# vrenkens/tfkaldi

Measured on AMD Instinct MI355X. Metric: acoustic frames/sec (train step), higher is better.
Workload: dtype f32 emulated (3xbf16 planes, 6 products, f32 accumulate)

## Files before the change

### tfkaldi_amd/build.py

```python
import os
import shutil
import subprocess
import sys
from concurrent.futures import ThreadPoolExecutor

HERE = os.path.dirname(os.path.abspath(__file__))
CSRC = os.path.join(HERE, "csrc")
LIBDIR = os.path.join(HERE, "lib")
LIBNAME = "libtfkaldi_hip.so"
SOURCES = ["gemm_f32.hip", "gemm_bf16.hip", "kernels.hip", "ctc.hip", "engine.hip", "features.hip", "exchange.hip"]
HEADERS = ["gemm_f32.h", "gemm_bf16.h", "kernels.h", "ctc.h", "x3_layout.h", os.path.join("..", "..", "include", "tfkaldi_hip.h")]
FLAGS = ["--offload-arch=gfx950", "-O3", "-std=c++17", "-fPIC", "-Wno-unused-value"]


def lib_path():
    return os.path.join(LIBDIR, LIBNAME)


TRAFFIC_STAMP_SOURCES = ("gemm_f32.hip", "gemm_f32.h", "gemm_bf16.hip", "gemm_bf16.h", "x3_layout.h")


def csrc_hash():
    import hashlib
    h = hashlib.sha256()
    for name in sorted(TRAFFIC_STAMP_SOURCES):
        with open(os.path.join(CSRC, name), "rb") as fid:
            h.update(name.encode() + b"\0" + fid.read())
    return h.hexdigest()[:16]


def _hipcc():
    exe = shutil.which("hipcc") or "/opt/rocm/bin/hipcc"
    if not os.path.exists(exe):
        raise RuntimeError("hipcc not found: cannot build the gfx950 engine")
    return exe


def _digest(names, extra=b""):
    import hashlib
    h = hashlib.sha256(extra)
    for name in names:
        with open(os.path.join(CSRC, name), "rb") as fid:
            h.update(os.path.basename(name).encode() + b"\0" + fid.read() + b"\0")
    return h.hexdigest()


def source_id():
    return _digest(sorted(SOURCES) + sorted(HEADERS), " ".join(FLAGS).encode())[:32]


_ID_MARK = b"TFK_BUILD_ID="


def library_id(path=None):
    path = path or lib_path()
    if not os.path.exists(path):
        return None
    with open(path, "rb") as fid:
        blob = fid.read()
    at = blob.find(_ID_MARK)
    if at < 0:
        return None
    return blob[at + len(_ID_MARK):at + len(_ID_MARK) + 32].decode("ascii", "replace")


def _stale():
    return library_id() != source_id()


def build_native(force=False, verbose=False):
    if not force and not _stale():
        return lib_path()
    hipcc = _hipcc()
    os.makedirs(LIBDIR, exist_ok=True)
    objdir = os.path.join(HERE, "..", "build", "obj")
    os.makedirs(objdir, exist_ok=True)
    build_id = source_id()

    def compile_one(src):
        obj = os.path.join(objdir, src.replace(".hip", ".o"))
        flags = list(FLAGS)
        if src == "engine.hip":
            flags.append('-DTFK_BUILD_ID="%s"' % build_id)
        key = _digest([src] + sorted(HEADERS), " ".join(flags).encode())
        stamp = obj + ".sha256"
        if not force and os.path.exists(obj) and os.path.exists(stamp) and open(stamp).read() == key:
            return obj
        cmd = [hipcc] + flags + ["-c", os.path.join(CSRC, src), "-o", obj]
        r = subprocess.run(cmd, capture_output=True, text=True)
        if r.returncode != 0:
            raise RuntimeError("hipcc failed for %s:\n%s" % (src, r.stderr[-4000:]))
        if verbose and r.stderr:
            sys.stderr.write(r.stderr)
        with open(stamp, "w") as fid:
# ... 19 lines not shown
```

### tfkaldi_amd/csrc/engine.hip

```cpp
#include "../../include/tfkaldi_hip.h"
#include "ctc.h"
#include "gemm_bf16.h"
#include "gemm_f32.h"
#include "kernels.h"

#include <hip/hip_runtime.h>
#include <chrono>

#include <math.h>
#include <stdarg.h>
#include <stdlib.h>
#include <stdio.h>
#include <string.h>

#include <algorithm>
#include <string>
#include <vector>

using namespace tfk;

namespace {

thread_local std::string g_err;

// ... 11 lines not shown
  do {                                                                                            \
    hipError_t e_ = (expr);                                                                       \
    if (e_ != hipSuccess) return fail((int)e_, "%s failed: %s (%s:%d)", #expr, hipGetErrorString(e_), \
                                      __FILE__, __LINE__);                                        \
  } while (0)
#define CHK(expr)            \
  do {                       \
    int rc_ = (expr);        \
    if (rc_ != 0) return rc_; \
  } while (0)

inline size_t up(size_t x, size_t a) { return (x + a - 1) / a * a; }

struct LayerLayout {
  int d_in, d_out, ld_in, ld_out;
  size_t w_off, b_off, beta_off;
  size_t w_sz, b_sz, beta_sz;
};

enum KernelFamily {
  KF_GEMM_NN = 0, KF_GEMM_NT, KF_GEMM_TN, KF_GEMM_DUAL, KF_BN_STATS, KF_ACT_FWD, KF_HIDDEN_BWD, KF_COLSUM, KF_SOFTMAX_XENT,
  KF_LOSS_REDUCE, KF_SOFTMAX, KF_ADAM, KF_EMA, KF_MISC, KF_CTC_BEST_PATH, KF_EDIT_DISTANCE, KF_COUNT
};
const char* kFamilyName[KF_COUNT] = {"gemm_f32_nn(fwd affine)", "gemm_f32_nt(dA)",  "gemm_f32_tn(dW)",
                                     "gemm_f32_dual(dA+dW)",    "bn_stats",
                                     "act_forward",             "hidden_backward",  "colsum",          "softmax_xent",
                                     "loss_reduce",             "softmax_rows",     "adam_apply",      "bn_ema_apply",
                                     "misc",                    "ctc_best_path",    "edit_distance"};

struct ProfRec {
  int family;
  hipEvent_t a, b;
  double flops, bytes;
};

}

struct tfk_engine {
  tfk_config cfg;
  int F, L, H, O, ldF, ldH, ldO;
  float bn_decay, bn_eps, b1, b2, adam_eps;
  bool dropout;

  hipStream_t stream = nullptr, copy_stream = nullptr;
  bool own_stream = false;
  hipStream_t opt_stream = nullptr;
  hipEvent_t ev_opt_begin = nullptr, ev_opt_vec = nullptr;
  std::vector<hipEvent_t> ev_adam;
  bool opt_overlap = false;
  bool opt_pending = false;
  float* d_snap = nullptr;
  hipEvent_t ev_loss = nullptr;
  unsigned loss_seq = 0;
  bool loss_event = false;
  bool slot_lazy = true;
  hipEvent_t ev_grow = nullptr;
  std::vector<void*> host_garbage;

  float* state = nullptr;
  bool own_state = false;
  size_t P = 0, E = 0, state_floats = 0;
  size_t off_param = 0, off_grad = 0, off_scalars = 0, off_ema = 0, off_m = 0, off_v = 0, off_mov = 0, off_shadow = 0;
  size_t reduce_floats = 0;
  std::vector<LayerLayout> lay;

  int cap = 0;
  float* dX[2] = {nullptr, nullptr};
  int32_t* dY[2] = {nullptr, nullptr};
  std::vector<float*> z, a, v, rowscale, mean, rstd;
  float *logits = nullptr, *post = nullptr, *dA[2] = {nullptr, nullptr}, *row_loss = nullptr, *ws = nullptr;
  float* dRaw[2] = {nullptr, nullptr};
  int32_t* dSeg[2] = {nullptr, nullptr};
  float* hRaw[2] = {nullptr, nullptr};
  int32_t* hSeg[2] = {nullptr, nullptr};
  float* dCmvn[2] = {nullptr, nullptr};
  float* hCmvn[2] = {nullptr, nullptr};
  size_t cmvn_cap = 0;
  int seg_cap = 0;
  std::vector<float*> seg_mean, seg_rstd;
  float* ws_stats = nullptr;
  float* ws_bwd = nullptr;
  float* ws_splitk = nullptr;
  size_t ws_splitk_floats = 0;
  size_t ws_bwd_stride = 0;
  float* prior = nullptr;
  bool have_prior = false;

  float* hX[2] = {nullptr, nullptr};
  int32_t* hY[2] = {nullptr, nullptr};
  float* h_post = nullptr;
  size_t h_post_floats = 0;
  float* h_scalars = nullptr;
  float* h_scalars_dev = nullptr;
  bool apply_open = false, apply_direct = false;
  float cur_lr_t = 0.f;
  bool scalars_fresh = true;
  bool colsum_done = false;
  bool fuse_hb_enabled = true;
  bool dual_gemm = true;
  bool stack_enabled = true;
  bool fuse_eval = true;
  int post_chunk = 2048;
  std::vector<hipEvent_t> post_ev;

  int32_t *ctc_seg = nullptr, *ctc_lab_off = nullptr, *ctc_lab = nullptr;
  float *ctc_lp = nullptr, *ctc_ab = nullptr, *ctc_bb = nullptr, *ctc_utt_loss = nullptr, *ctc_lse = nullptr;
  double *ctc_off = nullptr, *ctc_offb = nullptr, *ctc_logz = nullptr;
  size_t ctc_cap_bb = 0, ctc_cap_offb = 0, ctc_cap_logz = 0;
  int32_t* h_ctc[2] = {nullptr, nullptr};
  size_t h_ctc_cap[2] = {0, 0};
  hipEvent_t ctc_staged[2] = {nullptr, nullptr};
  int ctc_stage_slot = 0;
  size_t ctc_cap_offrows = 0;
  size_t ctc_cap_seg = 0, ctc_cap_off = 0, ctc_cap_loss = 0, ctc_cap_lab = 0, ctc_cap_lp = 0, ctc_cap_ab = 0,
         ctc_cap_rows = 0;
  int32_t* ctc_dec = nullptr;
  size_t ctc_cap_dec = 0;
  int32_t* h_dec = nullptr;
  size_t h_dec_cap = 0;

  bool bf16 = false;
  bool x3 = false;
  size_t tw_elems(size_t rows, int ld) const { return x3 ? x3::elems(rows, ld) : rows * ld; }
  size_t tw_row(size_t r, int ld) const { return x3 ? x3::at(r, 0, ld) : r * ld; }
  ShadowMap wb_map;
  int ldFb = 0, ldHb = 0, ldOb = 0;
  bf16_t* Xb[2] = {nullptr, nullptr};
  std::vector<bf16_t*> ab;
  bf16_t* logb = nullptr;
  bf16_t* dAb[2] = {nullptr, nullptr};
  bf16_t* Wb = nullptr;
  std::vector<size_t> wb_off;
  std::vector<int> wb_ld;
  bool wb_aligned = false;
  bool own_wb = false;
  unsigned long long* d_checksum = nullptr;
  bool shadow_dirty = true;
  hipEvent_t copy_done[2] = {nullptr, nullptr}, compute_done[2] = {nullptr, nullptr};
  bool slot_used[2] = {false, false};
  unsigned long long slot_step[2] = {0, 0}, steps_begun = 0, steps_seen = 0;
  int slot = 0;

  int64_t global_step = 0, adam_t = 0;
  double lr_fact = 1.0;
  int initialised_layers = 0;
  uint32_t call_counter = 0;
  int later_mb = 0;
  bool grads_fresh = true;

  tfk_bucket_fn cb = nullptr;
  void* cb_user = nullptr;
  tfk_layer_fn layer_cb = nullptr;
  void* layer_user = nullptr;

  int last_T = 0, last_nfw = 0;
  uint32_t last_call = 0;
  const float* last_in = nullptr;

  bool profiling = false;
  std::vector<ProfRec> prof;
  std::vector<hipEvent_t> ev_pool;
  size_t ev_next = 0;

  int nact() const {
    if (!cfg.layerwise_init) return L;
    int n = initialised_layers + 1;
// ... 165 lines not shown
    to_bf16_rows(e->stream, e->p_param() + y.w_off, y.ld_out, e->Wb + e->wb_off[l], e->wb_ld[l], y.d_in, y.d_out, e->x3);
  }
  HIPCHK(hipGetLastError());
  e->shadow_dirty = false;
  return 0;
}

struct ActEpi {
  const float *a, *z, *mean, *rstd;
  int nonlin;
  const float* beta = nullptr;
  float eps = 0.f;
  bf16_t* twin = nullptr;
  int ld_twin = 0;
  float scale = 1.f;
};
template <class Args>
void fill_epilogue(Args& g, const ActEpi* act, float* stats, const int* row_vend) {
  g.stats = stats;
  g.stats_stride = kMaxRowSplits;
  g.act_a = act ? act->a : nullptr; g.act_z = act ? act->z : nullptr;
  g.act_mean = act ? act->mean : nullptr; g.act_rstd = act ? act->rstd : nullptr;
  g.act_nonlin = act ? act->nonlin : 0;
  g.act_beta = act ? act->beta : nullptr; g.bn_eps = act ? act->eps : 0.f;
  g.act_scale = act ? act->scale : 1.f;
  g.act_keep = act ? 1.f / act->scale : 1.f;
  g.row_vend = row_vend;
}
int grow_splitk(tfk_engine* e, size_t need, bool zero, hipStream_t st) {
  if (need <= e->ws_splitk_floats) return 0;
  dev_free(e, e->ws_splitk, true);
  e->ws_splitk = nullptr;
  e->ws_splitk_floats = 0;
  CHK(dev_alloc(e, (void**)&e->ws_splitk, need * sizeof(float), false));
  e->ws_splitk_floats = need;
  if (zero) HIPCHK(hipMemsetAsync(e->ws_splitk, 0, need * sizeof(float), st));
  return 0;
}
int run_gemm(tfk_engine* e, GemmLayout layout, const float* A, int lda, const float* B, int ldb, float* C, int ldc,
             int M, int N, int K, const float* bias, int epi, hipStream_t st = nullptr, float* stats = nullptr,
             int cfg = -1, const ActEpi* act = nullptr, const int* row_vend = nullptr) {
  if (!st) st = e->stream;
  const int fam = layout == GEMM_NN ? KF_GEMM_NN : layout == GEMM_NT ? KF_GEMM_NT : KF_GEMM_TN;
  if (e->bf16) {
    GemmArgsB b = {};
    int lda8 = 0, ldb8 = 0;
    b.A = twin_of(e, A, &lda8);
    b.B = twin_of(e, B, &ldb8);
    if (!b.A || !b.B) return fail(-1, "internal: GEMM operand without a bf16 twin");
    b.C = C; b.bias = bias;
    fill_epilogue(b, act, stats, row_vend);
    b.C_twin = act ? act->twin : nullptr; b.ldct = act ? act->ld_twin : 0;
    b.ct_x3 = e->x3;
    b.M = M; b.N = N; b.K = K; b.lda = lda8; b.ldb = ldb8; b.ldc = ldc; b.epi = epi;
    if (e->x3) {
      CHK(grow_splitk(e, gemm_bf16x3_splitk_floats(layout, M, N, K), true, st));
      b.splitk_ws = e->ws_splitk;
      b.splitk_ws_floats = e->ws_splitk_floats;
      b.err = reinterpret_cast<unsigned*>(e->h_scalars_dev + kErrWord);
    }
    ProfScope ps(e, fam, 2.0 * M * N * K,
                 (e->x3 ? 6.0 : 2.0) * ((double)M * K + (double)K * N) + 4.0 * (double)M * N * ((epi & EPI_ACCUM) ? 2 : 1), st);
    const int rc = e->x3 ? gemm_bf16x3(layout, b, st) : gemm_bf16(layout, b, st);
    if (rc != 0) return fail(rc, "gemm_bf16%s launch failed: %s", e->x3 ? "x3" : "", hipGetErrorString((hipError_t)rc));
    return 0;
  }
  GemmArgs g;
  g.A = A; g.B = B; g.C = C; g.bias = bias;
  fill_epilogue(g, act, stats, row_vend);
  g.M = M; g.N = N; g.K = K; g.lda = lda; g.ldb = ldb; g.ldc = ldc; g.epi = epi;
  if (layout == GEMM_TN && K >= gemm_f32_splitk_min_k() && (size_t)M * N < ((size_t)1 << 20)) {
    CHK(grow_splitk(e, (size_t)32 * M * ldc, false, st));
    g.splitk_ws = e->ws_splitk;
    g.splitk_ws_floats = e->ws_splitk_floats;
  }
  ProfScope ps(e, fam, 2.0 * M * N * K, 4.0 * ((double)M * K + (double)K * N + (double)M * N * ((epi & EPI_ACCUM) ? 2 : 1)), st);
  const int rc = gemm_f32(layout, g, cfg, st);
  if (rc != 0) return fail(rc, "gemm_f32 launch failed: %s", hipGetErrorString((hipError_t)rc));
  return 0;
}

int run_gemm_dual(tfk_engine* e, const float* dz, int ld_dz, const float* W, int ldw, float* da_out, int ld_da, int T,
                  int N_da, int K_da, const ActEpi* act, float* stats, const float* in, int ld_in, float* Gw, int ld_g,
                  int d_in, int d_out, int epi_w, int* chunk_rows) {
  if (!e->dual_gemm) return 1;
  const double flops = 2.0 * T * N_da * K_da + 2.0 * d_in * d_out * T;
  const double out_w = (double)d_in * d_out * ((epi_w & EPI_ACCUM) ? 2 : 1);
  if (e->bf16) {
    const int dcfg = e->x3 ? -1 : gemm_bf16_dual_config(T, N_da, d_in, d_out);
    const int bm = e->x3 ? kGemmBf16x3TileRows : gemm_bf16_dual_tile_rows(dcfg);
    if (!dcfg || (act && (T + bm - 1) / bm > kMaxRowSplits)) return 1;
    GemmArgsB a = {}, w = {};
    int ld_a = 0, ld_b = 0, ld_c = 0, ld_d = 0;
    a.A = twin_of(e, dz, &ld_a);
    a.B = twin_of(e, W, &ld_b);
    w.A = twin_of(e, in, &ld_c);
    w.B = twin_of(e, dz, &ld_d);
    if (!a.A || !a.B || !w.A || !w.B) return fail(-1, "internal: GEMM operand without a bf16 twin");
    a.C = da_out;
    fill_epilogue(a, act, stats, nullptr);
    a.M = T; a.N = N_da; a.K = K_da; a.lda = ld_a; a.ldb = ld_b; a.ldc = ld_da; a.epi = act ? EPI_DACT : 0;
    w.C = Gw;
    w.M = d_in; w.N = d_out; w.K = T; w.lda = ld_c; w.ldb = ld_d; w.ldc = ld_g; w.epi = epi_w;
    const double ob = e->x3 ? 6.0 : 2.0;
    ProfScope ps(e, KF_GEMM_DUAL, flops, ob * ((double)T * K_da + (double)K_da * N_da) + 4.0 * (double)T * N_da +
                                             ob * ((double)T * d_in + (double)T * d_out) + 4.0 * out_w);
    const int rc = e->x3 ? gemm_bf16x3_dual(a, w, e->stream) : gemm_bf16_dual(a, w, e->stream);
    if (rc != 0) ps.drop();
    if (rc == -1) return 1;
    if (rc != 0) return fail(rc, "gemm_bf16%s_dual launch failed: %s", e->x3 ? "x3" : "", hipGetErrorString((hipError_t)rc));
    if (chunk_rows) *chunk_rows = bm;
    return 0;
  }
  GemmArgs a, w = {};
  a.A = dz; a.B = W; a.C = da_out; a.bias = nullptr;
  fill_epilogue(a, act, stats, nullptr);
  a.M = T; a.N = N_da; a.K = K_da; a.lda = ld_dz; a.ldb = ldw; a.ldc = ld_da; a.epi = act ? EPI_DACT : 0;
  w.A = in; w.B = dz; w.C = Gw;
  w.M = d_in; w.N = d_out; w.K = T; w.lda = ld_in; w.ldb = ld_dz; w.ldc = ld_g; w.epi = epi_w;
  ProfScope ps(e, KF_GEMM_DUAL, flops, 4.0 * ((double)T * K_da + (double)K_da * N_da + (double)T * N_da) +
                                           4.0 * ((double)T * d_in + (double)T * d_out + out_w));
  const int rc = gemm_f32_dual(a, w, e->stream);
  if (rc != 0) ps.drop();
  if (rc == -1) return 1;
  if (rc != 0) return fail(rc, "gemm_f32_dual launch failed: %s", hipGetErrorString((hipError_t)rc));
  return 0;
}

void free_activations(tfk_engine* e, bool async = false) {
  auto fr = [&](float*& p) { dev_free(e, p, async); p = nullptr; };
  for (int s = 0; s < 2; ++s) {
    fr(e->dX[s]);
    dev_free(e, e->dY[s], async); e->dY[s] = nullptr;
    fr(e->dA[s]);
    host_retire(e, e->hX[s], async); e->hX[s] = nullptr;
    host_retire(e, e->hY[s], async); e->hY[s] = nullptr;
    fr(e->dRaw[s]);
    dev_free(e, e->dSeg[s], async); e->dSeg[s] = nullptr;
    host_retire(e, e->hRaw[s], async); e->hRaw[s] = nullptr;
    host_retire(e, e->hSeg[s], async); e->hSeg[s] = nullptr;
    fr(e->dCmvn[s]);
    host_retire(e, e->hCmvn[s], async); e->hCmvn[s] = nullptr;
  }
  e->cmvn_cap = 0;
  auto frb = [&](bf16_t*& p) { dev_free(e, p, async); p = nullptr; };
  for (int s = 0; s < 2; ++s) { frb(e->Xb[s]); frb(e->dAb[s]); }
  for (auto& p : e->ab) frb(p);
  frb(e->logb);
  for (auto& p : e->z) fr(p);
  for (auto& p : e->a) fr(p);
  for (auto& p : e->v) fr(p);
  for (auto& p : e->rowscale) fr(p);
  fr(e->logits); fr(e->post); fr(e->row_loss); fr(e->ws); fr(e->ws_bwd); fr(e->ws_stats);
  e->cap = 0;
}

int alloc_zero(float** p, size_t floats) {
  HIPCHK(hipMalloc((void**)p, floats * sizeof(float)));
  HIPCHK(hipMemset(*p, 0, floats * sizeof(float)));
  return 0;
}
int alloc_zero_b(bf16_t** p, size_t elems) {
  HIPCHK(hipMalloc((void**)p, elems * sizeof(bf16_t)));
  HIPCHK(hipMemset(*p, 0, elems * sizeof(bf16_t)));
  return 0;
}
int grow_zero(tfk_engine* e, float** p, size_t floats) { return dev_alloc(e, (void**)p, floats * sizeof(float), true); }
int grow_zero_b(tfk_engine* e, bf16_t** p, size_t elems) { return dev_alloc(e, (void**)p, elems * sizeof(bf16_t), true); }

inline size_t seg_ints(int cap) { return (size_t)2 * cap + cap / 64 + 8; }

int reserve(tfk_engine* e, int T) {
  if (T <= e->cap) return 0;
  int cap = e->cap + e->cap / 2;
  if (cap < T) cap = T;
  cap = (int)up(cap, 64);
  for (int s = 0; s < 2; ++s)
    if (e->slot_used[s]) HIPCHK(hipEventSynchronize(e->copy_done[s]));
  free_activations(e, true);
  const int L = e->L;
  for (int s = 0; s < 2; ++s) {
    CHK(grow_zero(e, &e->dX[s], (size_t)cap * e->ldF));
    CHK(dev_alloc(e, (void**)&e->dY[s], (size_t)cap * sizeof(int32_t), false));
    CHK(grow_zero(e, &e->dA[s], (size_t)cap * e->ldH));
    HIPCHK(hipHostMalloc((void**)&e->hX[s], (size_t)cap * e->F * sizeof(float), hipHostMallocDefault));
    memset(e->hX[s], 0, (size_t)cap * e->F * sizeof(float));
    HIPCHK(hipHostMalloc((void**)&e->hY[s], (size_t)cap * sizeof(int32_t), hipHostMallocDefault));
    CHK(grow_zero(e, &e->dRaw[s], (size_t)cap * e->ldF));
    CHK(dev_alloc(e, (void**)&e->dSeg[s], seg_ints(cap) * sizeof(int32_t), false));
    HIPCHK(hipHostMalloc((void**)&e->hRaw[s], (size_t)cap * e->F * sizeof(float), hipHostMallocDefault));
// ... 272 lines not shown
      if (e->bf16) { ev.twin = e->ab[l]; ev.ld_twin = e->ldHb; }
      CHK(run_gemm(e, GEMM_NN, in, ld_in, e->p_param() + y.w_off, y.ld_out, e->a[l], ldH, T, H, y.d_in,
                   e->p_param() + y.b_off, EPI_BIAS | EPI_EVAL_ACT, nullptr, nullptr, -1, &ev));
      in = e->a[l];
      ld_in = ldH;
      continue;
    }
    CHK(run_gemm(e, GEMM_NN, in, ld_in, e->p_param() + y.w_off, y.ld_out, e->z[l], ldH, T, H, y.d_in,
                 e->p_param() + y.b_off, EPI_BIAS));
    if (e->cfg.batch_norm) {
      ProfScope ps(e, KF_BN_STATS, 0, 8.0 * T * H);
      if (train)
        bn_stats_train(e->stream, e->z[l], T, H, ldH, e->bn_eps, e->bn_decay, e->mean[l], e->rstd[l], e->ema_mean(l),
                       e->ema_var(l), e->ws);
      else
        bn_stats_eval(e->stream, e->mov_mean(l), e->mov_var(l), H, e->bn_eps, e->mean[l], e->rstd[l]);
    }
    {
      ProfScope ps(e, KF_ACT_FWD, 0, 8.0 * T * H);
      const ActDesc d = act_desc(e, l, train, call);
      act_forward(e->stream, d, e->z[l], e->a[l], e->cfg.l2_norm ? e->v[l] : nullptr,
                  e->cfg.l2_norm ? e->rowscale[l] : nullptr, e->mean[l], e->rstd[l],
                  e->cfg.batch_norm ? e->p_param() + y.beta_off : nullptr, T, H, ldH, twin_a(l));
    }
    in = e->a[l];
    ld_in = ldH;
  }
  const LayerLayout& o = e->lay[e->L];
  need_params(e, e->L);
  CHK(wait_layer_update(e, e->L, nfw == 0));
  CHK(run_gemm(e, GEMM_NN, e->a[nact - 1], ldH, e->p_param() + o.w_off, o.ld_out, e->logits, e->ldO, T, e->O, H,
               e->p_param() + o.b_off, EPI_BIAS));
  HIPCHK(hipGetLastError());
  return 0;
}

int backward(tfk_engine* e, const float* Xd, int ldx, int T, int nact, uint32_t call, bool fire, const Stack* st = nullptr) {
  const int L = e->L, H = e->H, ldH = e->ldH;
  const LayerLayout& o = e->lay[L];
  float* G = e->p_grad();
  const int acc = e->grads_fresh ? 0 : 1;
  const int epi_w = acc ? EPI_ACCUM : 0;
  if (!acc)
    for (int l = nact; l < L; ++l) {
      const LayerLayout& q = e->lay[l];
      HIPCHK(hipMemsetAsync(G + q.w_off, 0, q.w_sz * sizeof(float), e->stream));
      HIPCHK(hipMemsetAsync(G + q.b_off, 0, q.b_sz * sizeof(float), e->stream));
      if (q.beta_sz) HIPCHK(hipMemsetAsync(G + q.beta_off, 0, q.beta_sz * sizeof(float), e->stream));
    }
  FinalBatch fin;
  fin.n = 0;
  fin.accumulate = acc;
  const int rs = row_splits(T);
  auto ws_of = [&](int l) { return e->ws_bwd + (size_t)l * e->ws_bwd_stride; };
  {
    if (!e->colsum_done) {
      ProfScope ps(e, KF_COLSUM, 0, 4.0 * T * e->O);
      colsum_partial(e->stream, e->logits, T, e->ldO, ws_of(L));
    }
    e->colsum_done = false;
    fin.it[fin.n++] = {ws_of(L), G + o.b_off, 0, rs, e->O, e->ldO};
  }
  int pp = 0;
  int cfg_h, cfg_o;
  const int rows_h = gemm_chunk_rows(e, GEMM_NT, T, H, H, &cfg_h), rows_o = gemm_chunk_rows(e, GEMM_NT, T, H, e->O, &cfg_o);
  const bool drop = e->cfg.keep_prob < 1.f;
  const bool fuse_hb = e->cfg.batch_norm && !e->cfg.l2_norm && (!drop || e->cfg.nonlin == TFK_NONLIN_RELU) &&
                       e->fuse_hb_enabled && (T + rows_h - 1) / rows_h <= kMaxRowSplits &&
                       (T + rows_o - 1) / rows_o <= kMaxRowSplits;
  const std::vector<float*>& mean = st ? e->seg_mean : e->mean;
  const std::vector<float*>& rstd = st ? e->seg_rstd : e->rstd;
  auto act_of = [&](int l) {
    ActEpi act = {e->a[l], e->z[l], mean[l], rstd[l], e->cfg.nonlin};
    act.scale = drop ? 1.f / e->cfg.keep_prob : 1.f;
    act.beta = e->cfg.batch_norm ? e->p_param() + e->lay[l].beta_off : nullptr;
    return act;
  };
  auto dact_gemm = [&](const float* dz, int ld_dz, const float* W, int ldw, float* out, int K, int target, int cfg) {
    if (!fuse_hb) return run_gemm(e, GEMM_NT, dz, ld_dz, W, ldw, out, ldH, T, H, K, nullptr, 0);
    const ActEpi act = act_of(target);
    return run_gemm(e, GEMM_NT, dz, ld_dz, W, ldw, out, ldH, T, H, K, nullptr, EPI_DACT, nullptr, ws_of(target), cfg, &act);
  };
  int bm_in = rows_o;
  {
    const ActEpi act = act_of(nact - 1);
    const int rc = run_gemm_dual(e, e->logits, e->ldO, e->p_param() + o.w_off, o.ld_out, e->dA[pp], ldH, T, H, e->O,
                                 fuse_hb ? &act : nullptr, fuse_hb ? ws_of(nact - 1) : nullptr, e->a[nact - 1], ldH,
                                 G + o.w_off, o.ld_out, H, e->O, epi_w, &bm_in);
    if (rc < 0) return rc;
    if (rc > 0) {
      CHK(run_gemm(e, GEMM_TN, e->a[nact - 1], ldH, e->logits, e->ldO, G + o.w_off, o.ld_out, H, e->O, T, nullptr, epi_w));
      CHK(dact_gemm(e->logits, e->ldO, e->p_param() + o.w_off, o.ld_out, e->dA[pp], e->O, nact - 1, cfg_o));
    }
  }
  if (fire && e->cb) {
    e->cb(e->cb_user, 0);
    for (int l = L - 1; l >= nact; --l) e->cb(e->cb_user, L - l);
  }
  for (int l = nact - 1; l >= 0; --l) {
    const LayerLayout& y = e->lay[l];
    float* da = e->dA[pp];
    const int chunks_in = (T + bm_in - 1) / bm_in;
    auto fin_layer = [&](int n_beta, int n_bias) {
      if (e->cfg.batch_norm) fin.it[fin.n++] = {ws_of(l), G + y.beta_off, 0, n_beta, H, ldH};
      fin.it[fin.n++] = {ws_of(l), G + y.b_off, 2, n_bias, H, ldH};
      if (fin.n + 2 > kMaxFinalItems) {
        grad_final(e->stream, fin);
        fin.n = 0;
      }
    };
    Twin tw;
    if (e->bf16) { tw.p = e->dAb[pp]; tw.ld = e->ldHb; tw.x3 = e->x3; }
    if (st) {
      if (!fuse_hb || stack_align(e) % bm_in || chunks_in > kMaxRowSplits)
        return fail(-1, "internal: EPI_DACT chunks of %d rows do not fit a stacked pass of %d rows", bm_in, T);
      int slot = 0;
      for (int i = 0; i < st->k; ++i) {
        ProfScope ps(e, KF_HIDDEN_BWD, 0, 28.0 * st->rows[i] * H);
        const ActDesc d = act_desc(e, l, 1, call + (uint32_t)i);
        Twin tws = tw;
        if (e->bf16) tws.p += e->tw_row((size_t)st->r0[i], e->ldHb);
        const size_t r = (size_t)st->r0[i] * ldH;
        hidden_backward(e->stream, d, 1, da + r, e->a[l] + r, e->z[l] + r, mean[l] + (size_t)i * ldH, rstd[l] + (size_t)i * ldH,
                        st->rows[i], H, ldH, ws_of(l) + (size_t)(st->r0[i] / bm_in) * ldH, (st->rows[i] + bm_in - 1) / bm_in, tws,
                        st->span[i], ws_of(l) + ((size_t)2 * kMaxRowSplits + slot) * ldH);
        slot += row_splits(st->span[i]);
      }
      if (slot > kMaxRowSplits) return fail(-1, "internal: %d partial-sum slots in a stacked pass", slot);
      fin_layer(chunks_in, slot);
    } else {
      const ActDesc d = act_desc(e, l, 1, call);
      int pre_du = fuse_hb ? 1 : 0;
      if (e->cfg.l2_norm) {
        ProfScope ps(e, KF_HIDDEN_BWD, 0, 12.0 * T * H);
        act_backward_rows(e->stream, d, da, e->v[l], e->rowscale[l], T, H, ldH);
        pre_du = 1;
      }
      ProfScope ps(e, KF_HIDDEN_BWD, 0, (e->cfg.batch_norm ? 28.0 : 12.0) * T * H);
      int chunks_eff = fuse_hb ? chunks_in : 0;
      if (chunks_eff > kMergeOnceChunks) {
        chunk_totals(e->stream, ws_of(l), chunks_eff, ldH);
        chunks_eff = 1;
      }
      hidden_backward(e->stream, d, pre_du, da, e->a[l], e->z[l], mean[l], rstd[l], T, H, ldH, ws_of(l), chunks_eff, tw);
      fin_layer(fuse_hb ? chunks_eff : rs, rs);
    }
    const float* in = l == 0 ? Xd : e->a[l - 1];
    const int ld_in = l == 0 ? ldx : ldH;
    bool fused = false;
    bm_in = rows_h;
    if (l > 0) {
      const ActEpi act = act_of(l - 1);
      const int rc = run_gemm_dual(e, da, ldH, e->p_param() + y.w_off, y.ld_out, e->dA[pp ^ 1], ldH, T, H, H,
                                   fuse_hb ? &act : nullptr, fuse_hb ? ws_of(l - 1) : nullptr, in, ld_in, G + y.w_off,
                                   y.ld_out, y.d_in, H, epi_w, &bm_in);
      if (rc < 0) return rc;
      fused = rc == 0;
    }
    if (!fused) {
      CHK(run_gemm(e, GEMM_TN, in, ld_in, da, ldH, G + y.w_off, y.ld_out, y.d_in, H, T, nullptr, epi_w));
      if (l > 0) CHK(dact_gemm(da, ldH, e->p_param() + y.w_off, y.ld_out, e->dA[pp ^ 1], H, l - 1, cfg_h));
    }
    if (fire && e->cb) e->cb(e->cb_user, L - l);
    pp ^= 1;
  }
  {
    ProfScope ps(e, KF_COLSUM, 0, 0);
    grad_final(e->stream, fin);
  }
  HIPCHK(hipGetLastError());
  return 0;
}

int check_kernel_errors(tfk_engine* e) {
  volatile unsigned* w = reinterpret_cast<volatile unsigned*>(e->h_scalars + kErrWord);
  if (*w == 0) return 0;
  *w = 0;
  if (e->ws_splitk)
    (void)hipMemsetAsync(e->ws_splitk, 0, e->ws_splitk_floats * sizeof(float), e->stream);
  return fail(-1, "split-K exchange timed out: a block of the fp32-emulating contraction waited ~1 s for its partner's partial "
                  "sums (workspace not zeroed, or the partner block failed); the results of this step are invalid");
}

int settle_scalars(tfk_engine* e) {
  if (e->scalars_fresh) {
    HIPCHK(hipMemsetAsync(e->p_scalars(), 0, kScalarFloats * sizeof(float), e->stream));
    e->scalars_fresh = false;
  }
  return 0;
}
int read_scalars(tfk_engine* e) {
  CHK(settle_scalars(e));
  HIPCHK(hipMemcpyAsync(e->h_scalars, e->p_scalars(), 4 * sizeof(float), hipMemcpyDeviceToHost, e->stream));
  HIPCHK(hipStreamSynchronize(e->stream));
  e->scalars_fresh = true;
  return check_kernel_errors(e);
}

struct TensorRef {
  float* ptr;
  int rows, cols, ld;
};
int tensor_ref(tfk_engine* e, int kind, int slot, int layer, TensorRef* t) {
  const int L = e->L;
  if (kind == TFK_WEIGHTS || kind == TFK_BIASES) {
    if (layer < 0 || layer > L) return fail(-1, "layer %d out of range [0, %d]", layer, L);
  } else if (kind >= TFK_BN_BETA && kind <= TFK_BN_MOVING_VAR) {
    if (layer < 0 || layer >= L) return fail(-1, "layer %d out of range [0, %d)", layer, L);
    if (!e->cfg.batch_norm) return fail(-1, "batch norm tensors requested but batch_norm is off");
  } else {
    return fail(-1, "unknown tensor kind %d", kind);
  }
  float* base;
  switch (slot) {
    case TFK_SLOT_PARAM: base = e->p_param(); break;
    case TFK_SLOT_GRAD: base = e->p_grad(); break;
    case TFK_SLOT_ADAM_M: base = e->p_m(); break;
    case TFK_SLOT_ADAM_V: base = e->p_v(); break;
    default: return fail(-1, "unknown tensor slot %d", slot);
  }
  const LayerLayout& y = e->lay[layer < 0 ? 0 : layer];
  switch (kind) {
    case TFK_WEIGHTS: *t = {base + y.w_off, y.d_in, y.d_out, y.ld_out}; break;
    case TFK_BIASES: *t = {base + y.b_off, 1, y.d_out, y.ld_out}; break;
    case TFK_BN_BETA: *t = {base + y.beta_off, 1, e->H, e->ldH}; break;
    case TFK_BN_MOVING_MEAN:
    case TFK_BN_MOVING_VAR:
      if (slot != TFK_SLOT_PARAM) return fail(-1, "moving statistics only have the PARAM slot");
      *t = {kind == TFK_BN_MOVING_MEAN ? e->mov_mean(layer) : e->mov_var(layer), 1, e->H, e->ldH};
      break;
  }
  return 0;
}

int create_impl(const tfk_config* cfg, void* state, size_t state_bytes, void* stream, tfk_engine** out) {
  if (!out) return fail(-1, "out is NULL");
  *out = nullptr;
  CHK(validate(cfg));
  HIPCHK(hipSetDevice(cfg->device));
  tfk_engine* e = new tfk_engine();
  e->cfg = *cfg;
  e->F = cfg->input_dim; e->L = cfg->num_layers; e->H = cfg->num_units; e->O = cfg->output_dim;
  e->ldF = (int)up(e->F, 4); e->ldH = (int)up(e->H, 4); e->ldO = (int)up(e->O, 4);
  e->bf16 = cfg->compute_dtype != TFK_DTYPE_F32;
  e->x3 = cfg->compute_dtype == TFK_DTYPE_F32X3;
  const size_t ldq = e->x3 ? 32 : 8;
  e->ldFb = (int)up(e->F, ldq); e->ldHb = (int)up(e->H, ldq); e->ldOb = (int)up(e->O, ldq);
  e->bn_decay = cfg->bn_decay > 0.f ? cfg->bn_decay : 0.999f;
  e->bn_eps = cfg->bn_epsilon > 0.f ? cfg->bn_epsilon : 1e-3f;
  e->b1 = cfg->adam_beta1 > 0.f ? cfg->adam_beta1 : 0.9f;
  e->b2 = cfg->adam_beta2 > 0.f ? cfg->adam_beta2 : 0.999f;
  e->adam_eps = cfg->adam_epsilon > 0.f ? cfg->adam_epsilon : 1e-8f;
  e->dropout = cfg->keep_prob < 1.f;
  compute_layout(cfg, e->lay, e->P, e->E);
  e->state_floats = total_state_floats(e->P, e->E, shadow_floats(cfg, e->lay));
  e->off_param = 0;
  e->off_grad = e->P;
  e->off_scalars = 2 * e->P;
  e->off_ema = 2 * e->P + kScalarFloats;
  e->reduce_floats = e->P + kScalarFloats + e->E;
  e->off_m = e->off_ema + e->E;
  e->off_v = e->off_m + e->P;
  e->off_mov = e->off_v + e->P;
  e->off_shadow = e->off_mov + e->E;

  auto bail = [&](int rc) { tfk_destroy(e); return rc; };
#define HIPB(expr)                                                                                          \
  do {                                                                                                      \
    hipError_t e_ = (expr);                                                                                 \
    if (e_ != hipSuccess) return bail(fail((int)e_, "%s failed: %s", #expr, hipGetErrorString(e_)));        \
  } while (0)
  if (stream) {
    e->stream = (hipStream_t)stream;
  } else {
    HIPB(hipStreamCreateWithFlags(&e->stream, hipStreamNonBlocking));
    e->own_stream = true;
  }
  HIPB(hipStreamCreateWithFlags(&e->copy_stream, hipStreamNonBlocking));
  {
    const char* v;
    if ((v = getenv("TFK_FUSE_HB"))) e->fuse_hb_enabled = atoi(v) != 0;
    if ((v = getenv("TFK_POST_CHUNK"))) e->post_chunk = atoi(v) > 0 ? (int)up((size_t)atoi(v), 64) : 0;
    if ((v = getenv("TFK_DUAL_GEMM"))) e->dual_gemm = atoi(v) != 0;
    if ((v = getenv("TFK_STACK"))) e->stack_enabled = atoi(v) != 0;
    if ((v = getenv("TFK_LOSS_EVENT"))) e->loss_event = atoi(v) != 0;
    if ((v = getenv("TFK_SLOT_EVENT"))) e->slot_lazy = atoi(v) == 0;
    if ((v = getenv("TFK_FUSE_EVAL"))) e->fuse_eval = atoi(v) != 0;
  }
  {
    const char* v = getenv("TFK_ADAM_OVERLAP");
    e->opt_overlap = v ? atoi(v) != 0 : false;
  }
  if (e->opt_overlap) {
    HIPB(hipStreamCreateWithFlags(&e->opt_stream, hipStreamNonBlocking));
    HIPB(hipEventCreateWithFlags(&e->ev_opt_begin, hipEventDisableTiming));
    HIPB(hipEventCreateWithFlags(&e->ev_opt_vec, hipEventDisableTiming));
    e->ev_adam.assign(e->L + 1, nullptr);
    for (int l = 0; l <= e->L; ++l) HIPB(hipEventCreateWithFlags(&e->ev_adam[l], hipEventDisableTiming));
  }
  HIPB(hipMalloc((void**)&e->d_snap, 16 * sizeof(float)));
  HIPB(hipEventCreateWithFlags(&e->ev_loss, hipEventDisableTiming));
  HIPB(hipEventCreateWithFlags(&e->ev_grow, hipEventDisableTiming));
  for (int s = 0; s < 2; ++s) {
    HIPB(hipEventCreateWithFlags(&e->copy_done[s], hipEventDisableTiming));
    HIPB(hipEventCreateWithFlags(&e->compute_done[s], hipEventDisableTiming));
  }
  if (state) {
    if (state_bytes < e->state_floats * sizeof(float))
      return bail(fail(-1, "state arena too small: %zu < %zu bytes", state_bytes, e->state_floats * sizeof(float)));
    if (((uintptr_t)state) % 256) return bail(fail(-1, "state arena must be 256-byte aligned"));
    e->state = (float*)state;
  } else {
    HIPB(hipMalloc((void**)&e->state, e->state_floats * sizeof(float)));
    e->own_state = true;
  }
  HIPB(hipMemsetAsync(e->state, 0, e->state_floats * sizeof(float), e->stream));
  if (cfg->batch_norm)
    for (int l = 0; l < e->L; ++l) fill(e->stream, e->mov_var(l), (size_t)e->H, 1.0f);
  HIPB(hipHostMalloc((void**)&e->h_scalars, 16 * sizeof(float), hipHostMallocMapped | hipHostMallocCoherent));
  memset(e->h_scalars, 0, 16 * sizeof(float));
  HIPB(hipHostGetDevicePointer((void**)&e->h_scalars_dev, e->h_scalars, 0));
  e->mean.assign(e->L, nullptr);
  e->rstd.assign(e->L, nullptr);
  for (int l = 0; l < e->L; ++l) {
    if (alloc_zero(&e->mean[l], (size_t)e->ldH) || alloc_zero(&e->rstd[l], (size_t)e->ldH)) return bail(-1);
  }
  if (alloc_zero(&e->prior, (size_t)e->ldO)) return bail(-1);
  if (e->bf16) {
    e->wb_aligned = e->x3 ? (e->L + 1 <= kShadowMapMax) : shadow_mirrors(cfg, e->lay);
    e->wb_off.assign(e->L + 1, 0);
    e->wb_ld.assign(e->L + 1, 0);
    e->wb_map.n = 0;
    size_t off = 0;
    for (int l = 0; l <= e->L; ++l) {
      const LayerLayout& y = e->lay[l];
      e->wb_ld[l] = (int)up(y.d_out, e->x3 ? 32 : 8);
      e->wb_off[l] = (e->wb_aligned && !e->x3) ? y.w_off : off;
      off += e->x3 ? up(x3::elems(y.d_in, e->wb_ld[l]), 64) : up((size_t)y.d_in * e->wb_ld[l], 64);
      if (e->x3 && e->wb_aligned) {
        ShadowMap& m = e->wb_map;
        m.begin[l] = (uint32_t)y.w_off; m.rows[l] = (uint32_t)y.d_in; m.ld[l] = (uint32_t)y.ld_out;
        m.ld_twin[l] = (uint32_t)e->wb_ld[l]; m.twin[l] = e->wb_off[l];
        m.n = l + 1;
      }
    }
    if (e->x3) {
      if (alloc_zero_b(&e->Wb, up(off, 128))) return bail(-1);
      e->own_wb = true;
    } else if (e->wb_aligned) {
      e->Wb = reinterpret_cast<bf16_t*>(e->state + e->off_shadow);
    } else {
      if (alloc_zero_b(&e->Wb, off)) return bail(-1);
      e->own_wb = true;
    }
    e->shadow_dirty = true;
  }
  const int cap0 = cfg->max_frames > 0 ? cfg->max_frames : 1024;
  { const int rc = reserve(e, cap0); if (rc) return bail(rc); }
  HIPB(hipStreamSynchronize(e->stream));
#undef HIPB
  *out = e;
  return 0;
}

struct CtcSpec {
  const int32_t* utt_len;
  int U;
  const int32_t* labels;
  const int32_t* label_len;
};
template <class Tp>
int grow(tfk_engine* e, Tp** p, size_t* cap, size_t need) {
  if (need <= *cap) return 0;
  dev_free(e, *p, true);
  *p = nullptr;
  *cap = 0;
  const size_t n = need + need / 2;
  CHK(dev_alloc(e, (void**)p, n * sizeof(Tp), false));
  *cap = n;
  return 0;
}
int ctc_stage(tfk_engine* e, const CtcSpec& c, int T, bool need_labels, int* max_labels_out) {
  if (c.U <= 0 || !c.utt_len || (need_labels && !c.label_len)) return fail(-1, "CTC: no utterances");
  std::vector<int32_t> seg(c.U + 1, 0), off(c.U + 1, 0);
  int max_labels = 0;
  for (int u = 0; u < c.U; ++u) {
    const int32_t n = c.label_len ? c.label_len[u] : 0;
    if (c.utt_len[u] < 0 || n < 0) return fail(-1, "CTC: negative length");
    seg[u + 1] = seg[u] + c.utt_len[u];
    off[u + 1] = off[u] + n;
    max_labels = n > max_labels ? n : max_labels;
  }
  if (seg[c.U] != T) return fail(-1, "CTC: utterance lengths sum to %d, expected T = %d", seg[c.U], T);
  if (max_labels > kCtcMaxLabels) return fail(-1, "CTC: %d labels in one utterance (limit %d)", max_labels, kCtcMaxLabels);
  const int total = off[c.U];
  if (total > 0 && !c.labels) return fail(-1, "CTC: labels is NULL");
  for (int i = 0; i < total; ++i)
    if (c.labels[i] < 0 || c.labels[i] >= e->O - 1) return fail(-1, "CTC: label %d outside [0, %d)", c.labels[i], e->O - 1);
  CHK(grow(e, &e->ctc_seg, &e->ctc_cap_seg, (size_t)c.U + 1));
  CHK(grow(e, &e->ctc_lab_off, &e->ctc_cap_off, (size_t)c.U + 1));
  CHK(grow(e, &e->ctc_lab, &e->ctc_cap_lab, (size_t)(total > 0 ? total : 1)));
  {
    const int k = e->ctc_stage_slot ^= 1;
    const size_t need = 2 * ((size_t)c.U + 1) + (size_t)total;
    if (!e->ctc_staged[k]) HIPCHK(hipEventCreateWithFlags(&e->ctc_staged[k], hipEventDisableTiming));
    else HIPCHK(hipEventSynchronize(e->ctc_staged[k]));
    if (need > e->h_ctc_cap[k]) {
      if (e->h_ctc[k]) HIPCHK(hipHostFree(e->h_ctc[k]));
      e->h_ctc[k] = nullptr;
      e->h_ctc_cap[k] = need + need / 2;
// ... 271 lines not shown
  int D;
};
int check_seg_utts(const tfk_engine* e, const char* who, const int32_t* utt_len, int U, int T, int context_width,
                   const int32_t* seg_utts, int k, int flags, SegTable* t) {
  if (flags & (TFK_DEVICE_PTRS | TFK_RAW_DEVICE)) return fail(-1, "%s takes host pointers", who);
  if (k <= 0) return fail(-1, "no micro-batch (k = %d)", k);
  const int win = 2 * context_width + 1;
  if (context_width < 0 || e->F % win) return fail(-1, "input_dim %d is not a multiple of 2*context_width+1 = %d", e->F, win);
  t->D = e->F / win;
  t->first_utt.assign(k + 1, 0);
  t->first_row.assign(k + 1, 0);
  t->seg_rows.assign(k, 0);
  for (int i = 0; i < k; ++i) {
    if (seg_utts[i] <= 0) return fail(-1, "micro-batch %d of the stack holds no utterance", i);
    t->first_utt[i + 1] = t->first_utt[i] + seg_utts[i];
    if (t->first_utt[i + 1] > U) return fail(-1, "the micro-batches hold more than U = %d utterances", U);
    for (int u = t->first_utt[i]; u < t->first_utt[i + 1]; ++u) {
      if (utt_len[u] < 0) return fail(-1, "negative utterance length");
      t->seg_rows[i] += utt_len[u];
    }
    if (t->seg_rows[i] <= 0) return fail(-1, "micro-batch %d of the stack is empty", i);
    t->first_row[i + 1] = t->first_row[i] + t->seg_rows[i];
  }
  if (t->first_utt[k] != U || t->first_row[k] != T)
    return fail(-1, "the micro-batches hold %d utterances / %d frames, expected U = %d / T = %d", t->first_utt[k], t->first_row[k], U, T);
  return 0;
}

}

namespace tfk {
int set_error(int code, const char* msg) { return fail(code, "%s", msg); }
}

extern "C" {

int tfk_abi_version(void) { return TFK_ABI_VERSION; }
#ifndef TFK_BUILD_ID
#error "compile engine.hip through tfkaldi_amd/build.py: it passes -DTFK_BUILD_ID=<hash of the sources>"
#endif
static const char kBuildId[] = "TFK_BUILD_ID=" TFK_BUILD_ID;
const char* tfk_build_id(void) { return kBuildId + 13; }
const char* tfk_last_error(void) { return g_err.c_str(); }

int tfk_state_bytes(const tfk_config* cfg, size_t* bytes) {
  CHK(validate(cfg));
  if (!bytes) return fail(-1, "bytes is NULL");
  std::vector<LayerLayout> lay;
  size_t P, E;
  compute_layout(cfg, lay, P, E);
  *bytes = total_state_floats(P, E, shadow_floats(cfg, lay)) * sizeof(float);
  return 0;
}

int tfk_create(const tfk_config* cfg, tfk_engine** out) { return create_impl(cfg, nullptr, 0, nullptr, out); }
int tfk_create_ex(const tfk_config* cfg, void* state, size_t state_bytes, void* stream, tfk_engine** out) {
  return create_impl(cfg, state, state_bytes, stream, out);
}

int tfk_destroy(tfk_engine* e) {
  if (!e) return 0;
  hipSetDevice(e->cfg.device);
  if (e->stream) hipStreamSynchronize(e->stream);
  if (e->copy_stream) hipStreamSynchronize(e->copy_stream);
  if (e->opt_stream) hipStreamSynchronize(e->opt_stream);
  free_activations(e);
  for (void* p : e->host_garbage) (void)hipHostFree(p);
  e->host_garbage.clear();
  if (e->ev_loss) hipEventDestroy(e->ev_loss);
  if (e->ev_grow) hipEventDestroy(e->ev_grow);
  if (e->ev_opt_begin) hipEventDestroy(e->ev_opt_begin);
  if (e->ev_opt_vec) hipEventDestroy(e->ev_opt_vec);
  for (hipEvent_t ev : e->ev_adam) if (ev) hipEventDestroy(ev);
  if (e->opt_stream) hipStreamDestroy(e->opt_stream);
  if (e->d_snap) hipFree(e->d_snap);
  for (auto p : e->mean) if (p) hipFree(p);
  for (auto p : e->seg_mean) if (p) hipFree(p);
  for (auto p : e->seg_rstd) if (p) hipFree(p);
  for (auto p : e->rstd) if (p) hipFree(p);
  if (e->prior) hipFree(e->prior);
  if (e->Wb && e->own_wb) hipFree(e->Wb);
  if (e->d_checksum) hipFree(e->d_checksum);
  if (e->ws_splitk) hipFree(e->ws_splitk);
  for (void* p : {(void*)e->ctc_seg, (void*)e->ctc_lab_off, (void*)e->ctc_lab, (void*)e->ctc_lp, (void*)e->ctc_ab,
                  (void*)e->ctc_utt_loss, (void*)e->ctc_lse, (void*)e->ctc_off, (void*)e->ctc_bb, (void*)e->ctc_offb,
                  (void*)e->ctc_logz, (void*)e->ctc_dec})
    if (p) hipFree(p);
  if (e->h_dec) hipHostFree(e->h_dec);
  for (hipEvent_t ev : e->post_ev) hipEventDestroy(ev);
  for (int k = 0; k < 2; ++k) {
    if (e->h_ctc[k]) hipHostFree(e->h_ctc[k]);
    if (e->ctc_staged[k]) hipEventDestroy(e->ctc_staged[k]);
  }
  if (e->h_scalars) hipHostFree(e->h_scalars);
  if (e->h_post) hipHostFree(e->h_post);
  if (e->own_state && e->state) hipFree(e->state);
  for (int s = 0; s < 2; ++s) {
    if (e->copy_done[s]) hipEventDestroy(e->copy_done[s]);
    if (e->compute_done[s]) hipEventDestroy(e->compute_done[s]);
  }
  for (auto ev : e->ev_pool) hipEventDestroy(ev);
  if (e->copy_stream) hipStreamDestroy(e->copy_stream);
  if (e->own_stream && e->stream) hipStreamDestroy(e->stream);
  delete e;
  return 0;
}

int tfk_tensor_count(tfk_engine* e, int kind, int layer, size_t* count) {
  if (!e || !count) return fail(-1, "NULL argument");
  TensorRef t;
  CHK(tensor_ref(e, kind, TFK_SLOT_PARAM, layer, &t));
  *count = (size_t)t.rows * t.cols;
  return 0;
}

int tfk_tensor_get(tfk_engine* e, int kind, int slot, int layer, float* host, size_t count) {
  if (!e || !host) return fail(-1, "NULL argument");
  TensorRef t;
  CHK(tensor_ref(e, kind, slot, layer, &t));
  if (count != (size_t)t.rows * t.cols) return fail(-1, "count %zu != %d x %d", count, t.rows, t.cols);
  HIPCHK(hipSetDevice(e->cfg.device));
  if (slot == TFK_SLOT_GRAD && e->grads_fresh) {
    memset(host, 0, count * sizeof(float));
    return 0;
  }
  if (slot == TFK_SLOT_PARAM) need_params(e, -1);
  CHK(sync_streams(e));
  HIPCHK(hipMemcpy2D(host, (size_t)t.cols * 4, t.ptr, (size_t)t.ld * 4, (size_t)t.cols * 4, t.rows, hipMemcpyDeviceToHost));
  return 0;
}

int tfk_tensor_set(tfk_engine* e, int kind, int slot, int layer, const float* host, size_t count) {
  if (!e || !host) return fail(-1, "NULL argument");
  TensorRef t;
  CHK(tensor_ref(e, kind, slot, layer, &t));
  if (count != (size_t)t.rows * t.cols) return fail(-1, "count %zu != %d x %d", count, t.rows, t.cols);
  HIPCHK(hipSetDevice(e->cfg.device));
  if (slot == TFK_SLOT_PARAM) need_params(e, -1);
  CHK(sync_streams(e));
  if (slot == TFK_SLOT_GRAD && e->grads_fresh) {
    HIPCHK(hipMemsetAsync(e->p_grad(), 0, e->P * sizeof(float), e->stream));
    e->grads_fresh = false;
  }
  HIPCHK(hipStreamSynchronize(e->stream));
  HIPCHK(hipMemcpy2D(t.ptr, (size_t)t.ld * 4, host, (size_t)t.cols * 4, (size_t)t.cols * 4, t.rows, hipMemcpyHostToDevice));
  if (slot == TFK_SLOT_PARAM) e->shadow_dirty = true;
  return 0;
}

static double current_lr(const tfk_engine* e) {
  const double frac = e->cfg.num_steps > 0 ? (double)e->global_step / (double)e->cfg.num_steps : 0.0;
  return (double)e->cfg.init_learning_rate * pow((double)e->cfg.learning_rate_decay, frac) * e->lr_fact;
}

int tfk_scalar_get(tfk_engine* e, int which, double* value) {
  if (!e || !value) return fail(-1, "NULL argument");
  switch (which) {
    case TFK_GLOBAL_STEP: *value = (double)e->global_step; return 0;
    case TFK_LEARNING_RATE_FACT: *value = e->lr_fact; return 0;
    case TFK_INITIALISED_LAYERS: *value = (double)e->initialised_layers; return 0;
    case TFK_ADAM_STEPS: *value = (double)e->adam_t; return 0;
    case TFK_LEARNING_RATE: *value = current_lr(e); return 0;
    case TFK_BATCH_LOSS:
    case TFK_NUM_FRAMES: {
      HIPCHK(hipSetDevice(e->cfg.device));
      if (e->scalars_fresh) { *value = 0.0; return 0; }
// ... 857 lines not shown
```

### tfkaldi_amd/csrc/gemm_bf16.h

```cpp
#pragma once
#include <hip/hip_runtime.h>
#include <stdint.h>

#include "gemm_f32.h"

namespace tfk {

typedef uint16_t bf16_t;

struct GemmArgsB {
  const bf16_t* A;
  const bf16_t* B;
  float* C;
  const float* bias;
  float* stats;
  const float* act_a;
  const float* act_z;
  const float* act_mean;
  const float* act_rstd;
  int act_nonlin;
  int stats_stride;
  int M, N, K;
  int lda, ldb, ldc;
  int epi;
  const float* act_beta;
  float bn_eps;
  bf16_t* C_twin;
  int ldct;
  float act_scale;
  float act_keep;
  const int* row_vend;
  int ct_x3;
  float* splitk_ws;
  size_t splitk_ws_floats;
  unsigned* err;
  int splitk_local;
  int splitk_skew;
};

constexpr int kNumGemmBf16Configs = 9;

int gemm_bf16(GemmLayout layout, const GemmArgsB& args, hipStream_t stream);

int gemm_bf16_dual(const GemmArgsB& nt, const GemmArgsB& tn, hipStream_t stream);
int gemm_bf16_dual_config(int M_nt, int N_nt, int M_tn, int N_tn);
int gemm_bf16_dual_tile_rows(int cfg);

int gemm_bf16x3(GemmLayout layout, const GemmArgsB& args, hipStream_t stream);
constexpr int kGemmBf16x3TileRows = 128;
size_t gemm_bf16x3_splitk_floats(GemmLayout layout, int M, int N, int K);
int gemm_bf16x3_dual(const GemmArgsB& nt, const GemmArgsB& tn, hipStream_t stream);

int gemm_bf16_tile_rows(int M, int N);

void gemm_bf16_force_config(int cfg);
int gemm_bf16_pick_config(int M, int N);

}
```

### tfkaldi_amd/csrc/gemm_bf16.hip

```cpp
#include "gemm_bf16.h"
#include "x3_layout.h"

#include <math.h>
#include <stdlib.h>
#include <string.h>

#include <type_traits>

namespace tfk {
namespace {

typedef __bf16 bf16x8 __attribute__((ext_vector_type(8)));
typedef __bf16 bf16x4 __attribute__((ext_vector_type(4)));
typedef float f32x16 __attribute__((ext_vector_type(16)));
typedef uint32_t u32x4 __attribute__((ext_vector_type(4)));
typedef int i32x4 __attribute__((ext_vector_type(4)));

constexpr int BK = 64;
constexpr int kOOB = (int)0x80000000;
constexpr int NUM_XCD = 8;

__device__ __forceinline__ void tile_of_seq(int tiles_m, int tiles_n, int group_rows, int seq, int& tm, int& tn) {
  const int per_group = group_rows * tiles_n;
  const int grp = seq / per_group;
  const int first_m = grp * group_rows;
  const int gsize = min(group_rows, tiles_m - first_m);
  const int within = seq - grp * per_group;
  tm = first_m + within % gsize;
  tn = within / gsize;
}
__device__ __forceinline__ void tile_of_block(int tiles_m, int tiles_n, int group_rows, int bid, int& tm, int& tn) {
  const int nwg = tiles_m * tiles_n;
  const int xcd = bid % NUM_XCD, loc = bid / NUM_XCD;
  const int q = nwg / NUM_XCD, r = nwg % NUM_XCD;
  const int seq = (xcd < r ? xcd * (q + 1) : r * (q + 1) + (xcd - r) * q) + loc;
  tile_of_seq(tiles_m, tiles_n, group_rows, seq, tm, tn);
}

__device__ __forceinline__ uint16_t f2bf(float x) { return __builtin_bit_cast(uint16_t, (__bf16)x); }

template <int EPI, int WAVES_M, int WAVES_N, int FM, int FN, bool CBUF = false>
__device__ __forceinline__ void epilogue(const GemmArgsB& p, f32x16 (&acc)[FM][FN], int tiles_m, int tm, int m0, int n0,
                                         int wm, int wn, int i, int h, float* red) {
  constexpr int BM = WAVES_M * FM * 32, BN = WAVES_N * FN * 32;
  auto row_of = [&](int a, int r) { return m0 + (wm * FM + a) * 32 + 4 * h + (r & 3) + 8 * (r >> 2); };
#pragma unroll
  for (int b = 0; b < FN; ++b) {
    const int cidx = (wn * FN + b) * 32 + i;
    const int col = n0 + cidx;
    const bool col_ok = col < p.N;
    const int colc = col_ok ? col : p.N - 1;
    if constexpr ((EPI & EPI_BIAS) != 0) {
      const float bv = p.bias[colc];
#pragma unroll
      for (int a = 0; a < FM; ++a)
#pragma unroll
        for (int r = 0; r < 16; ++r) acc[a][b][r] += bv;
    }
    if constexpr ((EPI & EPI_EVAL_ACT) != 0) {
      const bool bn = p.act_mean != nullptr;
      const float mu = bn ? p.act_mean[colc] : 0.f;
      const float rs = bn ? rsqrtf(p.act_rstd[colc] + p.bn_eps) : 1.f;
      const float be = bn ? p.act_beta[colc] : 0.f;
#pragma unroll
      for (int a = 0; a < FM; ++a)
#pragma unroll
        for (int r = 0; r < 16; ++r) {
          float u = acc[a][b][r];
          if (bn) u = (u - mu) * rs + be;
          switch (p.act_nonlin) {
            case 0: u = fmaxf(u, 0.f); break;
            case 1: u = 1.f / (1.f + expf(-u)); break;
            case 2: u = tanhf(u); break;
            default: break;
          }
          acc[a][b][r] = u;
        }
    }
    if constexpr ((EPI & EPI_COLSTATS) != 0) {
      const int vlim = p.row_vend ? min(p.M, p.row_vend[m0 >> 6]) : p.M;
      const int n_tile = max(1, min(BM, vlim - m0));
      float cmean = 0.f;
#pragma unroll
      for (int pass = 0; pass < 2; ++pass) {
        float s = 0.f;
#pragma unroll
        for (int a = 0; a < FM; ++a)
#pragma unroll
          for (int r = 0; r < 16; ++r) {
            const float v = acc[a][b][r];
            if (row_of(a, r) < vlim) s += pass == 0 ? v : (v - cmean) * (v - cmean);
          }
        s += __shfl_xor(s, 32);
        if (h == 0) red[wm * BN + cidx] = s;
        __syncthreads();
        float t = 0.f;
#pragma unroll
        for (int w = 0; w < WAVES_M; ++w) t += red[w * BN + cidx];
        if (pass == 0) {
          cmean = t / (float)n_tile;
        } else if (wm == 0 && h == 0 && col_ok) {
          p.stats[((size_t)0 * tiles_m + tm) * p.ldc + col] = cmean;
          p.stats[((size_t)1 * tiles_m + tm) * p.ldc + col] = t;
        }
        __syncthreads();
      }
    }
    if constexpr ((EPI & EPI_DACT) != 0) {
      const float mu = p.act_mean[colc], rsd = p.act_rstd[colc];
      const float dscale = p.act_scale > 0.f ? p.act_scale : 1.f;
      const bool from_a = p.act_nonlin == 0 && p.act_beta != nullptr;
      const float be = from_a ? p.act_beta[colc] : 0.f;
      const float keep = p.act_keep > 0.f ? p.act_keep : 1.f;
      float s1 = 0.f, s2 = 0.f;
#pragma unroll
      for (int a = 0; a < FM; ++a) {
        float av[16], zv[16];
#pragma unroll
        for (int r = 0; r < 16; ++r) {
          const int row = min(row_of(a, r), p.M - 1);
          av[r] = p.act_a[(size_t)row * p.ldc + colc];
        }
        if (!from_a) {
#pragma unroll
          for (int r = 0; r < 16; ++r) {
            const int row = min(row_of(a, r), p.M - 1);
            zv[r] = p.act_z[(size_t)row * p.ldc + colc];
          }
        }
#pragma unroll
        for (int r = 0; r < 16; ++r) {
          float d1;
          switch (p.act_nonlin) {
            case 0: d1 = av[r] > 0.f ? dscale : 0.f; break;
            case 1: d1 = av[r] * (1.f - av[r]); break;
            case 2: d1 = 1.f - av[r] * av[r]; break;
            default: d1 = 1.f;
          }
          const float du = acc[a][b][r] * d1;
          acc[a][b][r] = du;
          if (row_of(a, r) < p.M) {
            s1 += du;
            s2 += du * (from_a ? av[r] * keep - be : (zv[r] - mu) * rsd);
          }
        }
      }
      s1 += __shfl_xor(s1, 32);
      s2 += __shfl_xor(s2, 32);
      if (h == 0) {
        red[(0 * WAVES_M + wm) * BN + cidx] = s1;
        red[(1 * WAVES_M + wm) * BN + cidx] = s2;
      }
      __syncthreads();
      if (wm == 0 && h == 0 && col_ok) {
        float t1 = 0.f, t2 = 0.f;
#pragma unroll
        for (int w = 0; w < WAVES_M; ++w) {
          t1 += red[(0 * WAVES_M + w) * BN + cidx];
          t2 += red[(1 * WAVES_M + w) * BN + cidx];
        }
        p.stats[((size_t)0 * p.stats_stride + tm) * p.ldc + col] = t1;
        p.stats[((size_t)1 * p.stats_stride + tm) * p.ldc + col] = t2;
      }
      __syncthreads();
    }
    if constexpr (CBUF) {
      static_assert((EPI & EPI_EVAL_ACT) == 0, "no bf16 twin on this path");
      const __amdgpu_buffer_rsrc_t crs =
          __builtin_amdgcn_make_buffer_rsrc((void*)p.C, 0, (int)(((unsigned)(p.M - 1) * p.ldc + p.N) * 4u), 0x00020000);
#pragma unroll
      for (int a = 0; a < FM; ++a) {
        const unsigned base = col_ok ? ((unsigned)(m0 + (wm * FM + a) * 32 + 4 * h) * p.ldc + col) * 4u : (unsigned)kOOB;
        float old[16];
        if constexpr ((EPI & EPI_ACCUM) != 0) {
#pragma unroll
          for (int r = 0; r < 16; ++r)
            old[r] = __builtin_bit_cast(float, __builtin_amdgcn_raw_buffer_load_b32(
                                                   crs, base + (unsigned)(((r & 3) + 8 * (r >> 2)) * p.ldc) * 4u, 0, 0));
        }
#pragma unroll
        for (int r = 0; r < 16; ++r) {
          float v = acc[a][b][r];
          if (EPI & EPI_ACCUM) v += old[r];
          __builtin_amdgcn_raw_buffer_store_b32(__builtin_bit_cast(unsigned, v), crs,
                                                base + (unsigned)(((r & 3) + 8 * (r >> 2)) * p.ldc) * 4u, 0, 0);
        }
      }
      continue;
    }
#pragma unroll
    for (int a = 0; a < FM; ++a) {
      float old[16];
      if constexpr ((EPI & EPI_ACCUM) != 0) {
#pragma unroll
        for (int r = 0; r < 16; ++r) old[r] = p.C[(size_t)min(row_of(a, r), p.M - 1) * p.ldc + colc];
      }
#pragma unroll
      for (int r = 0; r < 16; ++r) {
        const int row = row_of(a, r);
        float v = acc[a][b][r];
        if (EPI & EPI_ACCUM) v += old[r];
        if (col_ok && row < p.M) {
          p.C[(size_t)row * p.ldc + col] = v;
          if constexpr ((EPI & EPI_EVAL_ACT) != 0) {
            if (p.C_twin) {
              if (p.ct_x3) {
                const size_t at = x3::at((size_t)row, col, p.ldct);
                uint16_t q0, q1, q2;
                x3::split3(v, q0, q1, q2);
                p.C_twin[at] = (bf16_t)q0;
                p.C_twin[at + 64] = (bf16_t)q1;
                p.C_twin[at + 128] = (bf16_t)q2;
              } else {
                p.C_twin[(size_t)row * p.ldct + col] = f2bf(v);
              }
            }
          }
        }
      }
    }
  }
}


template <int EXT>
__device__ __forceinline__ int ks_swz(int r) {
  return EXT == 64 ? (((r >> 1) & 1) << 2) : ((r & 3) << 2);
}

template <bool KC, int EXT, int NTH, int BKT = 64>
struct DmaOperand {
  static_assert(BKT == 64 || BKT == 32, "ring slot of 64 or 32 k");
  static constexpr int NP = EXT * BKT / 8 / NTH;
  static_assert((EXT * BKT / 8) % NTH == 0 && NP >= 1, "pieces per thread");
  i32x4 rsrc;
  int voff[NP];
  int kidx[NP];
  int kstride;
  int k_lim;

  __device__ __forceinline__ void init(const bf16_t* base, int ld, int rows, int ext0, int ext_lim, int k_lim_,
                                       int tid, long extra_bytes = 0) {
    const unsigned long long a = (unsigned long long)base;
    rsrc[0] = (int)(unsigned)a;
    rsrc[1] = (int)((unsigned)(a >> 32) & 0xffffu);
    rsrc[2] = (int)(rows * ld * 2 + extra_bytes);
    rsrc[3] = 0x00020000;
    k_lim = k_lim_;
    kstride = KC ? 2 : ld * 2;
#pragma unroll
    for (int j = 0; j < NP; ++j) {
      const int idx = tid + j * NTH;
      if (KC) {
        constexpr int CPR = BKT / 8;
        const int r = idx / CPR;
        const int sw = BKT == 64 ? ((r >> 1) & 7) : ((r >> 2) & 3);
        const int k = ((idx % CPR) ^ sw) << 3;
        const int e = ext0 + r;
        voff[j] = e < ext_lim ? (e * ld + k) * 2 : kOOB;
        kidx[j] = k;
      } else {
        constexpr int CH = EXT / 8;
        const int r = idx / CH;
        const int c = (idx % CH) ^ ks_swz<EXT>(r);
        const int e = ext0 + (c << 3);
        voff[j] = e < ext_lim ? (r * ld + e) * 2 : kOOB;
        kidx[j] = r;
      }
// ... 81 lines not shown
  __device__ __forceinline__ void issue(int j, unsigned image, int k0, int wave) const {
    const int off = (!GUARD || k0 + kidx[j] < k_lim) ? voff[j] : kOOB;
    const unsigned dst = image + (unsigned)(wave * 64 + j * NTH) * 16u;
    const int soff = k0 * kstride;
    asm volatile("s_mov_b32 m0, %0\n\ts_nop 0\n\tbuffer_load_dwordx4 %1, %2, %3 offen lds"
                 :
                 : "s"(dst), "v"(off), "s"(rsrc), "s"(soff)
                 : "memory");
  }
};

template <bool KC, int EXT, int NF>
struct Frag3 {
  int off[2];
  __device__ __forceinline__ void init(int lane, int frag0) {
#pragma unroll
    for (int v = 0; v < 2; ++v) off[v] = KC ? x3::kc_lane_off(lane, frag0, v) : x3::ks_lane_off<EXT>(lane, frag0, v);
  }
  __device__ __forceinline__ Frag3 at(int bytes) const {
    Frag3 r;
    r.off[0] = off[0] + bytes;
    r.off[1] = off[1] + bytes;
    return r;
  }
  __device__ __forceinline__ bf16x8 read(const char* img, int f, int ks, int pl) const {
    if constexpr (KC) {
      return *reinterpret_cast<const bf16x8*>(img + off[ks] + x3::kc_imm(f, pl));
    } else {
      typedef __attribute__((address_space(3))) bf16x4 lds_bf16x4;
      const int X = 3 * f + pl;
      const char* q = img + off[X & 1];
      const bf16x4 lo = __builtin_amdgcn_ds_read_tr16_b64_v4bf16((lds_bf16x4*)(q + x3::ks_imm<EXT>(X, ks, 0)));
      const bf16x4 hi = __builtin_amdgcn_ds_read_tr16_b64_v4bf16((lds_bf16x4*)(q + x3::ks_imm<EXT>(X, ks, 1)));
      return __builtin_shufflevector(lo, hi, 0, 1, 2, 3, 4, 5, 6, 7);
    }
  }
};

template <bool KC, int EXT, int NF16>
struct Frag3M {
  int off[KC ? 1 : 4];
  __device__ __forceinline__ void init(int lane, int frag0) {
    if constexpr (KC) {
      off[0] = x3::kc16_lane_off(lane, frag0);
    } else {
#pragma unroll
      for (int v = 0; v < 4; ++v) off[v] = x3::ks16_lane_off<EXT>(lane, frag0, v & 1, v >> 1);
    }
  }
  __device__ __forceinline__ Frag3M at(int bytes) const {
    Frag3M r;
#pragma unroll
    for (int v = 0; v < (KC ? 1 : 4); ++v) r.off[v] = off[v] + bytes;
    return r;
  }
  __device__ __forceinline__ bf16x8 read(const char* img, int f, int pl) const {
    if constexpr (KC) {
      return *reinterpret_cast<const bf16x8*>(img + off[0] + x3::kc16_imm(f, pl));
    } else {
      typedef __attribute__((address_space(3))) bf16x4 lds_bf16x4;
      const int X = 3 * (f >> 1) + pl;
      const char* q = img + off[(X & 1) + 2 * (f & 1)];
      const bf16x4 lo = __builtin_amdgcn_ds_read_tr16_b64_v4bf16((lds_bf16x4*)(q + x3::ks16_imm<EXT>(X, 0)));
      const bf16x4 hi = __builtin_amdgcn_ds_read_tr16_b64_v4bf16((lds_bf16x4*)(q + x3::ks16_imm<EXT>(X, 1)));
      return __builtin_shufflevector(lo, hi, 0, 1, 2, 3, 4, 5, 6, 7);
    }
  }
};

#ifndef TFKB_ABL
#define TFKB_ABL 0
#endif

#ifndef TFKB_TL
#define TFKB_TL(ev, ti)
#endif

#define TFKB_WAIT_BARRIER(n) \
  asm volatile("s_waitcnt vmcnt(%0)\n\ts_waitcnt lgkmcnt(0)\n\ts_barrier" : : "n"(n) : "memory")

constexpr int kSplitFlagWords = 4096;
constexpr int kSplitXccWord = 2048;
template <bool A_KC, bool B_KC, int EPI, int WAVES_M, int WAVES_N, int FM, int FN, int NS, int BKT = 64, int SCHED = 0,
          int NPL = 1, int KSPLIT = 1, int LOADERS = 0, bool LIST = false, bool CBUF = false>
__device__ __forceinline__ void dma_tile(const GemmArgsB& p, int tiles_m, int tiles_n, int group_rows, int bid, char* smem,
                                         int seq0 = 0, int ntiles = 1) {
  static_assert(LOADERS == 0 || (NPL == 3 && LOADERS == WAVES_M * WAVES_N), "loader waves: one per multiplying wave, x3 only");
  static_assert(!LIST || (NPL == 3 && KSPLIT == 1 && LOADERS == 0), "tile lists: the unsplit fp32-emulating contraction, no loader waves");
  constexpr int NTH = WAVES_M * WAVES_N * 64;
  constexpr int BM = WAVES_M * FM * 32, BN = WAVES_N * FN * 32;
  typedef typename std::conditional<NPL == 3, DmaOperand3<A_KC, BM, NTH>, DmaOperand<A_KC, BM, NTH, BKT>>::type OA;
  typedef typename std::conditional<NPL == 3, DmaOperand3<B_KC, BN, NTH>, DmaOperand<B_KC, BN, NTH, BKT>>::type OB;
  constexpr int A_BYTES = BM * BKT * 2, B_BYTES = BN * BKT * 2, STAGE = NPL * (A_BYTES + B_BYTES);
  constexpr int NPA = OA::NP, NPB = OB::NP, NP = OA::NP + OB::NP;
  constexpr int KSPT = BKT / 16;
  static_assert(KSPT == 4 || KSPT == 2, "ring slot of 64 or 32 k");
  static_assert(NS >= 3 && (NS - 2) * NP + (NPL == 3 ? NP / 2 : 0) <= 63, "ring depth / vmcnt range");
  static_assert(FM * FN >= 2 || NPL == 3, "two independent accumulator chains per wave");
  static_assert(NPL == 1 || (NPL == 3 && SCHED == 0), "planes");
  static_assert(KSPLIT == 1 || (KSPLIT == 2 && NPL == 3), "split-K: the fp32-emulating contraction only");

  const int tid = threadIdx.x;
  const int lane = tid & 63;
  const int i = lane & 31, h = lane >> 5;
  const int wave = __builtin_amdgcn_readfirstlane(tid >> 6);
  const int wm = wave / WAVES_N, wn = wave % WAVES_N;
  int tm, tn;
  const int khalf = KSPLIT == 2 ? (bid / NUM_XCD) & 1 : 0;
  const int tile_bid = KSPLIT == 2 ? (bid / NUM_XCD >> 1) * NUM_XCD + bid % NUM_XCD : bid;
  if constexpr (LIST) tile_of_seq(tiles_m, tiles_n, group_rows, seq0, tm, tn);
  else tile_of_block(tiles_m, tiles_n, group_rows, tile_bid, tm, tn);
  int m0 = tm * BM, n0 = tn * BN;
  unsigned my_xcc = 0;
  if constexpr (KSPLIT == 2) {
    if (p.splitk_local) {
      asm volatile("s_getreg_b32 %0, hwreg(HW_REG_XCC_ID, 0, 4)" : "=s"(my_xcc));
      if (tid == 0)
        __hip_atomic_store(reinterpret_cast<unsigned*>(p.splitk_ws) + kSplitXccWord + 2 * (tm * tiles_n + tn) + khalf, my_xcc + 1,
                           __ATOMIC_RELAXED, __HIP_MEMORY_SCOPE_AGENT);
    }
  }

  const int K8 = (p.K + 7) & ~7;
  const int nk_all = (p.K + BKT - 1) / BKT;
  const int h0 = KSPLIT == 2 ? max(1, (nk_all + 1) / 2 - p.splitk_skew) : nk_all;
  const int kbase = khalf ? h0 : 0;
  const int nk = KSPLIT == 2 ? (khalf ? nk_all - h0 : h0) : nk_all;
  const int k_end = (kbase + nk) * BKT;
  const unsigned lds0 = __builtin_amdgcn_readfirstlane((unsigned)(unsigned long long)smem);
  OA la;
  OB lb;
  const int a_klim = min(A_KC ? K8 : p.K, k_end), b_klim = min(B_KC ? K8 : p.K, k_end);
  const int nk_full = min(a_klim, b_klim) / BKT - kbase;
  if constexpr (LOADERS > 0) {
    if (wave >= WAVES_M * WAVES_N) {
      const int lwave = wave - WAVES_M * WAVES_N;
      la.init(p.A, p.lda, A_KC ? p.M : p.K, m0, A_KC ? p.M : ((p.M + 7) & ~7), a_klim, tid - NTH);
      lb.init(p.B, p.ldb, B_KC ? p.N : p.K, n0, B_KC ? p.N : ((p.N + 7) & ~7), b_klim, tid - NTH);
      auto tile = [&](auto guard, int slot, int kt) {
        if (TFKB_ABL & 2) return;
#pragma unroll
        for (int j = 0; j < NPA; ++j)
          la.template issue<decltype(guard)::value>(j, lds0 + (unsigned)(slot * STAGE), (kt + kbase) * BKT, lwave);
#pragma unroll
        for (int j = 0; j < NPB; ++j)
          lb.template issue<decltype(guard)::value>(j, lds0 + (unsigned)(slot * STAGE + NPL * A_BYTES), (kt + kbase) * BKT, lwave);
      };
#pragma unroll
      for (int t = 0; t < NS - 1; ++t) tile(std::true_type(), t, t);
      TFKB_WAIT_BARRIER((NS - 2) * NP);
      int ws = NS - 1;
      const int n_fast = max(0, min(nk, nk_full - (NS - 1)));
#pragma unroll 1
      for (int kt = 0; kt < nk; ++kt) {
        if (kt < n_fast) tile(std::false_type(), ws, kt + NS - 1);
        else tile(std::true_type(), ws, kt + NS - 1);
        TFKB_WAIT_BARRIER((NS - 2) * NP);
        ws = ws + 1 == NS ? 0 : ws + 1;
      }
      TFKB_WAIT_BARRIER(0);
      return;
    }
  }
  auto init_loaders = [&]() {
    if constexpr (LOADERS == 0) {
      la.init(p.A, p.lda, A_KC ? p.M : p.K, m0, A_KC ? p.M : ((p.M + 7) & ~7), a_klim, tid);
      lb.init(p.B, p.ldb, B_KC ? p.N : p.K, n0, B_KC ? p.N : ((p.N + 7) & ~7), b_klim, tid);
    }
  };
  init_loaders();
  typename std::conditional<NPL == 3, Frag3<A_KC, BM, FM>, Frag<A_KC, BM, FM, BKT>>::type qa;
// ... 302 lines not shown
#pragma unroll
            for (int a = 0; a < FM; ++a)
#pragma unroll
              for (int b = 0; b < FN; ++b) {
                if (c < 5)
                  acc2[a][b] = __builtin_amdgcn_mfma_f32_32x32x16_bf16(fa[cur][PA[c]][a], fb[cur][PB[c]][b], acc2[a][b], 0, 0, 0);
                else
                  acc[a][b] = __builtin_amdgcn_mfma_f32_32x32x16_bf16(fa[cur][PA[c]][a], fb[cur][PB[c]][b], acc[a][b], 0, 0, 0);
              }
          }
          __builtin_amdgcn_sched_barrier(0);
        }
      };
      if (!primed) read_frags(0, smem, 0);
      const int n_fast = max(0, min(nk, nk_full - NS));
      auto iteration = [&](auto guard, int t1, int t2, bool fetch, bool switch_tile) {
        const auto ra = qa.at(rs * STAGE);
        const auto rb = qb.at(rs * STAGE + NPL * A_BYTES);
        step3(guard, 0, true, ra, rb, 1, NPH, NP, ws, t1);
        TFKB_WAIT_BARRIER((NS - 2) * NP);
        rs = rs + 1 == NS ? 0 : rs + 1;
        ws = ws + 1 == NS ? 0 : ws + 1;
        if constexpr (CHAIN) {
          if (switch_tile) {
            tile_of_seq(tiles_m, tiles_n, group_rows, seq0 + ti + 1, tm, tn);
            m0 = tm * BM;
            n0 = tn * BN;
            init_loaders();
          }
        }
        const auto na = qa.at(rs * STAGE);
        const auto nb = qb.at(rs * STAGE + NPL * A_BYTES);
        step3(guard, 1, fetch, na, nb, 0, 0, NPH, ws, t2);
      };
      const int n_own = chain_next ? nk - NS : nk;
      TFKB_TL(1, ti);
#pragma unroll 1
      for (int kt = 0; kt < n_fast; ++kt) iteration(std::false_type(), kt + NS - 1, kt + NS, kt + 1 < nk, false);
#pragma unroll 1
      for (int kt = n_fast; kt < n_own; ++kt) iteration(std::true_type(), kt + NS - 1, kt + NS, kt + 1 < nk, false);
      if constexpr (CHAIN) {
        if (chain_next) {
          iteration(std::true_type(), nk - 1, 0, true, true);
#pragma unroll 1
          for (int t = 0; t < NS - 1; ++t) iteration(std::true_type(), t, t + 1, true, false);
        }
      }
      TFKB_TL(2, ti);
    } else {
    read_frags(0, smem, 0);
#pragma unroll 1
    for (int kt = 0; kt < nk; ++kt) {
      const char* st = smem + rs * STAGE;
#pragma unroll
      for (int ks = 0; ks < KSPT - 1; ++ks) {
        const int cur = ks & 1;
        read_frags(cur ^ 1, st, ks + 1);
#pragma unroll
        for (int j = ks * NP / (KSPT - 1); j < (ks + 1) * NP / (KSPT - 1); ++j) piece(j, ws, kt + NS - 1);
        mfma_step(cur);
        __builtin_amdgcn_sched_barrier(0);
      }
      TFKB_WAIT_BARRIER((NS - 2) * NP);
      rs = rs + 1 == NS ? 0 : rs + 1;
      ws = ws + 1 == NS ? 0 : ws + 1;
      if (kt + 1 < nk) read_frags(0, smem + rs * STAGE, 0);
      mfma_step((KSPT - 1) & 1);
      __builtin_amdgcn_sched_barrier(0);
    }
    }
    if (!chain_next) TFKB_WAIT_BARRIER(0);
    if constexpr (NPL == 3) {
#pragma unroll
      for (int a = 0; a < FM; ++a)
#pragma unroll
        for (int b = 0; b < FN; ++b)
#pragma unroll
          for (int r = 0; r < 16; ++r) acc[a][b][r] += acc2[a][b][r];
    }
    if constexpr (KSPLIT == 2) {
      typedef float f32x4 __attribute__((ext_vector_type(4)));
      unsigned* flags = reinterpret_cast<unsigned*>(p.splitk_ws);
      const int tile = tm * tiles_n + tn;
      constexpr int kSys = 1 | (1 << 4);
      __amdgpu_buffer_rsrc_t part = __builtin_amdgcn_make_buffer_rsrc(
          (void*)(p.splitk_ws + kSplitFlagWords + (size_t)tile * (BM * BN)), 0, BM * BN * 4, 0x00020000);
      unsigned* sh = reinterpret_cast<unsigned*>(smem);
      if (tid == 0) {
        sh[0] = __hip_atomic_fetch_add(&flags[2 * tile], 1u, __ATOMIC_RELAXED, __HIP_MEMORY_SCOPE_AGENT);
        sh[1] = p.splitk_local ? __hip_atomic_load(&flags[kSplitXccWord + 2 * tile + (khalf ^ 1)], __ATOMIC_RELAXED, __HIP_MEMORY_SCOPE_AGENT)
                               : 0u;
      }
      __syncthreads();
      const bool first = sh[0] == 0;
      if (first) {
        const bool same_xcd = p.splitk_local && sh[1] == my_xcc + 1;
        if (same_xcd) {
#pragma unroll
          for (int a = 0; a < FM; ++a)
#pragma unroll
            for (int b = 0; b < FN; ++b)
#pragma unroll
              for (int q = 0; q < 4; ++q)
                __builtin_amdgcn_raw_buffer_store_b128(
                    __builtin_bit_cast(u32x4, f32x4{acc[a][b][4 * q], acc[a][b][4 * q + 1], acc[a][b][4 * q + 2], acc[a][b][4 * q + 3]}),
                    part, ((((wave * FM + a) * FN + b) * 4 + q) * 64 + lane) * 16, 0, 0);
        } else {
#pragma unroll
          for (int a = 0; a < FM; ++a)
#pragma unroll
            for (int b = 0; b < FN; ++b)
#pragma unroll
              for (int q = 0; q < 4; ++q)
                __builtin_amdgcn_raw_buffer_store_b128(
                    __builtin_bit_cast(u32x4, f32x4{acc[a][b][4 * q], acc[a][b][4 * q + 1], acc[a][b][4 * q + 2], acc[a][b][4 * q + 3]}),
                    part, ((((wave * FM + a) * FN + b) * 4 + q) * 64 + lane) * 16, 0, kSys);
        }
        asm volatile("s_waitcnt vmcnt(0)" : : : "memory");
        __syncthreads();
        if (tid == 0) __hip_atomic_store(&flags[2 * tile + 1], 1u, __ATOMIC_RELAXED, __HIP_MEMORY_SCOPE_AGENT);
        return;
      }
      if (tid == 0) {
        int spin = 0;
        for (; spin < (1 << 23) && __hip_atomic_load(&flags[2 * tile + 1], __ATOMIC_RELAXED, __HIP_MEMORY_SCOPE_AGENT) == 0; ++spin)
          __builtin_amdgcn_s_sleep(2);
        if (spin == (1 << 23) && p.err) __hip_atomic_store(p.err, 1u, __ATOMIC_RELAXED, __HIP_MEMORY_SCOPE_SYSTEM);
        __hip_atomic_store(&flags[2 * tile], 0u, __ATOMIC_RELAXED, __HIP_MEMORY_SCOPE_AGENT);
        __hip_atomic_store(&flags[2 * tile + 1], 0u, __ATOMIC_RELAXED, __HIP_MEMORY_SCOPE_AGENT);
        __hip_atomic_store(&flags[kSplitXccWord + 2 * tile], 0u, __ATOMIC_RELAXED, __HIP_MEMORY_SCOPE_AGENT);
        __hip_atomic_store(&flags[kSplitXccWord + 2 * tile + 1], 0u, __ATOMIC_RELAXED, __HIP_MEMORY_SCOPE_AGENT);
      }
      __syncthreads();
#pragma unroll
      for (int a = 0; a < FM; ++a)
#pragma unroll
        for (int b = 0; b < FN; ++b)
#pragma unroll
          for (int q = 0; q < 4; ++q) {
            const f32x4 o = __builtin_bit_cast(
                f32x4, __builtin_amdgcn_raw_buffer_load_b128(part, ((((wave * FM + a) * FN + b) * 4 + q) * 64 + lane) * 16, 0, kSys));
            acc[a][b][4 * q] += o.x;
            acc[a][b][4 * q + 1] += o.y;
            acc[a][b][4 * q + 2] += o.z;
            acc[a][b][4 * q + 3] += o.w;
          }
      __syncthreads();
    }
    epilogue<EPI, WAVES_M, WAVES_N, FM, FN, CBUF>(p, acc, tiles_m, tm_out, m0_out, n0_out, wm, wn, i, h, red);
    TFKB_TL(3, ti);
    if constexpr (LIST) {
      primed = chain_next;
      if (!chain_next && ti + 1 < nlist) __syncthreads();
    }
  }
}

template <bool A_KC, bool B_KC, int EPI, int WAVES_M, int WAVES_N, int FM, int FN, int NS, int BKT = 64, int SCHED = 0,
          int NPL = 1, int KSPLIT = 1, int LOADERS = 0>
__global__ void __launch_bounds__((WAVES_M * WAVES_N + LOADERS) * 64)
gemm_bf16_dma_kernel(GemmArgsB p, int tiles_m, int tiles_n, int group_rows) {
  extern __shared__ __attribute__((aligned(16))) char smem[];
  dma_tile<A_KC, B_KC, EPI, WAVES_M, WAVES_N, FM, FN, NS, BKT, SCHED, NPL, KSPLIT, LOADERS>(p, tiles_m, tiles_n, group_rows,
                                                                                            blockIdx.x, smem);
}

template <int EPI_NT, int EPI_TN, int GWM, int GWN, int GFM, int GFN, int GNS, int HWM, int HWN, int HFM, int HFN, int HNS,
          int HBK>
__global__ void __launch_bounds__(GWM * GWN * 64)
gemm_bf16_dual_kernel(GemmArgsB p1, GemmArgsB p2, int tiles_m1, int tiles_n1, int group1, int tiles_m2, int tiles_n2,
                      int group2) {
  static_assert(GWM * GWN == HWM * HWN, "both halves run on the same block size");
  extern __shared__ __attribute__((aligned(16))) char smem[];
  const int n1 = tiles_m1 * tiles_n1;
  if ((int)blockIdx.x < n1)
    dma_tile<true, true, EPI_NT, GWM, GWN, GFM, GFN, GNS>(p1, tiles_m1, tiles_n1, group1, blockIdx.x, smem);
  else
    dma_tile<false, false, EPI_TN, HWM, HWN, HFM, HFN, HNS, HBK, (HBK == 32 ? 2 : 0)>(p2, tiles_m2, tiles_n2, group2, blockIdx.x - n1,
                                                                                      smem);
}

constexpr int NT = 256, PF = 4;
constexpr int KC_LD = BK + 8;

template <bool KC, int EXT>
struct Operand {
  static constexpr int LD = KC ? KC_LD : EXT + 32;
  static constexpr int SZ = (KC ? EXT : BK) * LD;
  static constexpr int NCH = EXT * BK / 8 / NT;
};

template <bool KC, int EXT>
struct Loader {
  static constexpr int NCH = Operand<KC, EXT>::NCH;
  __amdgpu_buffer_rsrc_t rsrc;
  int voff[NCH];
  int kidx[NCH];
  int kstride;
  int k_lim;

  static __device__ __forceinline__ void coords(int c, int& r, int& q) {
    if (KC) { r = c >> 3; q = (c & 7) << 3; }
    else { r = c / (EXT / 8); q = (c % (EXT / 8)) << 3; }
  }
  __device__ __forceinline__ void init(const bf16_t* base, int ld, int rows, int ext0, int ext_lim, int k_lim_,
                                       int tid) {
    rsrc = __builtin_amdgcn_make_buffer_rsrc((void*)base, 0, rows * ld * 2, 0x00020000);
    k_lim = k_lim_;
    kstride = KC ? 2 : ld * 2;
#pragma unroll
    for (int j = 0; j < NCH; ++j) {
      int r, q;
      coords(tid + j * NT, r, q);
      if (KC) {
        voff[j] = (ext0 + r < ext_lim) ? ((ext0 + r) * ld + q) * 2 : kOOB;
        kidx[j] = q;
      } else {
        voff[j] = (ext0 + q < ext_lim) ? (r * ld + ext0 + q) * 2 : kOOB;
        kidx[j] = r;
      }
    }
  }
  __device__ __forceinline__ void load(u32x4 (&v)[NCH], int k0) const {
#pragma unroll
    for (int j = 0; j < NCH; ++j) {
      const int off = (k0 + kidx[j] < k_lim) ? voff[j] : kOOB;
      v[j] = __builtin_amdgcn_raw_buffer_load_b128(rsrc, off, k0 * kstride, 0);
    }
  }
  __device__ __forceinline__ void store(const u32x4 (&v)[NCH], bf16_t* s, int tid) const {
#pragma unroll
    for (int j = 0; j < NCH; ++j) {
// ... 39 lines not shown
  tile_of_block(tiles_m, tiles_n, group_rows, blockIdx.x, tm, tn);
  const int m0 = tm * BM, n0 = tn * BN;

  const int K8 = (p.K + 7) & ~7;
  Loader<A_KC, BM> la;
  Loader<B_KC, BN> lb;
  la.init(p.A, p.lda, A_KC ? p.M : p.K, m0, A_KC ? p.M : ((p.M + 7) & ~7), A_KC ? K8 : p.K, tid);
  lb.init(p.B, p.ldb, B_KC ? p.N : p.K, n0, B_KC ? p.N : ((p.N + 7) & ~7), B_KC ? K8 : p.K, tid);

  constexpr bool ALT = FM * FN == 1;
  f32x16 acc[FM][FN], acc_alt;
#pragma unroll
  for (int r = 0; r < 16; ++r) acc_alt[r] = 0.f;
#pragma unroll
  for (int a = 0; a < FM; ++a)
#pragma unroll
    for (int b = 0; b < FN; ++b)
#pragma unroll
      for (int r = 0; r < 16; ++r) acc[a][b][r] = 0.f;

  const int nk = (p.K + BK - 1) / BK;
  u32x4 ra[PF][OA::NCH], rb[PF][OB::NCH];
#pragma unroll
  for (int j = 0; j < PF; ++j) {
    la.load(ra[j], j * BK);
    lb.load(rb[j], j * BK);
  }
  bf16_t* st0 = smem;
  bf16_t* st1 = smem + STAGE;
  bf16_t* st2 = smem + 2 * STAGE;
  la.store(ra[0], st0, tid);
  lb.store(rb[0], st0 + A_SZ, tid);
  la.store(ra[1], st1, tid);
  lb.store(rb[1], st1 + A_SZ, tid);
  la.load(ra[0], PF * BK);
  lb.load(rb[0], PF * BK);
  la.load(ra[1], (PF + 1) * BK);
  lb.load(rb[1], (PF + 1) * BK);
  __syncthreads();
  bf16x8 fa[2][FM], fb[2][FN];
  auto read_frags = [&](int buf, const bf16_t* st, int ks) {
#pragma unroll
    for (int a = 0; a < FM; ++a) fa[buf][a] = fragment<A_KC, OA::LD>(st, wm * 32 * FM + a * 32, ks, lane);
#pragma unroll
    for (int b = 0; b < FN; ++b) fb[buf][b] = fragment<B_KC, OB::LD>(st + A_SZ, wn * 32 * FN + b * 32, ks, lane);
  };
  read_frags(0, st0, 0);
#pragma unroll 1
  for (int kt0 = 0; kt0 < nk; kt0 += PF) {
#pragma unroll
    for (int j = 0; j < PF; ++j) {
      const int kt = kt0 + j;
      const int s2 = (j + 2) % PF;
      la.store(ra[s2], st2, tid);
      lb.store(rb[s2], st2 + A_SZ, tid);
      la.load(ra[s2], (kt + 2 + PF) * BK);
      lb.load(rb[s2], (kt + 2 + PF) * BK);
#pragma unroll
      for (int ks = 0; ks < KSTEPS; ++ks) {
        const int cur = ks & 1;
        if (ks + 1 < KSTEPS) read_frags(cur ^ 1, st0, ks + 1);
        else read_frags(cur ^ 1, st1, 0);
        if (ALT && (ks & 1)) {
          acc_alt = __builtin_amdgcn_mfma_f32_32x32x16_bf16(fa[cur][0], fb[cur][0], acc_alt, 0, 0, 0);
        } else {
#pragma unroll
          for (int a = 0; a < FM; ++a)
#pragma unroll
            for (int b = 0; b < FN; ++b)
              acc[a][b] = __builtin_amdgcn_mfma_f32_32x32x16_bf16(fa[cur][a], fb[cur][b], acc[a][b], 0, 0, 0);
        }
      }
      __syncthreads();
      bf16_t* t = st0; st0 = st1; st1 = st2; st2 = t;
    }
  }
  if constexpr (ALT) {
#pragma unroll
    for (int r = 0; r < 16; ++r) acc[0][0][r] += acc_alt[r];
  }
  epilogue<EPI, 2, 2, FM, FN>(p, acc, tiles_m, tm, m0, n0, wm, wn, i, h, reinterpret_cast<float*>(smem));
}

template <int EPI_NT, int EPI_TN, int WN>
__global__ void __launch_bounds__(WN == 2 ? 256 : 512)
gemm_bf16x3_dual_kernel(GemmArgsB p1, GemmArgsB p2, int tiles_m1, int tiles_n1, int group1, int tiles_m2, int tiles_n2, int group2,
                        int tn_first, int per) {
  extern __shared__ __attribute__((aligned(16))) char smem[];
  const int n1 = tiles_m1 * tiles_n1, n2 = tiles_m2 * tiles_n2;
  const int b = blockIdx.x;
  constexpr bool LIST = WN != 0;
  constexpr int WNN = WN ? WN : 2, FNN = WN ? 4 / WN : 2, LD = WN ? 0 : 4;
  const int n_long = tn_first ? n2 : n1;
  if (b < n_long) {
    if (tn_first) dma_tile<false, false, EPI_TN, 2, WNN, 2, FNN, 3, 32, 0, 3, 1, LD, false, true>(p2, tiles_m2, tiles_n2, group2, b, smem);
    else dma_tile<true, true, EPI_NT, 2, WNN, 2, FNN, 3, 32, 0, 3, 1, LD, false, true>(p1, tiles_m1, tiles_n1, group1, b, smem);
    return;
  }
  int seq0 = 0, count = 1;
  if constexpr (LIST) {
    x3::dual_block_tiles(tn_first ? n1 : n2, per, b - n_long, seq0, count);
    if (count == 0) return;
  }
  if (tn_first)
    dma_tile<true, true, EPI_NT, 2, WNN, 2, FNN, 3, 32, 0, 3, 1, LD, LIST, true>(p1, tiles_m1, tiles_n1, group1, b - n_long, smem, seq0,
                                                                                 count);
  else
    dma_tile<false, false, EPI_TN, 2, WNN, 2, FNN, 3, 32, 0, 3, 1, LD, LIST, true>(p2, tiles_m2, tiles_n2, group2, b - n_long, smem, seq0,
                                                                                  count);
}

struct CfgB {
  int bm, bn;
};
const CfgB kCfgB[kNumGemmBf16Configs] = {{64, 64}, {128, 64}, {128, 128}, {128, 64}, {128, 128}, {256, 128}, {128, 64}, {256, 128},
                                         {256, 256}};
int g_forced_b = -2;
int g_group_rows = 0;

template <class Kern>
int launch_grid(Kern kern, const GemmArgsB& p, int bm, int bn, int threads, size_t lds, hipStream_t stream, bool* attr_done,
                int blocks_per_tile = 1) {
  const int tiles_m = (p.M + bm - 1) / bm, tiles_n = (p.N + bn - 1) / bn;
  if (!*attr_done) {
    hipError_t e = hipFuncSetAttribute(reinterpret_cast<const void*>(kern), hipFuncAttributeMaxDynamicSharedMemorySize,
                                       160 * 1024);
    if (e != hipSuccess) return (int)e;
    *attr_done = true;
  }
  int group_rows = g_group_rows;
  if (group_rows <= 0) {
    const double per_xcd = (double)tiles_m * tiles_n / NUM_XCD;
    group_rows = (int)(sqrt(per_xcd * bn / bm) + 0.5);
  }
  if (group_rows < 1) group_rows = 1;
  if (group_rows > tiles_m) group_rows = tiles_m;
  hipLaunchKernelGGL(kern, dim3(tiles_m * tiles_n * blocks_per_tile), dim3(threads), lds, stream, p, tiles_m, tiles_n, group_rows);
  return (int)hipGetLastError();
}

template <bool A_KC, bool B_KC, int EPI, int FM, int FN>
int launch_reg(const GemmArgsB& p, hipStream_t stream) {
  constexpr int BM = 64 * FM, BN = 64 * FN;
  const size_t lds = (size_t)3 * (Operand<A_KC, BM>::SZ + Operand<B_KC, BN>::SZ) * sizeof(bf16_t);
  static bool attr_done = false;
  return launch_grid(&gemm_bf16_kernel<A_KC, B_KC, EPI, FM, FN>, p, BM, BN, NT, lds, stream, &attr_done);
}
template <bool A_KC, bool B_KC, int EPI, int WAVES_M, int WAVES_N, int FM, int FN, int NS, int BKT = 64, int SCHED = 0,
          int NPL = 1, int KSPLIT = 1, int LOADERS = 0>
int launch_dma(const GemmArgsB& p, hipStream_t stream) {
  constexpr int BM = WAVES_M * FM * 32, BN = WAVES_N * FN * 32;
  const size_t lds = (size_t)NS * NPL * (BM + BN) * BKT * 2;
  static_assert((size_t)NS * NPL * (BM + BN) * BKT * 2 <= 160 * 1024, "LDS");
  static bool attr_done = false;
  return launch_grid(&gemm_bf16_dma_kernel<A_KC, B_KC, EPI, WAVES_M, WAVES_N, FM, FN, NS, BKT, SCHED, NPL, KSPLIT, LOADERS>, p,
                     BM, BN, (WAVES_M * WAVES_N + LOADERS) * 64, lds, stream, &attr_done, KSPLIT);
}

int g_x3_cfg = -2;
int x3_cfg() {
  if (g_x3_cfg == -2) {
    const char* q = getenv("TFK_BF16X3_CFG");
    g_x3_cfg = q ? atoi(q) : -1;
  }
  return g_x3_cfg;
}
bool x3_split_shape(bool tn, int M, int N, int K) {
  const long tiles = (long)((M + 127) / 128) * ((N + 127) / 128);
  return !tn && tiles >= 64 && tiles < 200 && tiles % NUM_XCD == 0 && 2 * tiles <= kSplitXccWord && K >= 512;
}
bool x3_split_shape_tn(int M, int N, int K) {
  const long m128 = (M + 127) / 128, tiles128 = m128 * ((N + 127) / 128), tiles64 = m128 * ((N + 63) / 64);
  return tiles128 < 100 && tiles64 >= 64 && tiles64 < 200 && tiles64 % NUM_XCD == 0 && 2 * tiles64 <= kSplitXccWord && K >= 512;
}
int x3_waves() {
  static const int w = [] {
    const char* q = getenv("TFK_BF16X3_WAVES");
    const int v = q ? atoi(q) : 8;
    return v == 4 || v == 44 ? v : 8;
  }();
  return w;
}
int x3_handover_local() {
  static const int v = [] {
    const char* q = getenv("TFK_X3_HANDOVER");
    return (q && !strcmp(q, "l2")) ? 1 : 0;
  }();
  return v;
}
int x3_kskew() {
  static const int v = [] {
    const char* q = getenv("TFK_X3_KSKEW");
// ... 77 lines not shown
    if (e != hipSuccess) return (int)e;
    attr_done = true;
  }
  const int tma = (a.M + BMA - 1) / BMA, tna = (a.N + BNA - 1) / BNA, tmw = (w.M + BMW - 1) / BMW, tnw = (w.N + BNW - 1) / BNW;
  hipLaunchKernelGGL(kern, dim3(tma * tna + tmw * tnw), dim3(GWM * GWN * 64), lds, stream, a, w, tma, tna,
                     pick_group_rows(tma, tna, BMA, BNA), tmw, tnw, pick_group_rows(tmw, tnw, BMW, BNW));
  return (int)hipGetLastError();
}

template <int GWM, int GWN, int GFM, int GFN, int GNS, int HWM, int HWN, int HFM, int HFN, int HNS, int HBK>
int launch_dual_epi(const GemmArgsB& a, const GemmArgsB& w, hipStream_t stream) {
  const int key = (a.epi == EPI_DACT ? 2 : 0) + (w.epi == EPI_ACCUM ? 1 : 0);
  switch (key) {
    case 0: return launch_dual<0, 0, GWM, GWN, GFM, GFN, GNS, HWM, HWN, HFM, HFN, HNS, HBK>(a, w, stream);
    case 1: return launch_dual<0, EPI_ACCUM, GWM, GWN, GFM, GFN, GNS, HWM, HWN, HFM, HFN, HNS, HBK>(a, w, stream);
    case 2: return launch_dual<EPI_DACT, 0, GWM, GWN, GFM, GFN, GNS, HWM, HWN, HFM, HFN, HNS, HBK>(a, w, stream);
    default: return launch_dual<EPI_DACT, EPI_ACCUM, GWM, GWN, GFM, GFN, GNS, HWM, HWN, HFM, HFN, HNS, HBK>(a, w, stream);
  }
}

int g_dual_cfg = -2;

}

int gemm_bf16_dual_config(int M_nt, int N_nt, int M_tn, int N_tn) {
  if (g_dual_cfg == -2) {
    const char* q = getenv("TFK_BF16_DUAL_CFG");
    g_dual_cfg = q ? atoi(q) : -1;
  }
  if (g_dual_cfg == 0) return 0;
  if (g_dual_cfg == 3 || g_dual_cfg == 4 || g_dual_cfg == 5 || g_dual_cfg == 8) return g_dual_cfg;
  auto tiles = [](int M, int N, int bm, int bn) { return (long)((M + bm - 1) / bm) * ((N + bn - 1) / bn); };
  if (tiles(M_nt, N_nt, 256, 128) >= 200 && tiles(M_tn, N_tn, 256, 256) >= 200) return 8;
  if (tiles(M_nt, N_nt, 256, 128) + tiles(M_tn, N_tn, 256, 128) >= 512) return 5;
  if (tiles(M_nt, N_nt, 128, 128) + tiles(M_tn, N_tn, 128, 128) >= 256) return 4;
  if (tiles(M_nt, N_nt, 128, 64) + tiles(M_tn, N_tn, 128, 64) >= 256) return 3;
  return 0;
}
int gemm_bf16_dual_tile_rows(int cfg) { return (cfg == 5 || cfg == 8) ? 256 : (cfg == 3 || cfg == 4) ? 128 : 0; }

int gemm_bf16_dual(const GemmArgsB& nt, const GemmArgsB& tn, hipStream_t stream) {
  if (nt.M <= 0 || nt.N <= 0 || nt.K <= 0 || tn.M <= 0 || tn.N <= 0 || tn.K <= 0) return (int)hipErrorInvalidValue;
  if ((nt.lda & 7) || (nt.ldb & 7) || (nt.ldc & 3) || (tn.lda & 7) || (tn.ldb & 7) || (tn.ldc & 3)) return (int)hipErrorInvalidValue;
  if ((long)nt.M * nt.lda * 2 >= (1L << 31) || (long)nt.N * nt.ldb * 2 >= (1L << 31) ||
      (long)tn.K * tn.lda * 2 >= (1L << 31) || (long)tn.K * tn.ldb * 2 >= (1L << 31)) return (int)hipErrorInvalidValue;
  if ((nt.epi != 0 && nt.epi != EPI_DACT) || (tn.epi != 0 && tn.epi != EPI_ACCUM)) return -1;
  switch (gemm_bf16_dual_config(nt.M, nt.N, tn.M, tn.N)) {
    case 3: return launch_dual_epi<2, 2, 2, 1, 5, 2, 2, 2, 1, 5, 64>(nt, tn, stream);
    case 4: return launch_dual_epi<2, 2, 2, 2, 4, 2, 2, 2, 2, 4, 64>(nt, tn, stream);
    case 5: return launch_dual_epi<4, 2, 2, 2, 3, 4, 2, 2, 2, 3, 64>(nt, tn, stream);
    case 8: return launch_dual_epi<4, 2, 2, 2, 3, 4, 2, 2, 4, 4, 32>(nt, tn, stream);
  }
  return -1;
}

void gemm_bf16_force_config(int cfg) { g_forced_b = (cfg >= 0 && cfg < kNumGemmBf16Configs) ? cfg : -1; }

int gemm_bf16_pick_config(int M, int N) {
  if (g_forced_b == -2) {
    const char* q = getenv("TFK_BF16_CFG");
    const int v = q ? atoi(q) : -1;
    g_forced_b = (v >= 0 && v < kNumGemmBf16Configs) ? v : -1;
    if ((q = getenv("TFK_BF16_GROUP_ROWS"))) g_group_rows = atoi(q);
  }
  if (g_forced_b >= 0) return g_forced_b;
  const long m256 = (M + 255) / 256, m128 = (M + 127) / 128, n128 = (N + 127) / 128, n64 = (N + 63) / 64;
  if (m256 * n128 >= 200) return 5;
  if (m128 * n128 >= 200) return 4;
  return m128 * n64 > 256 ? 6 : 3;
}

int gemm_bf16_tile_rows(int M, int N) { return kCfgB[gemm_bf16_pick_config(M, N)].bm; }

size_t gemm_bf16x3_splitk_floats(GemmLayout layout, int M, int N, int K) {
  const int forced = x3_cfg();
  if (!(forced == 2 || forced < 0)) return 0;
  if (layout == GEMM_TN)
    return x3_split_shape_tn(M, N, K) ? (size_t)kSplitFlagWords + (size_t)((M + 127) / 128) * ((N + 63) / 64) * 128 * 64 : 0;
  if (!x3_split_shape(false, M, N, K)) return 0;
  return (size_t)kSplitFlagWords + (size_t)((M + 127) / 128) * ((N + 127) / 128) * 128 * 128;
}

namespace {
template <int EPI_NT, int EPI_TN, int WN>
int launch_x3_dual(const GemmArgsB& a, const GemmArgsB& w, hipStream_t stream) {
  constexpr size_t lds = (size_t)3 * 3 * (128 + 128) * 32 * 2 + 2 * 2 * 128 * sizeof(float);
  auto kern = &gemm_bf16x3_dual_kernel<EPI_NT, EPI_TN, WN>;
  static bool attr_done = false;
  if (!attr_done) {
    hipError_t e = hipFuncSetAttribute(reinterpret_cast<const void*>(kern), hipFuncAttributeMaxDynamicSharedMemorySize, 160 * 1024);
    if (e != hipSuccess) return (int)e;
    attr_done = true;
  }
  const int tma = (a.M + 127) / 128, tna = (a.N + 127) / 128, tmw = (w.M + 127) / 128, tnw = (w.N + 127) / 128;
  const int tn_first = w.K > a.K ? 1 : 0;
  const int n_long = tn_first ? tmw * tnw : tma * tna, n_short = tn_first ? tma * tna : tmw * tnw;
  const int nk_long = ((tn_first ? w.K : a.K) + 31) / 32, nk_short = ((tn_first ? a.K : w.K) + 31) / 32;
  const int per = WN == 0 ? 1 : x3::dual_tiles_per_block(n_long, nk_long, n_short, nk_short);
  const int blocks = n_long + (WN == 0 ? n_short : x3::dual_short_blocks(n_short, per));
  hipLaunchKernelGGL(kern, dim3(blocks), dim3(WN == 2 ? 256 : 512), lds, stream, a, w, tma, tna, pick_group_rows(tma, tna, 128, 128), tmw, tnw,
                     pick_group_rows(tmw, tnw, 128, 128), tn_first, per);
  return (int)hipGetLastError();
}
bool x3_operands_ok(const GemmArgsB& p, long a_rows, long b_rows) {
  if (p.M <= 0 || p.N <= 0 || p.K <= 0 || (p.lda & 31) || (p.ldb & 31) || (p.ldc & 3)) return false;
  return (long)x3::elems(a_rows, p.lda) * 2 < (1L << 31) && (long)x3::elems(b_rows, p.ldb) * 2 < (1L << 31);
}
}

int gemm_bf16x3_dual(const GemmArgsB& nt, const GemmArgsB& tn, hipStream_t stream) {
  if (!x3_operands_ok(nt, nt.M, nt.N) || !x3_operands_ok(tn, tn.K, tn.K)) return (int)hipErrorInvalidValue;
  if ((nt.epi != 0 && nt.epi != EPI_DACT) || (tn.epi != 0 && tn.epi != EPI_ACCUM)) return -1;
  static const bool on = !getenv("TFK_BF16X3_DUAL") || atoi(getenv("TFK_BF16X3_DUAL")) != 0;
  const long tiles = (long)((nt.M + 127) / 128) * ((nt.N + 127) / 128) + (long)((tn.M + 127) / 128) * ((tn.N + 127) / 128);
  if (!on || tiles < 256) return -1;
  if ((long)nt.M * nt.ldc * 4 >= (1L << 31) || (long)tn.M * tn.ldc * 4 >= (1L << 31)) return -1;
  const int key = (nt.epi == EPI_DACT ? 2 : 0) + (tn.epi == EPI_ACCUM ? 1 : 0);
  switch (key) {
#define TFK_X3_DUAL(E1, E2)                                                                \
  (x3_waves() == 8    ? launch_x3_dual<E1, E2, 4>(nt, tn, stream)                            \
   : x3_waves() == 44 ? launch_x3_dual<E1, E2, 0>(nt, tn, stream)                            \
                      : launch_x3_dual<E1, E2, 2>(nt, tn, stream))
    case 0: return TFK_X3_DUAL(0, 0);
    case 1: return TFK_X3_DUAL(0, EPI_ACCUM);
    case 2: return TFK_X3_DUAL(EPI_DACT, 0);
    default: return TFK_X3_DUAL(EPI_DACT, EPI_ACCUM);
#undef TFK_X3_DUAL
  }
}

int gemm_bf16x3(GemmLayout layout, const GemmArgsB& p, hipStream_t stream) {
  if (p.M <= 0 || p.N <= 0 || p.K <= 0) return (int)hipErrorInvalidValue;
  if (!x3_operands_ok(p, layout == GEMM_TN ? p.K : p.M, layout == GEMM_NT ? p.N : p.K)) return (int)hipErrorInvalidValue;
  switch (layout) {
    case GEMM_NN:
      switch (p.epi) {
        case 0: return launch_x3<true, false, 0>(p, stream);
        case EPI_BIAS: return launch_x3<true, false, EPI_BIAS>(p, stream);
        case EPI_BIAS | EPI_COLSTATS: return launch_x3<true, false, EPI_BIAS | EPI_COLSTATS>(p, stream);
        case EPI_BIAS | EPI_EVAL_ACT: return launch_x3<true, false, EPI_BIAS | EPI_EVAL_ACT>(p, stream);
      }
      break;
    case GEMM_NT:
      if (p.epi == 0) return launch_x3<true, true, 0>(p, stream);
      if (p.epi == EPI_DACT) return launch_x3<true, true, EPI_DACT>(p, stream);
      break;
    case GEMM_TN:
      if (p.epi == 0) return launch_x3<false, false, 0>(p, stream);
      if (p.epi == EPI_ACCUM) return launch_x3<false, false, EPI_ACCUM>(p, stream);
      break;
  }
  return (int)hipErrorInvalidValue;
}

int gemm_bf16(GemmLayout layout, const GemmArgsB& p, hipStream_t stream) {
  if (p.M <= 0 || p.N <= 0 || p.K <= 0) return (int)hipErrorInvalidValue;
  if ((p.lda & 7) || (p.ldb & 7) || (p.ldc & 3)) return (int)hipErrorInvalidValue;
  {
    const long a_rows = layout == GEMM_TN ? p.K : p.M;
    const long b_rows = layout == GEMM_NT ? p.N : p.K;
    if (a_rows * p.lda * 2 >= (1L << 31) || b_rows * p.ldb * 2 >= (1L << 31)) return (int)hipErrorInvalidValue;
  }
  switch (layout) {
    case GEMM_NN:
      switch (p.epi) {
        case 0: return launch<true, false, 0>(p, stream);
        case EPI_BIAS: return launch<true, false, EPI_BIAS>(p, stream);
        case EPI_BIAS | EPI_COLSTATS: return launch<true, false, EPI_BIAS | EPI_COLSTATS>(p, stream);
        case EPI_BIAS | EPI_EVAL_ACT: return launch<true, false, EPI_BIAS | EPI_EVAL_ACT>(p, stream);
      }
      break;
    case GEMM_NT:
      if (p.epi == 0) return launch<true, true, 0>(p, stream);
      if (p.epi == EPI_DACT) return launch<true, true, EPI_DACT>(p, stream);
      break;
    case GEMM_TN:
      if (p.epi == 0) return launch<false, false, 0>(p, stream);
      if (p.epi == EPI_ACCUM) return launch<false, false, EPI_ACCUM>(p, stream);
      break;
  }
  return (int)hipErrorInvalidValue;
}

}
```

### tfkaldi_amd/csrc/kernels.hip

```cpp
#include "kernels.h"

#include <math.h>
#include <stdlib.h>

namespace tfk {
namespace {

constexpr int NONLIN_RELU = 0, NONLIN_SIGMOID = 1, NONLIN_TANH = 2, NONLIN_LINEAR = 3;

__device__ __forceinline__ float wave_sum(float v) {
#pragma unroll
  for (int o = 32; o > 0; o >>= 1) v += __shfl_xor(v, o);
  return v;
}
__device__ __forceinline__ float wave_max(float v) {
#pragma unroll
  for (int o = 32; o > 0; o >>= 1) v = fmaxf(v, __shfl_xor(v, o));
  return v;
}
__device__ __forceinline__ float block_sum(float v, float* sm) {
  v = wave_sum(v);
  const int w = threadIdx.x >> 6, nw = blockDim.x >> 6;
  if ((threadIdx.x & 63) == 0) sm[w] = v;
  __syncthreads();
  float t = 0.f;
  for (int k = 0; k < nw; ++k) t += sm[k];
  __syncthreads();
  return t;
}
__device__ __forceinline__ float block_max(float v, float* sm) {
  v = wave_max(v);
  const int w = threadIdx.x >> 6, nw = blockDim.x >> 6;
  if ((threadIdx.x & 63) == 0) sm[w] = v;
  __syncthreads();
  float t = sm[0];
  for (int k = 1; k < nw; ++k) t = fmaxf(t, sm[k]);
  __syncthreads();
  return t;
}

__device__ __forceinline__ uint4 philox4x32(uint4 c, uint2 k) {
#pragma unroll
  for (int r = 0; r < 7; ++r) {
    const uint32_t hi0 = __umulhi(0xD2511F53u, c.x), lo0 = 0xD2511F53u * c.x;
    const uint32_t hi1 = __umulhi(0xCD9E8D57u, c.z), lo1 = 0xCD9E8D57u * c.z;
    c = make_uint4(hi1 ^ c.y ^ k.x, lo1, hi0 ^ c.w ^ k.y, lo0);
    k.x += 0x9E3779B9u;
    k.y += 0xBB67AE85u;
  }
  return c;
}
struct Keep4 { bool k[4]; };
__device__ __forceinline__ Keep4 keep_mask(const ActDesc& d, int row, int c4) {
  const uint4 r = philox4x32(make_uint4((uint32_t)c4, (uint32_t)row, d.layer, d.call),
                             make_uint2((uint32_t)d.seed, (uint32_t)(d.seed >> 32)));
  const uint32_t thr = (uint32_t)fminf((1.0f - d.keep) * 4294967296.0f, 4294967295.0f);
  Keep4 m;
  m.k[0] = r.x >= thr; m.k[1] = r.y >= thr; m.k[2] = r.z >= thr; m.k[3] = r.w >= thr;
  return m;
}

__device__ __forceinline__ float nonlin_fwd(float u, int nonlin) {
  switch (nonlin) {
    case NONLIN_RELU: return fmaxf(u, 0.f);
    case NONLIN_SIGMOID: return 1.f / (1.f + expf(-u));
    case NONLIN_TANH: return tanhf(u);
    default: return u;
  }
}
__device__ __forceinline__ float nonlin_bwd(float v, int nonlin) {
  switch (nonlin) {
    case NONLIN_RELU: return v > 0.f ? 1.f : 0.f;
    case NONLIN_SIGMOID: return v * (1.f - v);
    case NONLIN_TANH: return 1.f - v * v;
    default: return 1.f;
  }
}

__device__ __forceinline__ float4 ld4(const float* p) { return *reinterpret_cast<const float4*>(p); }
typedef uint16_t u16x4 __attribute__((ext_vector_type(4)));
__device__ __forceinline__ uint16_t to_bf16(float x) { return __builtin_bit_cast(uint16_t, (__bf16)x); }
__device__ __forceinline__ void st4_twin(const Twin& t, size_t row, int col, float4 v) {
  if (!t.p) return;
  if (t.x3) {
    uint16_t a[4], b[4], c[4];
    twin_split3(v.x, a[0], b[0], c[0]); twin_split3(v.y, a[1], b[1], c[1]);
    twin_split3(v.z, a[2], b[2], c[2]); twin_split3(v.w, a[3], b[3], c[3]);
    u16x4 q1, q2, q3;
    q1.x = a[0]; q1.y = a[1]; q1.z = a[2]; q1.w = a[3];
    q2.x = b[0]; q2.y = b[1]; q2.z = b[2]; q2.w = b[3];
    q3.x = c[0]; q3.y = c[1]; q3.z = c[2]; q3.w = c[3];
    uint16_t* d = t.p + x3::at(row, col, t.ld);
    *reinterpret_cast<u16x4*>(d) = q1;
    *reinterpret_cast<u16x4*>(d + 64) = q2;
    *reinterpret_cast<u16x4*>(d + 128) = q3;
    return;
  }
  u16x4 q;
  q.x = to_bf16(v.x); q.y = to_bf16(v.y); q.z = to_bf16(v.z); q.w = to_bf16(v.w);
  *reinterpret_cast<u16x4*>(t.p + row * t.ld + col) = q;
}
__device__ __forceinline__ void st4(float* p, float4 v) { *reinterpret_cast<float4*>(p) = v; }
typedef float v4f_nt __attribute__((ext_vector_type(4)));
__device__ __forceinline__ void st4_nt(float* p, float4 v) {
  v4f_nt q;
  q.x = v.x; q.y = v.y; q.z = v.z; q.w = v.w;
  __builtin_nontemporal_store(q, reinterpret_cast<v4f_nt*>(p));
}
__device__ __forceinline__ void st4_twin_nt(const Twin& t, size_t row, int col, float4 v) {
  if (!t.p) return;
  if (t.x3) {
    uint16_t a[4], b[4], c[4];
    twin_split3(v.x, a[0], b[0], c[0]); twin_split3(v.y, a[1], b[1], c[1]);
    twin_split3(v.z, a[2], b[2], c[2]); twin_split3(v.w, a[3], b[3], c[3]);
    u16x4 q1, q2, q3;
    q1.x = a[0]; q1.y = a[1]; q1.z = a[2]; q1.w = a[3];
    q2.x = b[0]; q2.y = b[1]; q2.z = b[2]; q2.w = b[3];
    q3.x = c[0]; q3.y = c[1]; q3.z = c[2]; q3.w = c[3];
    uint16_t* d = t.p + x3::at(row, col, t.ld);
    __builtin_nontemporal_store(q1, reinterpret_cast<u16x4*>(d));
    __builtin_nontemporal_store(q2, reinterpret_cast<u16x4*>(d + 64));
    __builtin_nontemporal_store(q3, reinterpret_cast<u16x4*>(d + 128));
    return;
  }
  u16x4 q;
  q.x = to_bf16(v.x); q.y = to_bf16(v.y); q.z = to_bf16(v.z); q.w = to_bf16(v.w);
  __builtin_nontemporal_store(q, reinterpret_cast<u16x4*>(t.p + row * t.ld + col));
}
__device__ __forceinline__ float4 ld4s(const float* p, int nt) {
  if (nt & 4) {
    const v4f_nt q = __builtin_nontemporal_load(reinterpret_cast<const v4f_nt*>(p));
    return make_float4(q.x, q.y, q.z, q.w);
  }
  return *reinterpret_cast<const float4*>(p);
}
int bn_nt_mode(const Twin& tw, int rows, int ld) {
  static const int forced = [] { const char* q = getenv("TFK_BN_NT"); return q ? atoi(q) : -1; }();
  if (forced >= 0) return forced;
  const size_t twin_bytes = tw.p ? (size_t)rows * ld * (tw.x3 ? 6 : 2) : 0;
  return 1 | (twin_bytes >= ((size_t)8 << 20) ? 2 : 0);
}
__device__ __forceinline__ float& el(float4& v, int i) { return reinterpret_cast<float*>(&v)[i]; }
__device__ __forceinline__ float el(const float4& v, int i) { return reinterpret_cast<const float*>(&v)[i]; }

constexpr int CT_X = 32, CT_Y = 8;
constexpr int RB = 4;

struct ColTile {
  int c4;
  int col;
  bool valid;
  int r0, r1;
};
__device__ __forceinline__ ColTile col_tile(int T, int ld, int rows_per) {
  ColTile t;
  t.c4 = blockIdx.x * CT_X + threadIdx.x;
  t.col = t.c4 * 4;
  t.valid = t.col < ld;
  t.r0 = blockIdx.y * rows_per;
  t.r1 = min(T, t.r0 + rows_per);
  return t;
}
__device__ __forceinline__ float4 reduce_rows(float4 v, float4 (*sm)[CT_X]) {
  sm[threadIdx.y][threadIdx.x] = v;
  __syncthreads();
  float4 t = make_float4(0.f, 0.f, 0.f, 0.f);
  if (threadIdx.y == 0) {
#pragma unroll
    for (int k = 0; k < CT_Y; ++k) {
      const float4 q = sm[k][threadIdx.x];
      t.x += q.x; t.y += q.y; t.z += q.z; t.w += q.w;
    }
  }
  __syncthreads();
  return t;
}

__global__ void __launch_bounds__(CT_X * CT_Y)
bn_stats_partial_kernel(const float* __restrict__ z, int T, int ld, int rows_per, int rs, float* __restrict__ ws) {
  __shared__ float4 sm[CT_Y][CT_X];
  __shared__ float4 sm_mean[CT_X];
  const ColTile t = col_tile(T, ld, rows_per);
  const float4 zero4 = make_float4(0.f, 0.f, 0.f, 0.f);
  float4 s = zero4;
  float4 keep[RB];
#pragma unroll
  for (int j = 0; j < RB; ++j) keep[j] = zero4;
  if (t.valid) {
    const int rfirst = t.r0 + threadIdx.y;
#pragma unroll
    for (int j = 0; j < RB; ++j) {
      const int r = rfirst + j * CT_Y;
      if (r < t.r1) keep[j] = ld4(z + (size_t)r * ld + t.col);
    }
#pragma unroll
    for (int j = 0; j < RB; ++j) { s.x += keep[j].x; s.y += keep[j].y; s.z += keep[j].z; s.w += keep[j].w; }
    for (int r = rfirst + RB * CT_Y; r < t.r1; r += CT_Y) {
      const float4 v = ld4(z + (size_t)r * ld + t.col);
      s.x += v.x; s.y += v.y; s.z += v.z; s.w += v.w;
    }
  }
  s = reduce_rows(s, sm);
  const int n = max(t.r1 - t.r0, 0);
  if (threadIdx.y == 0) {
    const float inv = n > 0 ? 1.f / (float)n : 0.f;
    sm_mean[threadIdx.x] = make_float4(s.x * inv, s.y * inv, s.z * inv, s.w * inv);
  }
  __syncthreads();
  const float4 mu = sm_mean[threadIdx.x];
  float4 q = zero4;
  if (t.valid) {
    const int rfirst = t.r0 + threadIdx.y;
#pragma unroll
    for (int j = 0; j < RB; ++j) {
      if (rfirst + j * CT_Y < t.r1) {
        const float dx = keep[j].x - mu.x, dy = keep[j].y - mu.y, dz = keep[j].z - mu.z, dw = keep[j].w - mu.w;
        q.x += dx * dx; q.y += dy * dy; q.z += dz * dz; q.w += dw * dw;
      }
    }
    for (int r = rfirst + RB * CT_Y; r < t.r1; r += CT_Y) {
      const float4 v = ld4(z + (size_t)r * ld + t.col);
      const float dx = v.x - mu.x, dy = v.y - mu.y, dz = v.z - mu.z, dw = v.w - mu.w;
      q.x += dx * dx; q.y += dy * dy; q.z += dz * dz; q.w += dw * dw;
    }
  }
  q = reduce_rows(q, sm);
  if (threadIdx.y == 0 && t.valid) {
    st4(ws + ((size_t)0 * rs + blockIdx.y) * ld + t.col, mu);
    st4(ws + ((size_t)1 * rs + blockIdx.y) * ld + t.col, q);
  }
// ... 211 lines not shown
  const float4 rsd = smm[threadIdx.x];
  const bool drop = d.train && d.keep < 1.f;
  const float inv_keep = drop ? 1.f / d.keep : 1.f;
  for (int rb = rb0; rb < t.r1; rb += CT_Y * RB) {
    float4 zn[RB];
    const int rbn = rb + CT_Y * RB;
#pragma unroll
    for (int j = 0; j < RB; ++j) {
      const int r = rbn + j * CT_Y;
      zn[j] = rbn < t.r1 ? ld4s(z + (size_t)(r < t.r1 ? r : rbn) * ld + t.col, nt) : zero4;
    }
#pragma unroll
    for (int j = 0; j < RB; ++j) {
      const int r = rb + j * CT_Y;
      if (r >= t.r1) continue;
      float4 v;
      v.x = (zv[j].x - mu.x) * rsd.x + be.x; v.y = (zv[j].y - mu.y) * rsd.y + be.y;
      v.z = (zv[j].z - mu.z) * rsd.z + be.z; v.w = (zv[j].w - mu.w) * rsd.w + be.w;
#pragma unroll
      for (int k = 0; k < 4; ++k) el(v, k) = (t.col + k < H) ? nonlin_fwd(el(v, k), d.nonlin) : 0.f;
      if (drop) {
        const Keep4 m = keep_mask(d, r, t.c4);
#pragma unroll
        for (int k = 0; k < 4; ++k) el(v, k) = m.k[k] ? el(v, k) * inv_keep : 0.f;
      }
      if (nt & 1) st4_nt(a + (size_t)r * ld + t.col, v);
      else st4(a + (size_t)r * ld + t.col, v);
      if (nt & 2) st4_twin_nt(tw, r, t.col, v);
      else st4_twin(tw, r, t.col, v);
    }
#pragma unroll
    for (int j = 0; j < RB; ++j) zv[j] = zn[j];
  }
}

__global__ void __launch_bounds__(256)
act_backward_rows_kernel(ActDesc d, float* __restrict__ da, const float* __restrict__ vbuf,
                         const float* __restrict__ rowscale, int T, int H, int ld) {
  __shared__ float sm[4];
  const int nc4 = ld >> 2;
  const bool drop = d.keep < 1.f;
  const float inv_keep = drop ? 1.f / d.keep : 1.f;
  for (int row = blockIdx.x; row < T; row += gridDim.x) {
    float* gr = da + (size_t)row * ld;
    const float* vr = vbuf + (size_t)row * ld;
    const float s = rowscale[row];
    float dot = 0.f;
    if (s > 1.f) {
      for (int c4 = threadIdx.x; c4 < nc4; c4 += blockDim.x) {
        const int col = c4 << 2;
        float4 g = ld4(gr + col);
        const float4 v = ld4(vr + col);
        if (drop) {
          const Keep4 m = keep_mask(d, row, c4);
#pragma unroll
          for (int k = 0; k < 4; ++k) el(g, k) = m.k[k] ? el(g, k) * inv_keep : 0.f;
        }
        dot += g.x * v.x + g.y * v.y + g.z * v.z + g.w * v.w;
      }
      dot = block_sum(dot, sm);
    }
    const float k1 = s > 1.f ? 1.f / s : 1.f;
    const float k2 = s > 1.f ? 2.f * dot / ((float)H * s * s) : 0.f;
    for (int c4 = threadIdx.x; c4 < nc4; c4 += blockDim.x) {
      const int col = c4 << 2;
      float4 g = ld4(gr + col);
      const float4 v = ld4(vr + col);
      if (drop) {
        const Keep4 m = keep_mask(d, row, c4);
#pragma unroll
        for (int k = 0; k < 4; ++k) el(g, k) = m.k[k] ? el(g, k) * inv_keep : 0.f;
      }
      float4 o;
#pragma unroll
      for (int k = 0; k < 4; ++k) {
        const float dv = el(g, k) * k1 - el(v, k) * k2;
        el(o, k) = (col + k < H) ? dv * nonlin_bwd(el(v, k), d.nonlin) : 0.f;
      }
      st4(gr + col, o);
    }
  }
}

__device__ __forceinline__ float4 compute_du(const ActDesc& d, int pre_du, float4 g, float4 a, int row, int c4) {
  if (pre_du) return g;
  float4 o;
  if (d.keep < 1.f) {
    const Keep4 m = keep_mask(d, row, c4);
    const float inv_keep = 1.f / d.keep;
#pragma unroll
    for (int k = 0; k < 4; ++k)
      el(o, k) = m.k[k] ? el(g, k) * inv_keep * nonlin_bwd(el(a, k) * d.keep, d.nonlin) : 0.f;
  } else {
#pragma unroll
    for (int k = 0; k < 4; ++k) el(o, k) = el(g, k) * nonlin_bwd(el(a, k), d.nonlin);
  }
  return o;
}

__global__ void __launch_bounds__(CT_X * CT_Y)
hb_stats_kernel(ActDesc d, int pre_du, const float* __restrict__ da, const float* __restrict__ a,
                const float* __restrict__ z, const float* __restrict__ mean, const float* __restrict__ rstd, int T,
                int ld, int rows_per, int rs, float* __restrict__ ws) {
  __shared__ float4 sm[CT_Y][CT_X];
  const ColTile t = col_tile(T, ld, rows_per);
  float4 s1 = make_float4(0.f, 0.f, 0.f, 0.f), s2 = s1;
  if (t.valid) {
    const float4 mu = ld4(mean + t.col), rsd = ld4(rstd + t.col);
    for (int rb = t.r0 + threadIdx.y; rb < t.r1; rb += CT_Y * RB) {
      float4 g[RB], av[RB], zv[RB];
#pragma unroll
      for (int j = 0; j < RB; ++j) {
        const int r = rb + j * CT_Y;
        const size_t off = (size_t)(r < t.r1 ? r : rb) * ld + t.col;
        g[j] = ld4(da + off);
        av[j] = pre_du ? g[j] : ld4(a + off);
        zv[j] = ld4(z + off);
      }
#pragma unroll
      for (int j = 0; j < RB; ++j) {
        const int r = rb + j * CT_Y;
        if (r >= t.r1) continue;
        const float4 du = compute_du(d, pre_du, g[j], av[j], r, t.c4);
        s1.x += du.x; s1.y += du.y; s1.z += du.z; s1.w += du.w;
        s2.x += du.x * (zv[j].x - mu.x) * rsd.x; s2.y += du.y * (zv[j].y - mu.y) * rsd.y;
        s2.z += du.z * (zv[j].z - mu.z) * rsd.z; s2.w += du.w * (zv[j].w - mu.w) * rsd.w;
      }
    }
  }
  s1 = reduce_rows(s1, sm);
  s2 = reduce_rows(s2, sm);
  if (threadIdx.y == 0 && t.valid) {
    st4(ws + ((size_t)0 * kMaxRowSplits + blockIdx.y) * ld + t.col, s1);
    st4(ws + ((size_t)1 * kMaxRowSplits + blockIdx.y) * ld + t.col, s2);
  }
}

__global__ void __launch_bounds__(CT_X * CT_Y)
hb_apply_kernel(ActDesc d, int pre_du, float* __restrict__ da, const float* __restrict__ a,
                const float* __restrict__ z, const float* __restrict__ mean, const float* __restrict__ rstd, int T,
                int H, int ld, int rows_per, int rs_in, float* __restrict__ ws, Twin tw, int T_apply,
                float* __restrict__ ws_dz, int nt) {
  __shared__ float4 sm[CT_Y][CT_X];
  const ColTile t = col_tile(T_apply, ld, rows_per);
  float4 sz = make_float4(0.f, 0.f, 0.f, 0.f);
  const float4 zero4 = sz;
  float4 m1 = sz, m2 = sz;
  const int rb0 = t.r0 + threadIdx.y;
  float4 g[RB], av[RB], zv[RB];
#pragma unroll
  for (int j = 0; j < RB; ++j) {
    const int r = rb0 + j * CT_Y;
    const bool ok = t.valid && rb0 < t.r1;
    const size_t off = (size_t)(r < t.r1 ? r : rb0) * ld + t.col;
    g[j] = ok ? ld4s(da + off, nt) : zero4;
    av[j] = (ok && !pre_du) ? ld4s(a + off, nt) : g[j];
    zv[j] = (ok && d.bn) ? ld4s(z + off, nt) : g[j];
  }
  float4 mu = sz, rsd = sz;
  if (d.bn && t.valid) {
    mu = ld4(mean + t.col); rsd = ld4(rstd + t.col);
  }
  if (d.bn) {
    float4 p1 = sz, p2 = sz;
    if (t.valid)
      for (int k = threadIdx.y; k < rs_in; k += CT_Y) {
        const float4 q1 = ld4(ws + ((size_t)0 * kMaxRowSplits + k) * ld + t.col);
        const float4 q2 = ld4(ws + ((size_t)1 * kMaxRowSplits + k) * ld + t.col);
        p1.x += q1.x; p1.y += q1.y; p1.z += q1.z; p1.w += q1.w;
        p2.x += q2.x; p2.y += q2.y; p2.z += q2.z; p2.w += q2.w;
      }
    __shared__ float4 smm[2][CT_X];
    p1 = reduce_rows(p1, sm);
    p2 = reduce_rows(p2, sm);
    if (threadIdx.y == 0) {
      const float invT = 1.f / (float)T;
      smm[0][threadIdx.x] = make_float4(p1.x * invT, p1.y * invT, p1.z * invT, p1.w * invT);
      smm[1][threadIdx.x] = make_float4(p2.x * invT, p2.y * invT, p2.z * invT, p2.w * invT);
    }
    __syncthreads();
    m1 = smm[0][threadIdx.x];
    m2 = smm[1][threadIdx.x];
  }
  if (t.valid) {
    for (int rb = rb0; rb < t.r1; rb += CT_Y * RB) {
      float4 gn[RB], an[RB], zn[RB];
      const int rbn = rb + CT_Y * RB;
#pragma unroll
      for (int j = 0; j < RB; ++j) {
        const int r = rbn + j * CT_Y;
        const bool ok = rbn < t.r1;
        const size_t off = (size_t)(r < t.r1 ? r : rbn) * ld + t.col;
        gn[j] = ok ? ld4s(da + off, nt) : zero4;
        an[j] = (ok && !pre_du) ? ld4s(a + off, nt) : gn[j];
        zn[j] = (ok && d.bn) ? ld4s(z + off, nt) : gn[j];
      }
#pragma unroll
      for (int j = 0; j < RB; ++j) {
        const int r = rb + j * CT_Y;
        if (r >= t.r1) continue;
        float4 dz = compute_du(d, pre_du, g[j], av[j], r, t.c4);
        if (d.bn) {
          dz.x = rsd.x * (dz.x - m1.x - (zv[j].x - mu.x) * rsd.x * m2.x);
          dz.y = rsd.y * (dz.y - m1.y - (zv[j].y - mu.y) * rsd.y * m2.y);
          dz.z = rsd.z * (dz.z - m1.z - (zv[j].z - mu.z) * rsd.z * m2.z);
          dz.w = rsd.w * (dz.w - m1.w - (zv[j].w - mu.w) * rsd.w * m2.w);
        }
        if (r >= T) dz = zero4;
#pragma unroll
        for (int k = 0; k < 4; ++k)
          if (t.col + k >= H) el(dz, k) = 0.f;
        if (tw.p) {
          if (nt & 2) st4_twin_nt(tw, r, t.col, dz);
          else st4_twin(tw, r, t.col, dz);
        } else {
          st4(da + (size_t)r * ld + t.col, dz);
        }
        sz.x += dz.x; sz.y += dz.y; sz.z += dz.z; sz.w += dz.w;
      }
#pragma unroll
      for (int j = 0; j < RB; ++j) {
        g[j] = gn[j]; av[j] = an[j]; zv[j] = zn[j];
      }
    }
  }
  sz = reduce_rows(sz, sm);
  if (threadIdx.y == 0 && t.valid) st4(ws_dz + (size_t)blockIdx.y * ld + t.col, sz);
}

__global__ void __launch_bounds__(FIN_COLS * FIN_KL) grad_final_kernel(FinalBatch b) {
  __shared__ float sm[FIN_KL][FIN_COLS];
  const FinalItem it = b.it[blockIdx.y];
  const int c = blockIdx.x * FIN_COLS + threadIdx.x;
  const int ky = threadIdx.y;
  float v[FIN_PER];
#pragma unroll
  for (int j = 0; j < FIN_PER; ++j) {
    const int k = ky + j * FIN_KL;
    v[j] = (c < it.N && k < it.rs) ? it.ws[((size_t)it.which * kMaxRowSplits + k) * it.ld + c] : 0.f;
  }
  float s = 0.f;
#pragma unroll
  for (int j = 0; j < FIN_PER; ++j) s += v[j];
  sm[ky][threadIdx.x] = s;
  __syncthreads();
  if (ky != 0 || c >= it.N) return;
  s = 0.f;
#pragma unroll
  for (int k = 0; k < FIN_KL; ++k) s += sm[k][threadIdx.x];
  it.g[c] = b.accumulate ? it.g[c] + s : s;
}

__global__ void __launch_bounds__(FIN_COLS * FIN_KL) chunk_totals_kernel(float* __restrict__ ws, int chunks, int ld) {
  __shared__ float sm[FIN_KL][FIN_COLS];
  const int c = blockIdx.x * FIN_COLS + threadIdx.x;
  const int ky = threadIdx.y;
  float* slab = ws + (size_t)blockIdx.y * kMaxRowSplits * ld;
  float v[FIN_PER];
#pragma unroll
  for (int j = 0; j < FIN_PER; ++j) {
    const int k = ky + j * FIN_KL;
    v[j] = (c < ld && k < chunks) ? slab[(size_t)k * ld + c] : 0.f;
  }
  float s = 0.f;
#pragma unroll
  for (int j = 0; j < FIN_PER; ++j) s += v[j];
  sm[ky][threadIdx.x] = s;
  __syncthreads();
  if (ky != 0 || c >= ld) return;
  s = 0.f;
#pragma unroll
  for (int k = 0; k < FIN_KL; ++k) s += sm[k][threadIdx.x];
  slab[c] = s;
}

__global__ void __launch_bounds__(CT_X * CT_Y)
colsum_partial_kernel(const float* __restrict__ x, int T, int ld, int rows_per, int rs, float* __restrict__ ws) {
  __shared__ float4 sm[CT_Y][CT_X];
  const ColTile t = col_tile(T, ld, rows_per);
  float4 s = make_float4(0.f, 0.f, 0.f, 0.f);
  if (t.valid)
    for (int r = t.r0 + threadIdx.y; r < t.r1; r += CT_Y) {
      const float4 v = ld4(x + (size_t)r * ld + t.col);
      s.x += v.x; s.y += v.y; s.z += v.z; s.w += v.w;
    }
  s = reduce_rows(s, sm);
  if (threadIdx.y == 0 && t.valid) st4(ws + (size_t)blockIdx.y * ld + t.col, s);
}

__device__ __forceinline__ float loss_sum_256(const float* __restrict__ row_loss, int T, int tid, float* sm4) {
  float s = 0.f;
  for (int i = tid; i < T; i += 256) s += row_loss[i];
#pragma unroll
  for (int off = 32; off > 0; off >>= 1) s += __shfl_down(s, off, 64);
  if ((tid & 63) == 0) sm4[tid >> 6] = s;
  __syncthreads();
  return ((sm4[0] + sm4[1]) + sm4[2]) + sm4[3];
}
__device__ __forceinline__ void loss_commit(float s, float* __restrict__ scalars, int overwrite, float frames, float microbatches) {
  scalars[0] = overwrite ? s : scalars[0] + s;
  scalars[1] = overwrite ? frames : scalars[1] + frames;
  scalars[2] = overwrite ? microbatches : scalars[2] + microbatches;
}
__global__ void __launch_bounds__(CT_X * CT_Y)
colsum_loss_kernel(const float* __restrict__ x, int T, int ld, int rows_per, int rs, float* __restrict__ ws,
                   const float* __restrict__ row_loss, int T_loss, float* __restrict__ scalars, int overwrite, float frames,
                   float microbatches) {
  __shared__ float4 sm[CT_Y][CT_X];
  if ((int)blockIdx.y == rs) {
    if (blockIdx.x != 0) return;
// ... 348 lines not shown
      }
    }
    el(o, k) = v;
  }
  const int trow = out_seg ? out_seg[lo] + (t - first) : t;
  st4(out + (size_t)trow * ldo + (c4 << 2), o);
}

__global__ void __launch_bounds__(256)
checksum_kernel(const uint32_t* __restrict__ p, size_t n, unsigned long long* __restrict__ out) {
  unsigned long long acc = 0;
  const size_t stride = (size_t)gridDim.x * blockDim.x;
  for (size_t i = (size_t)blockIdx.x * blockDim.x + threadIdx.x; i < n; i += stride)
    acc += (unsigned long long)p[i] * (unsigned long long)((i & 0xffffu) + 1u);
#pragma unroll
  for (int o = 32; o > 0; o >>= 1) acc += __shfl_xor(acc, o);
  if ((threadIdx.x & 63) == 0) atomicAdd(out, acc);
}

inline dim3 ct_grid(int ld, int rs) { return dim3((ld / 4 + CT_X - 1) / CT_X, rs); }
inline dim3 ct_block() { return dim3(CT_X, CT_Y); }

}

int row_splits(int T) {
  static const int rows = [] { const char* q = getenv("TFK_CT_ROWS"); const int v = q ? atoi(q) : 32; return v >= 8 ? v : 32; }();
  int rs = (T + rows - 1) / rows;
  if (rs < 1) rs = 1;
  if (rs > kMaxRowSplits) rs = kMaxRowSplits;
  return rs;
}

int row_splits_fwd(int T) {
  static const int rows = [] { const char* q = getenv("TFK_CT_ROWS_FWD"); const int v = q ? atoi(q) : 16; return v >= 8 ? v : 16; }();
  if (getenv("TFK_CT_ROWS") && !getenv("TFK_CT_ROWS_FWD")) return row_splits(T);
  int rs = (T + rows - 1) / rows;
  if (rs < 1) rs = 1;
  if (rs > kMaxRowSplits) rs = kMaxRowSplits;
  return rs;
}

void bn_stats_train(hipStream_t s, const float* z, int T, int H, int ld, float eps, float decay, float* mean,
                    float* rstd, float* e_mean, float* e_var, float* ws) {
  const int rs = row_splits(T), rows_per = (T + rs - 1) / rs;
  hipLaunchKernelGGL(bn_stats_partial_kernel, ct_grid(ld, rs), ct_block(), 0, s, z, T, ld, rows_per, rs, ws);
  hipLaunchKernelGGL(bn_stats_final_kernel, dim3((ld + FIN_COLS - 1) / FIN_COLS), dim3(FIN_COLS, FIN_KL), 0, s, ws, T, H, ld, rows_per, rs, eps,
                     decay, mean, rstd, e_mean, e_var);
}

void bn_stats_eval(hipStream_t s, const float* mov_mean, const float* mov_var, int H, float eps, float* mean,
                   float* rstd) {
  hipLaunchKernelGGL(bn_stats_eval_kernel, dim3((H + 255) / 256), dim3(256), 0, s, mov_mean, mov_var, H, eps, mean,
                     rstd);
}

void bn_act_forward(hipStream_t s, const ActDesc& d, const float* z, float* a, const float* stats, int chunk_rows,
                    int T, int H, int ld, float eps, float decay, float* mean, float* rstd, float* e_mean,
                    float* e_var, const float* beta, Twin tw, int T_apply, int slab_chunks) {
  if (T_apply < T) T_apply = T;
  const int rs = row_splits_fwd(T_apply), rows_per = (T_apply + rs - 1) / rs;
  const int nchunk = (T + chunk_rows - 1) / chunk_rows;
  hipLaunchKernelGGL(bn_act_forward_kernel, ct_grid(ld, rs), ct_block(), 0, s, d, z, a, stats, nchunk, chunk_rows, T, H,
                     ld, rows_per, eps, decay, mean, rstd, e_mean, e_var, beta, tw, T_apply,
                     slab_chunks > 0 ? slab_chunks : nchunk, bn_nt_mode(tw, T_apply, ld));
}

void act_forward(hipStream_t s, const ActDesc& d, const float* z, float* a, float* v, float* rowscale,
                 const float* mean, const float* rstd, const float* beta, int T, int H, int ld, Twin tw) {
  const int grid = T < 4096 ? T : 4096;
  if (d.l2)
    hipLaunchKernelGGL(act_forward_kernel<true>, dim3(grid), dim3(256), 0, s, d, z, a, v, rowscale, mean, rstd, beta,
                       T, H, ld, tw);
  else
    hipLaunchKernelGGL(act_forward_kernel<false>, dim3(grid), dim3(256), 0, s, d, z, a, v, rowscale, mean, rstd, beta,
                       T, H, ld, tw);
}

void act_backward_rows(hipStream_t s, const ActDesc& d, float* da, const float* v, const float* rowscale, int T,
                       int H, int ld) {
  const int grid = T < 4096 ? T : 4096;
  hipLaunchKernelGGL(act_backward_rows_kernel, dim3(grid), dim3(256), 0, s, d, da, v, rowscale, T, H, ld);
}

void hidden_backward(hipStream_t s, const ActDesc& d, int pre_du, float* da, const float* a, const float* z,
                     const float* mean, const float* rstd, int T, int H, int ld, float* ws, int stats_chunks,
                     Twin tw, int T_apply, float* ws_dz) {
  if (T_apply < T) T_apply = T;
  const int rs = row_splits(T_apply), rows_per = (T_apply + rs - 1) / rs;
  if (d.bn && stats_chunks <= 0)
    hipLaunchKernelGGL(hb_stats_kernel, ct_grid(ld, rs), ct_block(), 0, s, d, pre_du, da, a, z, mean, rstd, T, ld,
                       rows_per, rs, ws);
  hipLaunchKernelGGL(hb_apply_kernel, ct_grid(ld, rs), ct_block(), 0, s, d, pre_du, da, a, z, mean, rstd, T, H, ld,
                     rows_per, stats_chunks > 0 ? stats_chunks : rs, ws, tw, T_apply,
                     ws_dz ? ws_dz : ws + (size_t)2 * kMaxRowSplits * ld, bn_nt_mode(tw, T_apply, ld));
}

void bn_stats_from_chunks(hipStream_t s, const float* stats, int chunk_rows, int T, int H, int ld, float eps, float decay,
                          float* mean, float* rstd, float* e_mean, float* e_var) {
  const int nchunk = (T + chunk_rows - 1) / chunk_rows;
  hipLaunchKernelGGL(bn_stats_final_kernel, dim3((ld + FIN_COLS - 1) / FIN_COLS), dim3(FIN_COLS, FIN_KL), 0, s, stats, T, H,
                     ld, chunk_rows, nchunk, eps, decay, mean, rstd, e_mean, e_var);
}

void chunk_totals(hipStream_t s, float* ws, int chunks, int ld) {
  hipLaunchKernelGGL(chunk_totals_kernel, dim3((ld + FIN_COLS - 1) / FIN_COLS, 2), dim3(FIN_COLS, FIN_KL), 0, s, ws, chunks,
                     ld);
}

void colsum_partial(hipStream_t s, const float* x, int T, int ld, float* ws) {
  const int rs = row_splits(T), rows_per = (T + rs - 1) / rs;
  hipLaunchKernelGGL(colsum_partial_kernel, ct_grid(ld, rs), ct_block(), 0, s, x, T, ld, rows_per, rs, ws);
}

void grad_final(hipStream_t s, const FinalBatch& b) {
  if (b.n <= 0) return;
  int maxn = 0;
  for (int i = 0; i < b.n; ++i) maxn = b.it[i].N > maxn ? b.it[i].N : maxn;
  hipLaunchKernelGGL(grad_final_kernel, dim3((maxn + FIN_COLS - 1) / FIN_COLS, b.n), dim3(FIN_COLS, FIN_KL), 0, s, b);
}

void softmax_xent(hipStream_t s, float* logits, const int32_t* y, int T, int O, int ld, float* row_loss,
                  int with_grad, Twin tw) {
  const int nc4 = ld / 4;
  const dim3 g(T), b(256);
#define TFK_SMX(NV) hipLaunchKernelGGL(softmax_xent_kernel<NV>, g, b, 0, s, logits, y, O, ld, row_loss, with_grad, tw)
  if (nc4 <= 256) TFK_SMX(1);
  else if (nc4 <= 512) TFK_SMX(2);
  else if (nc4 <= 1024) TFK_SMX(4);
  else if (nc4 <= 2048) TFK_SMX(8);
  else TFK_SMX(0);
#undef TFK_SMX
}

void loss_reduce(hipStream_t s, const float* row_loss, int T, float* scalars, bool overwrite, int frames, int microbatches) {
  hipLaunchKernelGGL(loss_reduce_kernel, dim3(1), dim3(256), 0, s, row_loss, T, scalars, overwrite ? 1 : 0,
                     (float)(frames >= 0 ? frames : T), (float)microbatches);
}

void colsum_loss(hipStream_t s, const float* x, int T, int ld, float* ws, const float* row_loss, int T_loss, float* scalars,
                 bool overwrite, int frames, int microbatches) {
  const int rs = row_splits(T), rows_per = (T + rs - 1) / rs;
  const dim3 g = ct_grid(ld, rs);
  hipLaunchKernelGGL(colsum_loss_kernel, dim3(g.x, rs + 1), ct_block(), 0, s, x, T, ld, rows_per, rs, ws, row_loss, T_loss,
                     scalars, overwrite ? 1 : 0, (float)(frames >= 0 ? frames : T_loss), (float)microbatches);
}

void softmax_rows(hipStream_t s, const float* logits, int T, int O, int ld, float* out, int64_t ldo,
                  const float* prior) {
  const int nc4 = ld / 4;
  const int vec = ((ldo & 3) == 0 && (((uintptr_t)out) & 15) == 0) ? 1 : 0;
  const dim3 g(T), b(256);
  if (nc4 <= 256) hipLaunchKernelGGL(softmax_rows_kernel<1>, g, b, 0, s, logits, O, ld, out, ldo, prior, vec);
  else if (nc4 <= 512) hipLaunchKernelGGL(softmax_rows_kernel<2>, g, b, 0, s, logits, O, ld, out, ldo, prior, vec);
  else if (nc4 <= 1024) hipLaunchKernelGGL(softmax_rows_kernel<4>, g, b, 0, s, logits, O, ld, out, ldo, prior, vec);
  else if (nc4 <= 2048) hipLaunchKernelGGL(softmax_rows_kernel<8>, g, b, 0, s, logits, O, ld, out, ldo, prior, vec);
  else hipLaunchKernelGGL(softmax_rows_kernel<0>, g, b, 0, s, logits, O, ld, out, ldo, prior, vec);
}

void adam_apply(hipStream_t s, float* w, float* g, float* m, float* v, size_t n, const float* scalars, float lr_t,
                float beta1, float beta2, float eps, int grid_cap, uint16_t* wb, size_t n_wb, const ShadowMap* map,
                size_t first) {
  ShadowMap sm;
  if (map) sm = *map;
  else sm.n = 0;
  const size_t n4 = n / 4;
  static const int un_div = [] { const char* q = getenv("TFK_ADAM_UNROLL"); const int u = q ? atoi(q) : 2; return u == 4 ? 4 : u == 2 ? 2 : 1; }();
  size_t blocks = ((n4 + un_div - 1) / un_div + 255) / 256;
  static const size_t max_blocks = [] { const char* q = getenv("TFK_ADAM_GRID"); return (size_t)(q ? atoi(q) : (1 << 22)); }();
  if (blocks > max_blocks) blocks = max_blocks;
  if (grid_cap > 0 && blocks > (size_t)grid_cap) blocks = grid_cap;
  if (blocks == 0) return;
  static const int forced = [] { const char* q = getenv("TFK_ADAM_NT"); return q ? atoi(q) : -1; }();
  const int nt = forced >= 0 ? forced : ((wb && sm.n == 0) ? 2 : 1);
  static const int un = [] { const char* q = getenv("TFK_ADAM_UNROLL"); return q ? atoi(q) : 2; }();
#define TFK_ADAM_LAUNCH(NTV, UNV)                                                                                  \
  hipLaunchKernelGGL((adam_kernel<NTV, UNV>), dim3((unsigned)blocks), dim3(256), 0, s, w, g, m, v, n4, scalars, lr_t, \
                     beta1, beta2, eps, wb, n_wb / 4, sm, first)
// ... 52 lines not shown
```

### tfkaldi_amd/csrc/x3_layout.h

```cpp
#pragma once
#include <stddef.h>
#include <stdint.h>

#if defined(__HIPCC__)
#define X3_HD __host__ __device__ __forceinline__
#else
#define X3_HD inline
#endif

namespace tfk {
namespace x3 {

constexpr int kSlotK = 32;

#ifndef TFK_X3_M16
#define TFK_X3_M16 0
#endif

X3_HD size_t elems(size_t rows, int ld) { return ((rows + 1) >> 1) * (size_t)(ld >> 5) * 192; }
X3_HD size_t at(size_t row, int col, int ld) {
  return ((row >> 1) * (size_t)(ld >> 5) + (size_t)(col >> 5)) * 192 + (row & 1) * 32 + (col & 31);
}

#if TFK_X3_M16
// ... 10 lines not shown
X3_HD int kc_addr(int r, int q, int c) { return (r >> 1) * 384 + q * 128 + (r & 1) * 64 + ((c ^ kc_swz(r)) << 4); }

template <int EXT>
X3_HD void ks_decode(int n, int& r, int& b, int& q, int& e8) {
  constexpr int CPP = EXT / 32 * 24;
  const int P = n / CPP, pos = n - P * CPP;
  const int nq = (pos >> 2) ^ ((P & 1) << 1);
  b = nq / 6;
  const int rem = nq - 6 * b;
  q = rem >> 1;
  r = 2 * P + (rem & 1);
#if TFK_X3_M16
  e8 = (pos & 3) ^ (((P >> 2) & 1) << 1);
#else
  e8 = pos & 3;
#endif
}
template <int EXT>
X3_HD int ks_addr(int r, int b, int q, int e8) {
  const int P = r >> 1;
#if TFK_X3_M16
  e8 ^= ((P >> 2) & 1) << 1;
#endif
  return P * (EXT / 32 * 384) + ((((6 * b + 2 * q + (r & 1)) ^ ((P & 1) << 1)) << 2) + e8) * 16;
}

X3_HD int kc_lane_off(int lane, int frag0, int ks) { return kc_addr(frag0 * 32 + (lane & 31), 0, 2 * ks + (lane >> 5)); }
X3_HD int kc_imm(int f, int q) { return f * (16 * 384) + q * 128; }
template <int EXT>
X3_HD int ks_lane_off(int lane, int frag0, int x_odd) {
  const int kb = lane >> 5, half = (lane >> 4) & 1, j = (lane >> 2) & 3, qq = lane & 3;
  const int t = (j >> 1) & 1;
  const int base = (4 * kb + (j >> 1)) * (EXT / 32 * 384) + (j & 1) * 64 + (2 * half + (qq >> 1)) * 16 + ((qq & 1) << 3) +
                   128 * 3 * frag0;
  const int xt_odd = (frag0 + x_odd) & 1;
  return base + (xt_odd ? -128 * t : 128 * t) + (x_odd ? 128 : 0);
}
template <int EXT>
X3_HD int ks_imm(int X, int ks, int hi) {
  return 128 * (X & ~1) + (ks * 8 + hi * 2) * (EXT / 32 * 384);
}

X3_HD int kc16_lane_off(int lane, int frag0) { return kc_addr(frag0 * 16 + (lane & 15), 0, lane >> 4); }
X3_HD int kc16_imm(int f, int q) { return f * (8 * 384) + q * 128; }
template <int EXT>
X3_HD int ks16_lane_off(int lane, int frag0, int x_odd, int f_odd) {
  const int g = lane >> 4, j = (lane >> 2) & 3, qq = lane & 3;
  const int t = (j >> 1) & 1;
  const int unit0 = frag0 >> 1;
  const int base = (4 * g + (j >> 1)) * (EXT / 32 * 384) + (j & 1) * 64 + ((f_odd ^ (g & 1)) << 5) + (qq >> 1) * 16 + ((qq & 1) << 3) +
                   128 * 3 * unit0;
  const int xt_odd = (unit0 + x_odd) & 1;
  return base + (xt_odd ? -128 * t : 128 * t) + (x_odd ? 128 : 0);
}
template <int EXT>
X3_HD int ks16_imm(int X, int hi) {
  return 128 * (X & ~1) + hi * 2 * (EXT / 32 * 384);
}

constexpr int kXcds = 8;
constexpr int kCus = 256;
X3_HD int dual_tiles_per_block(int n_long, int nk_long, int n_short, int nk_short) {
  int per = (nk_long + (nk_short - 1) / 2) / nk_short;
  if (per < 1) per = 1;
  while (per > 1 && n_long + (n_short + per - 1) / per < kCus) --per;
  return per;
}
X3_HD void dual_block_tiles(int n_short, int per, int g, int& seq0, int& count) {
  const int xcd = g % kXcds, j = g / kXcds;
  const int q = n_short / kXcds, r = n_short % kXcds;
  const int start = xcd < r ? xcd * (q + 1) : r * (q + 1) + (xcd - r) * q;
  const int cnt = q + (xcd < r ? 1 : 0);
  const int left = cnt - j * per;
  seq0 = start + j * per;
  count = left <= 0 ? 0 : left < per ? left : per;
}
X3_HD int dual_short_blocks(int n_short, int per) {
  const int q = n_short / kXcds, r = n_short % kXcds;
  if (q == 0) return r;
  const int j_q = (q + per - 1) / per, j_q1 = (q + 1 + per - 1) / per;
  return (r > 0 && j_q1 > j_q) ? kXcds * j_q + r : kXcds * j_q;
}

#if defined(__HIPCC__)
__device__ __forceinline__ void split3(float x, uint16_t& p1, uint16_t& p2, uint16_t& p3) {
  const uint32_t ux = __builtin_bit_cast(uint32_t, x);
  uint32_t b1 = (uint32_t)__builtin_bit_cast(uint16_t, (__bf16)x) << 16;
  const bool edge = (b1 & 0x7fffffffu) == 0x7f800000u && (ux & 0x7fffffffu) < 0x7f800000u;
  if (edge) b1 = ux & 0xffff0000u;
  const float r1 = x - __builtin_bit_cast(float, b1);
  uint32_t b2 = (uint32_t)__builtin_bit_cast(uint16_t, (__bf16)r1) << 16;
  if (edge) b2 = __builtin_bit_cast(uint32_t, r1) & 0xffff0000u;
  const float r2 = r1 - __builtin_bit_cast(float, b2);
  p1 = (uint16_t)(b1 >> 16);
  p2 = (uint16_t)(b2 >> 16);
  p3 = (uint16_t)(__builtin_bit_cast(uint32_t, r2) >> 16);
}
#endif

}
}
```

Baseline: 960,500.

## Fuse hidden-layer backward apply as a tail of the dual x3 GEMM kernel

Moves the hidden-backward apply step into the end of the fp32-emulating dual GEMM launch. Blocks of the dz half count completions with an atomic counter, and once all are done every block pulls work items from a ticket counter and runs the shared hb_apply body. The dz results and stats are written with system-coherent buffer stores so other blocks can see them. The aim is to drop a separate kernel launch and fill idle CUs at the tail of the GEMM. The cost is spin polling, counter reset logic and a deadlock risk if the blocks are not all resident at once.

```diff
diff --git a/tfkaldi_amd/build.py b/tfkaldi_amd/build.py
--- a/tfkaldi_amd/build.py
+++ b/tfkaldi_amd/build.py
@@ -9,7 +9,7 @@
 LIBDIR = os.path.join(HERE, "lib")
 LIBNAME = "libtfkaldi_hip.so"
 SOURCES = ["gemm_f32.hip", "gemm_bf16.hip", "kernels.hip", "ctc.hip", "engine.hip", "features.hip", "exchange.hip"]
-HEADERS = ["gemm_f32.h", "gemm_bf16.h", "kernels.h", "ctc.h", "x3_layout.h", os.path.join("..", "..", "include", "tfkaldi_hip.h")]
+HEADERS = ["gemm_f32.h", "gemm_bf16.h", "kernels.h", "hb_apply.h", "ctc.h", "x3_layout.h", os.path.join("..", "..", "include", "tfkaldi_hip.h")]
 FLAGS = ["--offload-arch=gfx950", "-O3", "-std=c++17", "-fPIC", "-Wno-unused-value"]
 
 
diff --git a/tfkaldi_amd/csrc/engine.hip b/tfkaldi_amd/csrc/engine.hip
--- a/tfkaldi_amd/csrc/engine.hip
+++ b/tfkaldi_amd/csrc/engine.hip
@@ -117,6 +117,7 @@
   float* ws_bwd = nullptr;
   float* ws_splitk = nullptr;
   size_t ws_splitk_floats = 0;
+  float* hb_tail_ctr = nullptr;
   size_t ws_bwd_stride = 0;
   float* prior = nullptr;
   bool have_prior = false;
@@ -448,7 +449,8 @@
 
 int run_gemm_dual(tfk_engine* e, const float* dz, int ld_dz, const float* W, int ldw, float* da_out, int ld_da, int T,
                   int N_da, int K_da, const ActEpi* act, float* stats, const float* in, int ld_in, float* Gw, int ld_g,
-                  int d_in, int d_out, int epi_w, int* chunk_rows) {
+                  int d_in, int d_out, int epi_w, int* chunk_rows, const HbTailArgs* tail = nullptr, int* tail_ran = nullptr) {
+  if (tail_ran) *tail_ran = 0;
   if (!e->dual_gemm) return 1;
   const double flops = 2.0 * T * N_da * K_da + 2.0 * d_in * d_out * T;
   const double out_w = (double)d_in * d_out * ((epi_w & EPI_ACCUM) ? 2 : 1);
@@ -471,7 +473,7 @@
     const double ob = e->x3 ? 6.0 : 2.0;
     ProfScope ps(e, KF_GEMM_DUAL, flops, ob * ((double)T * K_da + (double)K_da * N_da) + 4.0 * (double)T * N_da +
                                              ob * ((double)T * d_in + (double)T * d_out) + 4.0 * out_w);
-    const int rc = e->x3 ? gemm_bf16x3_dual(a, w, e->stream) : gemm_bf16_dual(a, w, e->stream);
+    const int rc = e->x3 ? gemm_bf16x3_dual(a, w, e->stream, tail, tail_ran) : gemm_bf16_dual(a, w, e->stream);
     if (rc != 0) ps.drop();
     if (rc == -1) return 1;
     if (rc != 0) return fail(rc, "gemm_bf16%s_dual launch failed: %s", e->x3 ? "x3" : "", hipGetErrorString((hipError_t)rc));
@@ -910,11 +912,24 @@
     return run_gemm(e, GEMM_NT, dz, ld_dz, W, ldw, out, ldH, T, H, K, nullptr, EPI_DACT, nullptr, ws_of(target), cfg, &act);
   };
   int bm_in = rows_o;
+  HbTailArgs tail_args;
+  auto tail_of = [&](int target, int slot) -> const HbTailArgs* {
+    if (st || !fuse_hb || !e->x3 || !e->hb_tail_ctr || (T + kGemmBf16x3TileRows - 1) / kGemmBf16x3TileRows > kMergeOnceChunks)
+      return nullptr;
+    Twin tw;
+    tw.p = e->dAb[slot]; tw.ld = e->ldHb; tw.x3 = e->x3;
+    tail_args = HbTailArgs();
+    tail_args.hb = hidden_backward_args(act_desc(e, target, 1, call), 1, e->dA[slot], e->a[target], e->z[target], mean[target],
+                                        rstd[target], T, H, ldH, ws_of(target), (T + kGemmBf16x3TileRows - 1) / kGemmBf16x3TileRows, tw);
+    tail_args.ctr = reinterpret_cast<unsigned*>(e->hb_tail_ctr);
+    return &tail_args;
+  };
+  int hb_done = 0;
   {
     const ActEpi act = act_of(nact - 1);
     const int rc = run_gemm_dual(e, e->logits, e->ldO, e->p_param() + o.w_off, o.ld_out, e->dA[pp], ldH, T, H, e->O,
                                  fuse_hb ? &act : nullptr, fuse_hb ? ws_of(nact - 1) : nullptr, e->a[nact - 1], ldH,
-                                 G + o.w_off, o.ld_out, H, e->O, epi_w, &bm_in);
+                                 G + o.w_off, o.ld_out, H, e->O, epi_w, &bm_in, tail_of(nact - 1, pp), &hb_done);
     if (rc < 0) return rc;
     if (rc > 0) {
       CHK(run_gemm(e, GEMM_TN, e->a[nact - 1], ldH, e->logits, e->ldO, G + o.w_off, o.ld_out, H, e->O, T, nullptr, epi_w));
@@ -964,24 +979,27 @@
         act_backward_rows(e->stream, d, da, e->v[l], e->rowscale[l], T, H, ldH);
         pre_du = 1;
       }
-      ProfScope ps(e, KF_HIDDEN_BWD, 0, (e->cfg.batch_norm ? 28.0 : 12.0) * T * H);
       int chunks_eff = fuse_hb ? chunks_in : 0;
-      if (chunks_eff > kMergeOnceChunks) {
-        chunk_totals(e->stream, ws_of(l), chunks_eff, ldH);
-        chunks_eff = 1;
+      if (!hb_done) {
+        ProfScope ps(e, KF_HIDDEN_BWD, 0, (e->cfg.batch_norm ? 28.0 : 12.0) * T * H);
+        if (chunks_eff > kMergeOnceChunks) {
+          chunk_totals(e->stream, ws_of(l), chunks_eff, ldH);
+          chunks_eff = 1;
+        }
+        hidden_backward(e->stream, d, pre_du, da, e->a[l], e->z[l], mean[l], rstd[l], T, H, ldH, ws_of(l), chunks_eff, tw);
       }
-      hidden_backward(e->stream, d, pre_du, da, e->a[l], e->z[l], mean[l], rstd[l], T, H, ldH, ws_of(l), chunks_eff, tw);
       fin_layer(fuse_hb ? chunks_eff : rs, rs);
     }
     const float* in = l == 0 ? Xd : e->a[l - 1];
     const int ld_in = l == 0 ? ldx : ldH;
     bool fused = false;
     bm_in = rows_h;
+    hb_done = 0;
     if (l > 0) {
       const ActEpi act = act_of(l - 1);
       const int rc = run_gemm_dual(e, da, ldH, e->p_param() + y.w_off, y.ld_out, e->dA[pp ^ 1], ldH, T, H, H,
                                    fuse_hb ? &act : nullptr, fuse_hb ? ws_of(l - 1) : nullptr, in, ld_in, G + y.w_off,
-                                   y.ld_out, y.d_in, H, epi_w, &bm_in);
+                                   y.ld_out, y.d_in, H, epi_w, &bm_in, tail_of(l - 1, pp ^ 1), &hb_done);
       if (rc < 0) return rc;
       fused = rc == 0;
     }
@@ -1006,6 +1024,8 @@
   *w = 0;
   if (e->ws_splitk)
     (void)hipMemsetAsync(e->ws_splitk, 0, e->ws_splitk_floats * sizeof(float), e->stream);
+  if (e->hb_tail_ctr)
+    (void)hipMemsetAsync(e->hb_tail_ctr, 0, kHbTailCtrWords * sizeof(unsigned), e->stream);
   return fail(-1, "split-K exchange timed out: a block of the fp32-emulating contraction waited ~1 s for its partner's partial "
                   "sums (workspace not zeroed, or the partner block failed); the results of this step are invalid");
 }
@@ -1154,6 +1174,7 @@
     if (alloc_zero(&e->mean[l], (size_t)e->ldH) || alloc_zero(&e->rstd[l], (size_t)e->ldH)) return bail(-1);
   }
   if (alloc_zero(&e->prior, (size_t)e->ldO)) return bail(-1);
+  if (e->x3 && alloc_zero(&e->hb_tail_ctr, (size_t)kHbTailCtrWords)) return bail(-1);
   if (e->bf16) {
     e->wb_aligned = e->x3 ? (e->L + 1 <= kShadowMapMax) : shadow_mirrors(cfg, e->lay);
     e->wb_off.assign(e->L + 1, 0);
@@ -1591,6 +1612,7 @@
   if (e->Wb && e->own_wb) hipFree(e->Wb);
   if (e->d_checksum) hipFree(e->d_checksum);
   if (e->ws_splitk) hipFree(e->ws_splitk);
+  if (e->hb_tail_ctr) hipFree(e->hb_tail_ctr);
   for (void* p : {(void*)e->ctc_seg, (void*)e->ctc_lab_off, (void*)e->ctc_lab, (void*)e->ctc_lp, (void*)e->ctc_ab,
                   (void*)e->ctc_utt_loss, (void*)e->ctc_lse, (void*)e->ctc_off, (void*)e->ctc_bb, (void*)e->ctc_offb,
                   (void*)e->ctc_logz, (void*)e->ctc_dec})
diff --git a/tfkaldi_amd/csrc/gemm_bf16.h b/tfkaldi_amd/csrc/gemm_bf16.h
--- a/tfkaldi_amd/csrc/gemm_bf16.h
+++ b/tfkaldi_amd/csrc/gemm_bf16.h
@@ -3,6 +3,7 @@
 #include <stdint.h>
 
 #include "gemm_f32.h"
+#include "hb_apply.h"
 
 namespace tfk {
 
@@ -49,7 +50,17 @@
 int gemm_bf16x3(GemmLayout layout, const GemmArgsB& args, hipStream_t stream);
 constexpr int kGemmBf16x3TileRows = 128;
 size_t gemm_bf16x3_splitk_floats(GemmLayout layout, int M, int N, int K);
-int gemm_bf16x3_dual(const GemmArgsB& nt, const GemmArgsB& tn, hipStream_t stream);
+struct HbTailArgs {
+  HbApplyArgs hb;
+  unsigned* ctr;
+  int n_da;
+  int n_items;
+  int polls;
+  int polls_dw;
+};
+constexpr int kHbTailCtrWords = 96;
+int gemm_bf16x3_dual(const GemmArgsB& nt, const GemmArgsB& tn, hipStream_t stream, const HbTailArgs* tail = nullptr,
+                     int* tail_ran = nullptr);
 
 int gemm_bf16_tile_rows(int M, int N);
 
diff --git a/tfkaldi_amd/csrc/gemm_bf16.hip b/tfkaldi_amd/csrc/gemm_bf16.hip
--- a/tfkaldi_amd/csrc/gemm_bf16.hip
+++ b/tfkaldi_amd/csrc/gemm_bf16.hip
@@ -1,4 +1,5 @@
 #include "gemm_bf16.h"
+#include "hb_apply.h"
 #include "x3_layout.h"
 
 #include <math.h>
@@ -39,7 +40,8 @@
 
 __device__ __forceinline__ uint16_t f2bf(float x) { return __builtin_bit_cast(uint16_t, (__bf16)x); }
 
-template <int EPI, int WAVES_M, int WAVES_N, int FM, int FN, bool CBUF = false>
+constexpr int kAuxSys = 1 | (1 << 4);
+template <int EPI, int WAVES_M, int WAVES_N, int FM, int FN, bool CBUF = false, bool WT = false>
 __device__ __forceinline__ void epilogue(const GemmArgsB& p, f32x16 (&acc)[FM][FN], int tiles_m, int tm, int m0, int n0,
                                          int wm, int wn, int i, int h, float* red) {
   constexpr int BM = WAVES_M * FM * 32, BN = WAVES_N * FN * 32;
@@ -159,12 +161,23 @@
           t1 += red[(0 * WAVES_M + w) * BN + cidx];
           t2 += red[(1 * WAVES_M + w) * BN + cidx];
         }
-        p.stats[((size_t)0 * p.stats_stride + tm) * p.ldc + col] = t1;
-        p.stats[((size_t)1 * p.stats_stride + tm) * p.ldc + col] = t2;
+        if constexpr (WT) {
+          const __amdgpu_buffer_rsrc_t srs = __builtin_amdgcn_make_buffer_rsrc(
+              (void*)p.stats, 0, (int)(2u * (unsigned)p.stats_stride * (unsigned)p.ldc * 4u), 0x00020000);
+          __builtin_amdgcn_raw_buffer_store_b32(__builtin_bit_cast(unsigned, t1), srs,
+                                                ((unsigned)(0 * p.stats_stride + tm) * p.ldc + col) * 4u, 0, kAuxSys);
+          __builtin_amdgcn_raw_buffer_store_b32(__builtin_bit_cast(unsigned, t2), srs,
+                                                ((unsigned)(1 * p.stats_stride + tm) * p.ldc + col) * 4u, 0, kAuxSys);
+        } else {
+          p.stats[((size_t)0 * p.stats_stride + tm) * p.ldc + col] = t1;
+          p.stats[((size_t)1 * p.stats_stride + tm) * p.ldc + col] = t2;
+        }
       }
       __syncthreads();
     }
     if constexpr (CBUF) {
+      static_assert(!WT || (EPI & EPI_DACT) != 0, "write-through results: the EPI_DACT half of a dual launch");
+      constexpr int c_aux = WT ? kAuxSys : 0;
       static_assert((EPI & EPI_EVAL_ACT) == 0, "no bf16 twin on this path");
       const __amdgpu_buffer_rsrc_t crs =
           __builtin_amdgcn_make_buffer_rsrc((void*)p.C, 0, (int)(((unsigned)(p.M - 1) * p.ldc + p.N) * 4u), 0x00020000);
@@ -183,7 +196,7 @@
           float v = acc[a][b][r];
           if (EPI & EPI_ACCUM) v += old[r];
           __builtin_amdgcn_raw_buffer_store_b32(__builtin_bit_cast(unsigned, v), crs,
-                                                base + (unsigned)(((r & 3) + 8 * (r >> 2)) * p.ldc) * 4u, 0, 0);
+                                                base + (unsigned)(((r & 3) + 8 * (r >> 2)) * p.ldc) * 4u, 0, c_aux);
         }
       }
       continue;
@@ -431,11 +444,12 @@
 constexpr int kSplitFlagWords = 4096;
 constexpr int kSplitXccWord = 2048;
 template <bool A_KC, bool B_KC, int EPI, int WAVES_M, int WAVES_N, int FM, int FN, int NS, int BKT = 64, int SCHED = 0,
-          int NPL = 1, int KSPLIT = 1, int LOADERS = 0, bool LIST = false, bool CBUF = false>
+          int NPL = 1, int KSPLIT = 1, int LOADERS = 0, bool LIST = false, bool CBUF = false, bool WT = false>
 __device__ __forceinline__ void dma_tile(const GemmArgsB& p, int tiles_m, int tiles_n, int group_rows, int bid, char* smem,
                                          int seq0 = 0, int ntiles = 1) {
   static_assert(LOADERS == 0 || (NPL == 3 && LOADERS == WAVES_M * WAVES_N), "loader waves: one per multiplying wave, x3 only");
   static_assert(!LIST || (NPL == 3 && KSPLIT == 1 && LOADERS == 0), "tile lists: the unsplit fp32-emulating contraction, no loader waves");
+  static_assert(!WT || (!LIST && CBUF && NPL == 3 && KSPLIT == 1), "write-through results: the one-tile blocks of a dual launch");
   constexpr int NTH = WAVES_M * WAVES_N * 64;
   constexpr int BM = WAVES_M * FM * 32, BN = WAVES_N * FN * 32;
   typedef typename std::conditional<NPL == 3, DmaOperand3<A_KC, BM, NTH>, DmaOperand<A_KC, BM, NTH, BKT>>::type OA;
@@ -904,7 +918,7 @@
       typedef float f32x4 __attribute__((ext_vector_type(4)));
       unsigned* flags = reinterpret_cast<unsigned*>(p.splitk_ws);
       const int tile = tm * tiles_n + tn;
-      constexpr int kSys = 1 | (1 << 4);
+      constexpr int kSys = kAuxSys;
       __amdgpu_buffer_rsrc_t part = __builtin_amdgcn_make_buffer_rsrc(
           (void*)(p.splitk_ws + kSplitFlagWords + (size_t)tile * (BM * BN)), 0, BM * BN * 4, 0x00020000);
       unsigned* sh = reinterpret_cast<unsigned*>(smem);
@@ -969,7 +983,7 @@
           }
       __syncthreads();
     }
-    epilogue<EPI, WAVES_M, WAVES_N, FM, FN, CBUF>(p, acc, tiles_m, tm_out, m0_out, n0_out, wm, wn, i, h, red);
+    epilogue<EPI, WAVES_M, WAVES_N, FM, FN, CBUF, WT>(p, acc, tiles_m, tm_out, m0_out, n0_out, wm, wn, i, h, red);
     TFKB_TL(3, ti);
     if constexpr (LIST) {
       primed = chain_next;
@@ -1175,15 +1189,86 @@
   epilogue<EPI, 2, 2, FM, FN>(p, acc, tiles_m, tm, m0, n0, wm, wn, i, h, reinterpret_cast<float*>(smem));
 }
 
-template <int EPI_NT, int EPI_TN, int WN>
+template <int NTH>
+__device__ __forceinline__ void hb_tail(const HbTailArgs& t, bool is_da, char* smem) {
+  using namespace hbk;
+  constexpr int NV = NTH / (CT_X * CT_Y);
+  static_assert(NV == 1 || NV == 2, "one or two virtual blocks per block");
+  constexpr int kVbBytes = (CT_Y + 2) * CT_X * (int)sizeof(float4);
+  const int tid = threadIdx.x;
+  unsigned* sh = reinterpret_cast<unsigned*>(smem);
+  const int half = tid / (CT_X * CT_Y), within = tid % (CT_X * CT_Y);
+  float4(*sm)[CT_X] = reinterpret_cast<float4(*)[CT_X]>(smem + 64 + half * kVbBytes);
+  float4(*smm)[CT_X] = sm + CT_Y;
+  unsigned* done = t.ctr;
+  unsigned* ticket = t.ctr + 32;
+  unsigned* exited = t.ctr + 64;
+  if (is_da) asm volatile("s_waitcnt vmcnt(0)" : : : "memory");
+  __syncthreads();
+  if (tid == 0) {
+    unsigned go = 0;
+    if (is_da) {
+      go = __hip_atomic_fetch_add(done, 1u, __ATOMIC_RELAXED, __HIP_MEMORY_SCOPE_AGENT) + 1u == (unsigned)t.n_da;
+      TFKB_TL(5, 0);
+    }
+    const int polls = is_da ? t.polls : t.polls_dw;
+    for (int spin = 0; !go && spin < polls; ++spin) {
+      if (spin) __builtin_amdgcn_s_sleep(8);
+      go = __hip_atomic_load(done, __ATOMIC_RELAXED, __HIP_MEMORY_SCOPE_AGENT) >= (unsigned)t.n_da;
+    }
+    sh[0] = go;
+  }
+  __syncthreads();
+  if (sh[0]) {
+    bool first = true;
+    for (;;) {
+      if (tid == 0) sh[1] = __hip_atomic_fetch_add(ticket, 1u, __ATOMIC_RELAXED, __HIP_MEMORY_SCOPE_AGENT);
+      __syncthreads();
+      const int item = (int)sh[1];
+      if (item >= t.n_items) break;
+      if (first) TFKB_TL(6, 0);
+      first = false;
+      VBlock vb;
+      vb.tx = within % CT_X;
+      vb.ty = within / CT_X;
+      vb.live = x3::hb_tail_vblock(t.hb.gx, t.hb.gy, NV, item, half, vb.bx, vb.by);
+      hb_apply_body<true>(t.hb, vb, sm, smm);
+      TFKB_TL(7, 0);
+    }
+  }
+  if (tid == 0) {
+    if (__hip_atomic_fetch_add(exited, 1u, __ATOMIC_RELAXED, __HIP_MEMORY_SCOPE_AGENT) + 1u == gridDim.x) {
+      __hip_atomic_store(done, 0u, __ATOMIC_RELAXED, __HIP_MEMORY_SCOPE_AGENT);
+      __hip_atomic_store(ticket, 0u, __ATOMIC_RELAXED, __HIP_MEMORY_SCOPE_AGENT);
+      __hip_atomic_store(exited, 0u, __ATOMIC_RELAXED, __HIP_MEMORY_SCOPE_AGENT);
+    }
+  }
+}
+
+template <int EPI_NT, int EPI_TN, int WN, bool TAIL = false>
 __global__ void __launch_bounds__(WN == 2 ? 256 : 512)
 gemm_bf16x3_dual_kernel(GemmArgsB p1, GemmArgsB p2, int tiles_m1, int tiles_n1, int group1, int tiles_m2, int tiles_n2, int group2,
-                        int tn_first, int per) {
+                        int tn_first, int per, HbTailArgs tail) {
   extern __shared__ __attribute__((aligned(16))) char smem[];
   const int n1 = tiles_m1 * tiles_n1, n2 = tiles_m2 * tiles_n2;
   const int b = blockIdx.x;
   constexpr bool LIST = WN != 0;
   constexpr int WNN = WN ? WN : 2, FNN = WN ? 4 / WN : 2, LD = WN ? 0 : 4;
+  if constexpr (TAIL) {
+    static_assert(LIST && (EPI_NT & EPI_DACT) != 0, "a tail: tile lists, behind an EPI_DACT half");
+    const bool is_da = b < n1;
+    if (is_da) {
+      dma_tile<true, true, EPI_NT, 2, WNN, 2, FNN, 3, 32, 0, 3, 1, LD, false, true, true>(p1, tiles_m1, tiles_n1, group1, b, smem);
+    } else {
+      int seq0 = 0, count = 1;
+      x3::dual_block_tiles(n2, per, b - n1, seq0, count);
+      if (count > 0)
+        dma_tile<false, false, EPI_TN, 2, WNN, 2, FNN, 3, 32, 0, 3, 1, LD, LIST, true>(p2, tiles_m2, tiles_n2, group2, b - n1, smem, seq0,
+                                                                                      count);
+    }
+    hb_tail<(WN == 2 ? 256 : 512)>(tail, is_da, smem);
+    return;
+  } else {
   const int n_long = tn_first ? n2 : n1;
   if (b < n_long) {
     if (tn_first) dma_tile<false, false, EPI_TN, 2, WNN, 2, FNN, 3, 32, 0, 3, 1, LD, false, true>(p2, tiles_m2, tiles_n2, group2, b, smem);
@@ -1201,6 +1286,7 @@
   else
     dma_tile<false, false, EPI_TN, 2, WNN, 2, FNN, 3, 32, 0, 3, 1, LD, LIST, true>(p2, tiles_m2, tiles_n2, group2, b - n_long, smem, seq0,
                                                                                   count);
+  }
 }
 
 struct CfgB {
@@ -1444,10 +1530,10 @@
 }
 
 namespace {
-template <int EPI_NT, int EPI_TN, int WN>
-int launch_x3_dual(const GemmArgsB& a, const GemmArgsB& w, hipStream_t stream) {
+template <int EPI_NT, int EPI_TN, int WN, bool TAIL = false>
+int launch_x3_dual(const GemmArgsB& a, const GemmArgsB& w, hipStream_t stream, const HbTailArgs* tail = nullptr) {
   constexpr size_t lds = (size_t)3 * 3 * (128 + 128) * 32 * 2 + 2 * 2 * 128 * sizeof(float);
-  auto kern = &gemm_bf16x3_dual_kernel<EPI_NT, EPI_TN, WN>;
+  auto kern = &gemm_bf16x3_dual_kernel<EPI_NT, EPI_TN, WN, TAIL>;
   static bool attr_done = false;
   if (!attr_done) {
     hipError_t e = hipFuncSetAttribute(reinterpret_cast<const void*>(kern), hipFuncAttributeMaxDynamicSharedMemorySize, 160 * 1024);
@@ -1460,9 +1546,22 @@
   const int nk_long = ((tn_first ? w.K : a.K) + 31) / 32, nk_short = ((tn_first ? a.K : w.K) + 31) / 32;
   const int per = WN == 0 ? 1 : x3::dual_tiles_per_block(n_long, nk_long, n_short, nk_short);
   const int blocks = n_long + (WN == 0 ? n_short : x3::dual_short_blocks(n_short, per));
+  HbTailArgs t = {};
+  if (TAIL) {
+    if (!tail || tn_first) return (int)hipErrorInvalidValue;
+    t = *tail;
+    t.n_da = n_long;
+    t.n_items = x3::hb_tail_items(t.hb.gx, t.hb.gy, WN == 2 ? 1 : 2);
+    t.polls = 64;
+    t.polls_dw = 8;
+  }
   hipLaunchKernelGGL(kern, dim3(blocks), dim3(WN == 2 ? 256 : 512), lds, stream, a, w, tma, tna, pick_group_rows(tma, tna, 128, 128), tmw, tnw,
-                     pick_group_rows(tmw, tnw, 128, 128), tn_first, per);
+                     pick_group_rows(tmw, tnw, 128, 128), tn_first, per, t);
   return (int)hipGetLastError();
+}
+bool hb_tail_on() {
+  static const bool on = [] { const char* q = getenv("TFK_HB_TAIL"); return q && atoi(q) != 0; }();
+  return on;
 }
 bool x3_operands_ok(const GemmArgsB& p, long a_rows, long b_rows) {
   if (p.M <= 0 || p.N <= 0 || p.K <= 0 || (p.lda & 31) || (p.ldb & 31) || (p.ldc & 3)) return false;
@@ -1470,13 +1569,27 @@
 }
 }
 
-int gemm_bf16x3_dual(const GemmArgsB& nt, const GemmArgsB& tn, hipStream_t stream) {
+int gemm_bf16x3_dual(const GemmArgsB& nt, const GemmArgsB& tn, hipStream_t stream, const HbTailArgs* tail, int* tail_ran) {
+  if (tail_ran) *tail_ran = 0;
   if (!x3_operands_ok(nt, nt.M, nt.N) || !x3_operands_ok(tn, tn.K, tn.K)) return (int)hipErrorInvalidValue;
   if ((nt.epi != 0 && nt.epi != EPI_DACT) || (tn.epi != 0 && tn.epi != EPI_ACCUM)) return -1;
   static const bool on = !getenv("TFK_BF16X3_DUAL") || atoi(getenv("TFK_BF16X3_DUAL")) != 0;
   const long tiles = (long)((nt.M + 127) / 128) * ((nt.N + 127) / 128) + (long)((tn.M + 127) / 128) * ((tn.N + 127) / 128);
   if (!on || tiles < 256) return -1;
   if ((long)nt.M * nt.ldc * 4 >= (1L << 31) || (long)tn.M * tn.ldc * 4 >= (1L << 31)) return -1;
+  if (tail && tail->ctr && hb_tail_on() && nt.epi == EPI_DACT && tn.K <= nt.K && x3_waves() != 44 && tail->hb.pre_du == 1 &&
+      tail->hb.da == nt.C && tail->hb.ws == nt.stats && tail->hb.ld == nt.ldc && tail->hb.T == nt.M && tail->hb.T_apply == nt.M &&
+      tail->hb.gx > 0 && tail->hb.gy > 0) {
+    int rc;
+    if (tn.epi == EPI_ACCUM)
+      rc = x3_waves() == 8 ? launch_x3_dual<EPI_DACT, EPI_ACCUM, 4, true>(nt, tn, stream, tail)
+                           : launch_x3_dual<EPI_DACT, EPI_ACCUM, 2, true>(nt, tn, stream, tail);
+    else
+      rc = x3_waves() == 8 ? launch_x3_dual<EPI_DACT, 0, 4, true>(nt, tn, stream, tail)
+                           : launch_x3_dual<EPI_DACT, 0, 2, true>(nt, tn, stream, tail);
+    if (rc == 0 && tail_ran) *tail_ran = 1;
+    return rc;
+  }
   const int key = (nt.epi == EPI_DACT ? 2 : 0) + (tn.epi == EPI_ACCUM ? 1 : 0);
   switch (key) {
 #define TFK_X3_DUAL(E1, E2)                                                                \
diff --git a/tfkaldi_amd/csrc/hb_apply.h b/tfkaldi_amd/csrc/hb_apply.h
--- /dev/null
+++ b/tfkaldi_amd/csrc/hb_apply.h
@@ -0,0 +1,281 @@
+#pragma once
+#include "kernels.h"
+
+namespace tfk {
+
+struct HbApplyArgs {
+  ActDesc d;
+  int pre_du;
+  float* da;
+  const float *a, *z, *mean, *rstd;
+  int T, H, ld, rows_per, rs_in;
+  float* ws;
+  Twin tw;
+  int T_apply;
+  float* ws_dz;
+  int nt;
+  int gx, gy;
+};
+HbApplyArgs hidden_backward_args(const ActDesc& d, int pre_du, float* da, const float* a, const float* z, const float* mean,
+                                 const float* rstd, int T, int H, int ld, float* ws, int stats_chunks, Twin tw, int T_apply = 0,
+                                 float* ws_dz = nullptr);
+
+#if defined(__HIPCC__)
+namespace hbk {
+
+constexpr int NONLIN_RELU = 0, NONLIN_SIGMOID = 1, NONLIN_TANH = 2, NONLIN_LINEAR = 3;
+
+__device__ __forceinline__ uint4 philox4x32(uint4 c, uint2 k) {
+#pragma unroll
+  for (int r = 0; r < 7; ++r) {
+    const uint32_t hi0 = __umulhi(0xD2511F53u, c.x), lo0 = 0xD2511F53u * c.x;
+    const uint32_t hi1 = __umulhi(0xCD9E8D57u, c.z), lo1 = 0xCD9E8D57u * c.z;
+    c = make_uint4(hi1 ^ c.y ^ k.x, lo1, hi0 ^ c.w ^ k.y, lo0);
+    k.x += 0x9E3779B9u;
+    k.y += 0xBB67AE85u;
+  }
+  return c;
+}
+struct Keep4 { bool k[4]; };
+__device__ __forceinline__ Keep4 keep_mask(const ActDesc& d, int row, int c4) {
+  const uint4 r = philox4x32(make_uint4((uint32_t)c4, (uint32_t)row, d.layer, d.call),
+                             make_uint2((uint32_t)d.seed, (uint32_t)(d.seed >> 32)));
+  const uint32_t thr = (uint32_t)fminf((1.0f - d.keep) * 4294967296.0f, 4294967295.0f);
+  Keep4 m;
+  m.k[0] = r.x >= thr; m.k[1] = r.y >= thr; m.k[2] = r.z >= thr; m.k[3] = r.w >= thr;
+  return m;
+}
+
+__device__ __forceinline__ float nonlin_bwd(float v, int nonlin) {
+  switch (nonlin) {
+    case NONLIN_RELU: return v > 0.f ? 1.f : 0.f;
+    case NONLIN_SIGMOID: return v * (1.f - v);
+    case NONLIN_TANH: return 1.f - v * v;
+    default: return 1.f;
+  }
+}
+
+__device__ __forceinline__ float4 ld4(const float* p) { return *reinterpret_cast<const float4*>(p); }
+typedef uint16_t u16x4 __attribute__((ext_vector_type(4)));
+__device__ __forceinline__ uint16_t to_bf16(float x) { return __builtin_bit_cast(uint16_t, (__bf16)x); }
+__device__ __forceinline__ void st4_twin(const Twin& t, size_t row, int col, float4 v) {
+  if (!t.p) return;
+  if (t.x3) {
+    uint16_t a[4], b[4], c[4];
+    twin_split3(v.x, a[0], b[0], c[0]); twin_split3(v.y, a[1], b[1], c[1]);
+    twin_split3(v.z, a[2], b[2], c[2]); twin_split3(v.w, a[3], b[3], c[3]);
+    u16x4 q1, q2, q3;
+    q1.x = a[0]; q1.y = a[1]; q1.z = a[2]; q1.w = a[3];
+    q2.x = b[0]; q2.y = b[1]; q2.z = b[2]; q2.w = b[3];
+    q3.x = c[0]; q3.y = c[1]; q3.z = c[2]; q3.w = c[3];
+    uint16_t* d = t.p + x3::at(row, col, t.ld);
+    *reinterpret_cast<u16x4*>(d) = q1;
+    *reinterpret_cast<u16x4*>(d + 64) = q2;
+    *reinterpret_cast<u16x4*>(d + 128) = q3;
+    return;
+  }
+  u16x4 q;
+  q.x = to_bf16(v.x); q.y = to_bf16(v.y); q.z = to_bf16(v.z); q.w = to_bf16(v.w);
+  *reinterpret_cast<u16x4*>(t.p + row * t.ld + col) = q;
+}
+__device__ __forceinline__ void st4(float* p, float4 v) { *reinterpret_cast<float4*>(p) = v; }
+typedef float v4f_nt __attribute__((ext_vector_type(4)));
+__device__ __forceinline__ void st4_nt(float* p, float4 v) {
+  v4f_nt q;
+  q.x = v.x; q.y = v.y; q.z = v.z; q.w = v.w;
+  __builtin_nontemporal_store(q, reinterpret_cast<v4f_nt*>(p));
+}
+__device__ __forceinline__ void st4_twin_nt(const Twin& t, size_t row, int col, float4 v) {
+  if (!t.p) return;
+  if (t.x3) {
+    uint16_t a[4], b[4], c[4];
+    twin_split3(v.x, a[0], b[0], c[0]); twin_split3(v.y, a[1], b[1], c[1]);
+    twin_split3(v.z, a[2], b[2], c[2]); twin_split3(v.w, a[3], b[3], c[3]);
+    u16x4 q1, q2, q3;
+    q1.x = a[0]; q1.y = a[1]; q1.z = a[2]; q1.w = a[3];
+    q2.x = b[0]; q2.y = b[1]; q2.z = b[2]; q2.w = b[3];
+    q3.x = c[0]; q3.y = c[1]; q3.z = c[2]; q3.w = c[3];
+    uint16_t* d = t.p + x3::at(row, col, t.ld);
+    __builtin_nontemporal_store(q1, reinterpret_cast<u16x4*>(d));
+    __builtin_nontemporal_store(q2, reinterpret_cast<u16x4*>(d + 64));
+    __builtin_nontemporal_store(q3, reinterpret_cast<u16x4*>(d + 128));
+    return;
+  }
+  u16x4 q;
+  q.x = to_bf16(v.x); q.y = to_bf16(v.y); q.z = to_bf16(v.z); q.w = to_bf16(v.w);
+  __builtin_nontemporal_store(q, reinterpret_cast<u16x4*>(t.p + row * t.ld + col));
+}
+__device__ __forceinline__ float4 ld4s(const float* p, int nt) {
+  if (nt & 4) {
+    const v4f_nt q = __builtin_nontemporal_load(reinterpret_cast<const v4f_nt*>(p));
+    return make_float4(q.x, q.y, q.z, q.w);
+  }
+  return *reinterpret_cast<const float4*>(p);
+}
+__device__ __forceinline__ float& el(float4& v, int i) { return reinterpret_cast<float*>(&v)[i]; }
+__device__ __forceinline__ float el(const float4& v, int i) { return reinterpret_cast<const float*>(&v)[i]; }
+
+constexpr int CT_X = 32, CT_Y = 8;
+constexpr int RB = 4;
+
+struct VBlock {
+  int bx, by, tx, ty;
+  bool live;
+};
+__device__ __forceinline__ float4 reduce_rows_v(float4 v, float4 (*sm)[CT_X], const VBlock& vb) {
+  sm[vb.ty][vb.tx] = v;
+  __syncthreads();
+  float4 t = make_float4(0.f, 0.f, 0.f, 0.f);
+  if (vb.ty == 0) {
+#pragma unroll
+    for (int k = 0; k < CT_Y; ++k) {
+      const float4 q = sm[k][vb.tx];
+      t.x += q.x; t.y += q.y; t.z += q.z; t.w += q.w;
+    }
+  }
+  __syncthreads();
+  return t;
+}
+
+__device__ __forceinline__ float4 compute_du(const ActDesc& d, int pre_du, float4 g, float4 a, int row, int c4) {
+  if (pre_du) return g;
+  float4 o;
+  if (d.keep < 1.f) {
+    const Keep4 m = keep_mask(d, row, c4);
+    const float inv_keep = 1.f / d.keep;
+#pragma unroll
+    for (int k = 0; k < 4; ++k)
+      el(o, k) = m.k[k] ? el(g, k) * inv_keep * nonlin_bwd(el(a, k) * d.keep, d.nonlin) : 0.f;
+  } else {
+#pragma unroll
+    for (int k = 0; k < 4; ++k) el(o, k) = el(g, k) * nonlin_bwd(el(a, k), d.nonlin);
+  }
+  return o;
+}
+
+constexpr int kAuxSc1 = 1 << 4;
+__device__ __forceinline__ float4 ld4_handed(__amdgpu_buffer_rsrc_t rs, size_t float_off, bool ok) {
+  typedef float f32x4 __attribute__((ext_vector_type(4)));
+  const f32x4 q = __builtin_bit_cast(
+      f32x4, __builtin_amdgcn_raw_buffer_load_b128(rs, ok ? (unsigned)(float_off * 4) : 0x80000000u, 0, kAuxSc1));
+  return make_float4(q.x, q.y, q.z, q.w);
+}
+
+template <bool HANDED>
+__device__ __forceinline__ void hb_apply_body(const HbApplyArgs& p, const VBlock& vb, float4 (*sm)[CT_X], float4 (*smm)[CT_X]) {
+  const ActDesc& d = p.d;
+  const int pre_du = HANDED ? 1 : p.pre_du;
+  float* __restrict__ da = p.da;
+  const float* __restrict__ a = p.a;
+  const float* __restrict__ z = p.z;
+  const float* __restrict__ ws = p.ws;
+  const int T = p.T, H = p.H, ld = p.ld, rs_in = p.rs_in, nt = p.nt;
+  const Twin tw = p.tw;
+  __amdgpu_buffer_rsrc_t da_rs, ws_rs;
+  if constexpr (HANDED) {
+    da_rs = __builtin_amdgcn_make_buffer_rsrc((void*)p.da, 0, (int)((unsigned)p.T_apply * (unsigned)ld * 4u), 0x00020000);
+    ws_rs = __builtin_amdgcn_make_buffer_rsrc((void*)p.ws, 0, (int)(2u * kMaxRowSplits * (unsigned)ld * 4u), 0x00020000);
+  }
+  auto ld_du = [&](size_t off, bool ok) {
+    if constexpr (HANDED) return ld4_handed(da_rs, off, ok);
+    else return ok ? ld4s(da + off, nt) : make_float4(0.f, 0.f, 0.f, 0.f);
+  };
+  const int c4 = vb.bx * CT_X + vb.tx;
+  const int col = c4 * 4;
+  const bool valid = vb.live && col < ld;
+  const int r0 = vb.by * p.rows_per;
+  const int r1 = min(p.T_apply, r0 + p.rows_per);
+  float4 sz = make_float4(0.f, 0.f, 0.f, 0.f);
+  const float4 zero4 = sz;
+  float4 m1 = sz, m2 = sz;
+  const int rb0 = r0 + vb.ty;
+  float4 g[RB], av[RB], zv[RB];
+#pragma unroll
+  for (int j = 0; j < RB; ++j) {
+    const int r = rb0 + j * CT_Y;
+    const bool ok = valid && rb0 < r1;
+    const size_t off = (size_t)(r < r1 ? r : rb0) * ld + col;
+    g[j] = ld_du(off, ok);
+    av[j] = (ok && !pre_du) ? ld4s(a + off, nt) : g[j];
+    zv[j] = (ok && d.bn) ? ld4s(z + off, nt) : (HANDED ? zero4 : g[j]);
+  }
+  float4 mu = sz, rsd = sz;
+  if (d.bn && valid) {
+    mu = ld4(p.mean + col); rsd = ld4(p.rstd + col);
+  }
+  if (d.bn) {
+    float4 p1 = sz, p2 = sz;
+    if (valid)
+      for (int k = vb.ty; k < rs_in; k += CT_Y) {
+        float4 q1, q2;
+        if constexpr (HANDED) {
+          q1 = ld4_handed(ws_rs, ((size_t)0 * kMaxRowSplits + k) * ld + col, true);
+          q2 = ld4_handed(ws_rs, ((size_t)1 * kMaxRowSplits + k) * ld + col, true);
+        } else {
+          q1 = ld4(ws + ((size_t)0 * kMaxRowSplits + k) * ld + col);
+          q2 = ld4(ws + ((size_t)1 * kMaxRowSplits + k) * ld + col);
+        }
+        p1.x += q1.x; p1.y += q1.y; p1.z += q1.z; p1.w += q1.w;
+        p2.x += q2.x; p2.y += q2.y; p2.z += q2.z; p2.w += q2.w;
+      }
+    p1 = reduce_rows_v(p1, sm, vb);
+    p2 = reduce_rows_v(p2, sm, vb);
+    if (vb.ty == 0) {
+      const float invT = 1.f / (float)T;
+      smm[0][vb.tx] = make_float4(p1.x * invT, p1.y * invT, p1.z * invT, p1.w * invT);
+      smm[1][vb.tx] = make_float4(p2.x * invT, p2.y * invT, p2.z * invT, p2.w * invT);
+    }
+    __syncthreads();
+    m1 = smm[0][vb.tx];
+    m2 = smm[1][vb.tx];
+  }
+  if (valid) {
+    for (int rb = rb0; rb < r1; rb += CT_Y * RB) {
+      float4 gn[RB], an[RB], zn[RB];
+      const int rbn = rb + CT_Y * RB;
+#pragma unroll
+      for (int j = 0; j < RB; ++j) {
+        const int r = rbn + j * CT_Y;
+        const bool ok = rbn < r1;
+        const size_t off = (size_t)(r < r1 ? r : rbn) * ld + col;
+        gn[j] = ld_du(off, ok);
+        an[j] = (ok && !pre_du) ? ld4s(a + off, nt) : gn[j];
+        zn[j] = (ok && d.bn) ? ld4s(z + off, nt) : (HANDED ? zero4 : gn[j]);
+      }
+#pragma unroll
+      for (int j = 0; j < RB; ++j) {
+        const int r = rb + j * CT_Y;
+        if (r >= r1) continue;
+        float4 dz = compute_du(d, pre_du, g[j], av[j], r, c4);
+        if (d.bn) {
+          dz.x = rsd.x * (dz.x - m1.x - (zv[j].x - mu.x) * rsd.x * m2.x);
+          dz.y = rsd.y * (dz.y - m1.y - (zv[j].y - mu.y) * rsd.y * m2.y);
+          dz.z = rsd.z * (dz.z - m1.z - (zv[j].z - mu.z) * rsd.z * m2.z);
+          dz.w = rsd.w * (dz.w - m1.w - (zv[j].w - mu.w) * rsd.w * m2.w);
+        }
+        if (r >= T) dz = zero4;
+#pragma unroll
+        for (int k = 0; k < 4; ++k)
+          if (col + k >= H) el(dz, k) = 0.f;
+        if (tw.p) {
+          if (nt & 2) st4_twin_nt(tw, r, col, dz);
+          else st4_twin(tw, r, col, dz);
+        } else {
+          st4(da + (size_t)r * ld + col, dz);
+        }
+        sz.x += dz.x; sz.y += dz.y; sz.z += dz.z; sz.w += dz.w;
+      }
+#pragma unroll
+      for (int j = 0; j < RB; ++j) {
+        g[j] = gn[j]; av[j] = an[j]; zv[j] = zn[j];
+      }
+    }
+  }
+  sz = reduce_rows_v(sz, sm, vb);
+  if (vb.ty == 0 && valid) st4(p.ws_dz + (size_t)vb.by * ld + col, sz);
+}
+
+}
+#endif
+
+}
diff --git a/tfkaldi_amd/csrc/kernels.hip b/tfkaldi_amd/csrc/kernels.hip
--- a/tfkaldi_amd/csrc/kernels.hip
+++ b/tfkaldi_amd/csrc/kernels.hip
@@ -1,4 +1,5 @@
 #include "kernels.h"
+#include "hb_apply.h"
 
 #include <math.h>
 #include <stdlib.h>
@@ -6,7 +7,7 @@
 namespace tfk {
 namespace {
 
-constexpr int NONLIN_RELU = 0, NONLIN_SIGMOID = 1, NONLIN_TANH = 2, NONLIN_LINEAR = 3;
+using namespace hbk;
 
 __device__ __forceinline__ float wave_sum(float v) {
 #pragma unroll
@@ -37,27 +38,6 @@
   for (int k = 1; k < nw; ++k) t = fmaxf(t, sm[k]);
   __syncthreads();
   return t;
-}
-
-__device__ __forceinline__ uint4 philox4x32(uint4 c, uint2 k) {
-#pragma unroll
-  for (int r = 0; r < 7; ++r) {
-    const uint32_t hi0 = __umulhi(0xD2511F53u, c.x), lo0 = 0xD2511F53u * c.x;
-    const uint32_t hi1 = __umulhi(0xCD9E8D57u, c.z), lo1 = 0xCD9E8D57u * c.z;
-    c = make_uint4(hi1 ^ c.y ^ k.x, lo1, hi0 ^ c.w ^ k.y, lo0);
-    k.x += 0x9E3779B9u;
-    k.y += 0xBB67AE85u;
-  }
-  return c;
-}
-struct Keep4 { bool k[4]; };
-__device__ __forceinline__ Keep4 keep_mask(const ActDesc& d, int row, int c4) {
-  const uint4 r = philox4x32(make_uint4((uint32_t)c4, (uint32_t)row, d.layer, d.call),
-                             make_uint2((uint32_t)d.seed, (uint32_t)(d.seed >> 32)));
-  const uint32_t thr = (uint32_t)fminf((1.0f - d.keep) * 4294967296.0f, 4294967295.0f);
-  Keep4 m;
-  m.k[0] = r.x >= thr; m.k[1] = r.y >= thr; m.k[2] = r.z >= thr; m.k[3] = r.w >= thr;
-  return m;
 }
 
 __device__ __forceinline__ float nonlin_fwd(float u, int nonlin) {
@@ -68,84 +48,12 @@
     default: return u;
   }
 }
-__device__ __forceinline__ float nonlin_bwd(float v, int nonlin) {
-  switch (nonlin) {
-    case NONLIN_RELU: return v > 0.f ? 1.f : 0.f;
-    case NONLIN_SIGMOID: return v * (1.f - v);
-    case NONLIN_TANH: return 1.f - v * v;
-    default: return 1.f;
-  }
-}
-
-__device__ __forceinline__ float4 ld4(const float* p) { return *reinterpret_cast<const float4*>(p); }
-typedef uint16_t u16x4 __attribute__((ext_vector_type(4)));
-__device__ __forceinline__ uint16_t to_bf16(float x) { return __builtin_bit_cast(uint16_t, (__bf16)x); }
-__device__ __forceinline__ void st4_twin(const Twin& t, size_t row, int col, float4 v) {
-  if (!t.p) return;
-  if (t.x3) {
-    uint16_t a[4], b[4], c[4];
-    twin_split3(v.x, a[0], b[0], c[0]); twin_split3(v.y, a[1], b[1], c[1]);
-    twin_split3(v.z, a[2], b[2], c[2]); twin_split3(v.w, a[3], b[3], c[3]);
-    u16x4 q1, q2, q3;
-    q1.x = a[0]; q1.y = a[1]; q1.z = a[2]; q1.w = a[3];
-    q2.x = b[0]; q2.y = b[1]; q2.z = b[2]; q2.w = b[3];
-    q3.x = c[0]; q3.y = c[1]; q3.z = c[2]; q3.w = c[3];
-    uint16_t* d = t.p + x3::at(row, col, t.ld);
-    *reinterpret_cast<u16x4*>(d) = q1;
-    *reinterpret_cast<u16x4*>(d + 64) = q2;
-    *reinterpret_cast<u16x4*>(d + 128) = q3;
-    return;
-  }
-  u16x4 q;
-  q.x = to_bf16(v.x); q.y = to_bf16(v.y); q.z = to_bf16(v.z); q.w = to_bf16(v.w);
-  *reinterpret_cast<u16x4*>(t.p + row * t.ld + col) = q;
-}
-__device__ __forceinline__ void st4(float* p, float4 v) { *reinterpret_cast<float4*>(p) = v; }
-typedef float v4f_nt __attribute__((ext_vector_type(4)));
-__device__ __forceinline__ void st4_nt(float* p, float4 v) {
-  v4f_nt q;
-  q.x = v.x; q.y = v.y; q.z = v.z; q.w = v.w;
-  __builtin_nontemporal_store(q, reinterpret_cast<v4f_nt*>(p));
-}
-__device__ __forceinline__ void st4_twin_nt(const Twin& t, size_t row, int col, float4 v) {
-  if (!t.p) return;
-  if (t.x3) {
-    uint16_t a[4], b[4], c[4];
-    twin_split3(v.x, a[0], b[0], c[0]); twin_split3(v.y, a[1], b[1], c[1]);
-    twin_split3(v.z, a[2], b[2], c[2]); twin_split3(v.w, a[3], b[3], c[3]);
-    u16x4 q1, q2, q3;
-    q1.x = a[0]; q1.y = a[1]; q1.z = a[2]; q1.w = a[3];
-    q2.x = b[0]; q2.y = b[1]; q2.z = b[2]; q2.w = b[3];
-    q3.x = c[0]; q3.y = c[1]; q3.z = c[2]; q3.w = c[3];
-    uint16_t* d = t.p + x3::at(row, col, t.ld);
-    __builtin_nontemporal_store(q1, reinterpret_cast<u16x4*>(d));
-    __builtin_nontemporal_store(q2, reinterpret_cast<u16x4*>(d + 64));
-    __builtin_nontemporal_store(q3, reinterpret_cast<u16x4*>(d + 128));
-    return;
-  }
-  u16x4 q;
-  q.x = to_bf16(v.x); q.y = to_bf16(v.y); q.z = to_bf16(v.z); q.w = to_bf16(v.w);
-  __builtin_nontemporal_store(q, reinterpret_cast<u16x4*>(t.p + row * t.ld + col));
-}
-__device__ __forceinline__ float4 ld4s(const float* p, int nt) {
-  if (nt & 4) {
-    const v4f_nt q = __builtin_nontemporal_load(reinterpret_cast<const v4f_nt*>(p));
-    return make_float4(q.x, q.y, q.z, q.w);
-  }
-  return *reinterpret_cast<const float4*>(p);
-}
 int bn_nt_mode(const Twin& tw, int rows, int ld) {
   static const int forced = [] { const char* q = getenv("TFK_BN_NT"); return q ? atoi(q) : -1; }();
   if (forced >= 0) return forced;
   const size_t twin_bytes = tw.p ? (size_t)rows * ld * (tw.x3 ? 6 : 2) : 0;
   return 1 | (twin_bytes >= ((size_t)8 << 20) ? 2 : 0);
 }
-__device__ __forceinline__ float& el(float4& v, int i) { return reinterpret_cast<float*>(&v)[i]; }
-__device__ __forceinline__ float el(const float4& v, int i) { return reinterpret_cast<const float*>(&v)[i]; }
-
-constexpr int CT_X = 32, CT_Y = 8;
-constexpr int RB = 4;
-
 struct ColTile {
   int c4;
   int col;
@@ -523,22 +431,6 @@
   }
 }
 
-__device__ __forceinline__ float4 compute_du(const ActDesc& d, int pre_du, float4 g, float4 a, int row, int c4) {
-  if (pre_du) return g;
-  float4 o;
-  if (d.keep < 1.f) {
-    const Keep4 m = keep_mask(d, row, c4);
-    const float inv_keep = 1.f / d.keep;
-#pragma unroll
-    for (int k = 0; k < 4; ++k)
-      el(o, k) = m.k[k] ? el(g, k) * inv_keep * nonlin_bwd(el(a, k) * d.keep, d.nonlin) : 0.f;
-  } else {
-#pragma unroll
-    for (int k = 0; k < 4; ++k) el(o, k) = el(g, k) * nonlin_bwd(el(a, k), d.nonlin);
-  }
-  return o;
-}
-
 __global__ void __launch_bounds__(CT_X * CT_Y)
 hb_stats_kernel(ActDesc d, int pre_du, const float* __restrict__ da, const float* __restrict__ a,
                 const float* __restrict__ z, const float* __restrict__ mean, const float* __restrict__ rstd, int T,
@@ -577,96 +469,11 @@
   }
 }
 
-__global__ void __launch_bounds__(CT_X * CT_Y)
-hb_apply_kernel(ActDesc d, int pre_du, float* __restrict__ da, const float* __restrict__ a,
-                const float* __restrict__ z, const float* __restrict__ mean, const float* __restrict__ rstd, int T,
-                int H, int ld, int rows_per, int rs_in, float* __restrict__ ws, Twin tw, int T_apply,
-                float* __restrict__ ws_dz, int nt) {
+__global__ void __launch_bounds__(CT_X * CT_Y) hb_apply_kernel(HbApplyArgs p) {
   __shared__ float4 sm[CT_Y][CT_X];
-  const ColTile t = col_tile(T_apply, ld, rows_per);
-  float4 sz = make_float4(0.f, 0.f, 0.f, 0.f);
-  const float4 zero4 = sz;
-  float4 m1 = sz, m2 = sz;
-  const int rb0 = t.r0 + threadIdx.y;
-  float4 g[RB], av[RB], zv[RB];
-#pragma unroll
-  for (int j = 0; j < RB; ++j) {
-    const int r = rb0 + j * CT_Y;
-    const bool ok = t.valid && rb0 < t.r1;
-    const size_t off = (size_t)(r < t.r1 ? r : rb0) * ld + t.col;
-    g[j] = ok ? ld4s(da + off, nt) : zero4;
-    av[j] = (ok && !pre_du) ? ld4s(a + off, nt) : g[j];
-    zv[j] = (ok && d.bn) ? ld4s(z + off, nt) : g[j];
-  }
-  float4 mu = sz, rsd = sz;
-  if (d.bn && t.valid) {
-    mu = ld4(mean + t.col); rsd = ld4(rstd + t.col);
-  }
-  if (d.bn) {
-    float4 p1 = sz, p2 = sz;
-    if (t.valid)
-      for (int k = threadIdx.y; k < rs_in; k += CT_Y) {
-        const float4 q1 = ld4(ws + ((size_t)0 * kMaxRowSplits + k) * ld + t.col);
-        const float4 q2 = ld4(ws + ((size_t)1 * kMaxRowSplits + k) * ld + t.col);
-        p1.x += q1.x; p1.y += q1.y; p1.z += q1.z; p1.w += q1.w;
-        p2.x += q2.x; p2.y += q2.y; p2.z += q2.z; p2.w += q2.w;
-      }
-    __shared__ float4 smm[2][CT_X];
-    p1 = reduce_rows(p1, sm);
-    p2 = reduce_rows(p2, sm);
-    if (threadIdx.y == 0) {
-      const float invT = 1.f / (float)T;
-      smm[0][threadIdx.x] = make_float4(p1.x * invT, p1.y * invT, p1.z * invT, p1.w * invT);
-      smm[1][threadIdx.x] = make_float4(p2.x * invT, p2.y * invT, p2.z * invT, p2.w * invT);
-    }
-    __syncthreads();
-    m1 = smm[0][threadIdx.x];
-    m2 = smm[1][threadIdx.x];
-  }
-  if (t.valid) {
-    for (int rb = rb0; rb < t.r1; rb += CT_Y * RB) {
-      float4 gn[RB], an[RB], zn[RB];
-      const int rbn = rb + CT_Y * RB;
-#pragma unroll
-      for (int j = 0; j < RB; ++j) {
-        const int r = rbn + j * CT_Y;
-        const bool ok = rbn < t.r1;
-        const size_t off = (size_t)(r < t.r1 ? r : rbn) * ld + t.col;
-        gn[j] = ok ? ld4s(da + off, nt) : zero4;
-        an[j] = (ok && !pre_du) ? ld4s(a + off, nt) : gn[j];
-        zn[j] = (ok && d.bn) ? ld4s(z + off, nt) : gn[j];
-      }
-#pragma unroll
-      for (int j = 0; j < RB; ++j) {
-        const int r = rb + j * CT_Y;
-        if (r >= t.r1) continue;
-        float4 dz = compute_du(d, pre_du, g[j], av[j], r, t.c4);
-        if (d.bn) {
-          dz.x = rsd.x * (dz.x - m1.x - (zv[j].x - mu.x) * rsd.x * m2.x);
-          dz.y = rsd.y * (dz.y - m1.y - (zv[j].y - mu.y) * rsd.y * m2.y);
-          dz.z = rsd.z * (dz.z - m1.z - (zv[j].z - mu.z) * rsd.z * m2.z);
-          dz.w = rsd.w * (dz.w - m1.w - (zv[j].w - mu.w) * rsd.w * m2.w);
-        }
-        if (r >= T) dz = zero4;
-#pragma unroll
-        for (int k = 0; k < 4; ++k)
-          if (t.col + k >= H) el(dz, k) = 0.f;
-        if (tw.p) {
-          if (nt & 2) st4_twin_nt(tw, r, t.col, dz);
-          else st4_twin(tw, r, t.col, dz);
-        } else {
-          st4(da + (size_t)r * ld + t.col, dz);
-        }
-        sz.x += dz.x; sz.y += dz.y; sz.z += dz.z; sz.w += dz.w;
-      }
-#pragma unroll
-      for (int j = 0; j < RB; ++j) {
-        g[j] = gn[j]; av[j] = an[j]; zv[j] = zn[j];
-      }
-    }
-  }
-  sz = reduce_rows(sz, sm);
-  if (threadIdx.y == 0 && t.valid) st4(ws_dz + (size_t)blockIdx.y * ld + t.col, sz);
+  __shared__ float4 smm[2][CT_X];
+  const VBlock vb = {(int)blockIdx.x, (int)blockIdx.y, (int)threadIdx.x, (int)threadIdx.y, true};
+  hb_apply_body<false>(p, vb, sm, smm);
 }
 
 __global__ void __launch_bounds__(FIN_COLS * FIN_KL) grad_final_kernel(FinalBatch b) {
@@ -1181,17 +988,30 @@
   hipLaunchKernelGGL(act_backward_rows_kernel, dim3(grid), dim3(256), 0, s, d, da, v, rowscale, T, H, ld);
 }
 
+HbApplyArgs hidden_backward_args(const ActDesc& d, int pre_du, float* da, const float* a, const float* z, const float* mean,
+                                 const float* rstd, int T, int H, int ld, float* ws, int stats_chunks, Twin tw, int T_apply,
+                                 float* ws_dz) {
+  if (T_apply < T) T_apply = T;
+  const int rs = row_splits(T_apply), rows_per = (T_apply + rs - 1) / rs;
+  const dim3 grid = ct_grid(ld, rs);
+  HbApplyArgs p = {};
+  p.d = d; p.pre_du = pre_du; p.da = da; p.a = a; p.z = z; p.mean = mean; p.rstd = rstd;
+  p.T = T; p.H = H; p.ld = ld; p.rows_per = rows_per; p.rs_in = stats_chunks > 0 ? stats_chunks : rs;
+  p.ws = ws; p.tw = tw; p.T_apply = T_apply;
+  p.ws_dz = ws_dz ? ws_dz : ws + (size_t)2 * kMaxRowSplits * ld;
+  p.nt = bn_nt_mode(tw, T_apply, ld);
+  p.gx = (int)grid.x; p.gy = (int)grid.y;
+  return p;
+}
+
 void hidden_backward(hipStream_t s, const ActDesc& d, int pre_du, float* da, const float* a, const float* z,
                      const float* mean, const float* rstd, int T, int H, int ld, float* ws, int stats_chunks,
                      Twin tw, int T_apply, float* ws_dz) {
-  if (T_apply < T) T_apply = T;
-  const int rs = row_splits(T_apply), rows_per = (T_apply + rs - 1) / rs;
+  const HbApplyArgs p = hidden_backward_args(d, pre_du, da, a, z, mean, rstd, T, H, ld, ws, stats_chunks, tw, T_apply, ws_dz);
   if (d.bn && stats_chunks <= 0)
-    hipLaunchKernelGGL(hb_stats_kernel, ct_grid(ld, rs), ct_block(), 0, s, d, pre_du, da, a, z, mean, rstd, T, ld,
-                       rows_per, rs, ws);
-  hipLaunchKernelGGL(hb_apply_kernel, ct_grid(ld, rs), ct_block(), 0, s, d, pre_du, da, a, z, mean, rstd, T, H, ld,
-                     rows_per, stats_chunks > 0 ? stats_chunks : rs, ws, tw, T_apply,
-                     ws_dz ? ws_dz : ws + (size_t)2 * kMaxRowSplits * ld, bn_nt_mode(tw, T_apply, ld));
+    hipLaunchKernelGGL(hb_stats_kernel, dim3(p.gx, p.gy), ct_block(), 0, s, d, pre_du, da, a, z, mean, rstd, T, ld,
+                       p.rows_per, p.gy, ws);
+  hipLaunchKernelGGL(hb_apply_kernel, dim3(p.gx, p.gy), ct_block(), 0, s, p);
 }
 
 void bn_stats_from_chunks(hipStream_t s, const float* stats, int chunk_rows, int T, int H, int ld, float eps, float decay,
diff --git a/tfkaldi_amd/csrc/x3_layout.h b/tfkaldi_amd/csrc/x3_layout.h
--- a/tfkaldi_amd/csrc/x3_layout.h
+++ b/tfkaldi_amd/csrc/x3_layout.h
@@ -116,6 +116,14 @@
   return (r > 0 && j_q1 > j_q) ? kXcds * j_q + r : kXcds * j_q;
 }
 
+X3_HD int hb_tail_items(int gx, int gy, int nv) { return (gx * gy + nv - 1) / nv; }
+X3_HD bool hb_tail_vblock(int gx, int gy, int nv, int item, int half, int& bx, int& by) {
+  const int v = item * nv + half;
+  bx = v % gx;
+  by = v / gx;
+  return item >= 0 && half >= 0 && half < nv && v < gx * gy;
+}
+
 #if defined(__HIPCC__)
 __device__ __forceinline__ void split3(float x, uint16_t& p1, uint16_t& p2, uint16_t& p3) {
   const uint32_t ux = __builtin_bit_cast(uint32_t, x);
```

After: 956,900. Within noise of the previous version (-0.4%).
